# uzh-rpg/event_representation_study

Measured on AMD Instinct MI355X. Metric: events/sec/GPU (OptimizedRep, Gen1 640x480) + 12-rep GWD matrix wall-time, higher is better.
Workload: dtype f64

## Files before the change

### event_representation_study_amd/csrc/evrep_bin.hip

```cpp
#include "evrep_common.h"

namespace evrep {

#ifndef EVREP_BIN_THREADS
#define EVREP_BIN_THREADS 256
#endif
constexpr int kBinThreads = EVREP_BIN_THREADS;
constexpr int kBinWaves = kBinThreads / kWave;

template <typename Op>
__device__ inline int wave_reduce_dpp(int v, int identity, Op op) {
    v = op(v, __builtin_amdgcn_update_dpp(identity, v, 0x111, 0xf, 0xf, false));
    v = op(v, __builtin_amdgcn_update_dpp(identity, v, 0x112, 0xf, 0xf, false));
    v = op(v, __builtin_amdgcn_update_dpp(identity, v, 0x114, 0xf, 0xf, false));
    v = op(v, __builtin_amdgcn_update_dpp(identity, v, 0x118, 0xf, 0xf, false));
    v = op(v, __builtin_amdgcn_update_dpp(identity, v, 0x142, 0xa, 0xf, false));
    v = op(v, __builtin_amdgcn_update_dpp(identity, v, 0x143, 0xc, 0xf, false));
    return __builtin_amdgcn_readlane(v, 63);
}
__device__ inline int wave_min(int v) { return wave_reduce_dpp(v, INT32_MAX, [](int a, int b) { return min(a, b); }); }
__device__ inline int wave_max(int v) { return wave_reduce_dpp(v, INT32_MIN, [](int a, int b) { return max(a, b); }); }
__device__ inline uint32_t wave_or(uint32_t v) { return (uint32_t)wave_reduce_dpp((int)v, 0, [](int a, int b) { return a | b; }); }
__device__ inline int wave_sum(int v) { return wave_reduce_dpp(v, 0, [](int a, int b) { return a + b; }); }

__device__ inline void wave_phase_lds() {
    __builtin_amdgcn_fence(__ATOMIC_RELEASE, "wavefront");
    __builtin_amdgcn_wave_barrier();
    __builtin_amdgcn_fence(__ATOMIC_ACQUIRE, "wavefront");
}

struct BlockStats {
    int32_t tmin, tmax, xmin, xmax, ymin, ymax;
    uint32_t neg_flags, oob_flags, status;
    int32_t n_valid;
    int32_t pad[2];
};
static_assert(sizeof(BlockStats) == 48, "BlockStats");

__device__ inline void stats_identity(BlockStats &s) {
    s.tmin = INT32_MAX; s.tmax = INT32_MIN; s.xmin = INT32_MAX; s.xmax = INT32_MIN; s.ymin = INT32_MAX; s.ymax = INT32_MIN;
    s.neg_flags = 0; s.oob_flags = 0; s.status = 0; s.n_valid = 0; s.pad[0] = 0; s.pad[1] = 0;
}
__device__ inline void stats_merge(BlockStats &a, const BlockStats &b) {
    a.tmin = min(a.tmin, b.tmin); a.tmax = max(a.tmax, b.tmax);
    a.xmin = min(a.xmin, b.xmin); a.xmax = max(a.xmax, b.xmax);
    a.ymin = min(a.ymin, b.ymin); a.ymax = max(a.ymax, b.ymax);
    a.neg_flags |= b.neg_flags; a.oob_flags |= b.oob_flags; a.status |= b.status; a.n_valid += b.n_valid;
}
__device__ inline void stats_wave_reduce(BlockStats &s) {
    s.tmin = wave_min(s.tmin); s.tmax = wave_max(s.tmax);
    s.xmin = wave_min(s.xmin); s.xmax = wave_max(s.xmax);
    s.ymin = wave_min(s.ymin); s.ymax = wave_max(s.ymax);
    s.neg_flags = wave_or(s.neg_flags); s.oob_flags = wave_or(s.oob_flags); s.status = wave_or(s.status);
    s.n_valid = wave_sum(s.n_valid);
}

constexpr int kRegBatch = 8;

__device__ inline bool decode_window_block(int B, int nblk, int &b, int &blk) {
    const int id = blockIdx.x;
    const int per_group = 8 * nblk;
    const int grp = id / per_group, r = id - grp * per_group;
    const int nw = min(8, B - 8 * grp);
    if (nw == 8) {
        b = grp * 8 + (r & 7);
        blk = r >> 3;
        return true;
    }
    if (r >= nw * nblk) return false;
    b = grp * 8 + r / nblk;
    blk = r - (r / nblk) * nblk;
    return true;
}

#ifdef EVREP_TU_CORE
static __global__ __launch_bounds__(kBinThreads) void k_row_hist(const int4 *__restrict__ ev, const int64_t *__restrict__ off,
                                                      int B, int H, int W, int chunk, int nblk,
                                                      uint32_t *__restrict__ table, BlockStats *__restrict__ stats) {
    extern __shared__ uint32_t hist[];
    __shared__ BlockStats wstats[kBinWaves];
    int b, blk;
    if (!decode_window_block(B, nblk, b, blk)) return;
    const int64_t beg = off[b];
    const int64_t n = off[b + 1] - beg;
    const int64_t lo = (int64_t)blk * chunk;
    if (lo >= n) return;
    for (int i = threadIdx.x; i < H; i += kBinThreads) hist[i] = 0;
    __syncthreads();
    const int64_t hi = (lo + chunk < n) ? lo + chunk : n;
    const MdesWindows mw = mdes_windows(n);
    const int64_t HW = (int64_t)H * W;
    BlockStats st;
    stats_identity(st);
    for (int64_t r0 = lo; r0 < hi; r0 += (int64_t)kRegBatch * kBinThreads) {
        int4 e[kRegBatch];
        int tprev[kRegBatch];
#pragma unroll
        for (int i = 0; i < kRegBatch; ++i) {
            const int64_t r = r0 + (int64_t)i * kBinThreads + threadIdx.x;
            e[i] = make_int4(0, 0, INT32_MAX, 0);
            tprev[i] = INT32_MIN;
            if (r < hi) {
                e[i] = ev[beg + r];
                if ((threadIdx.x & 63) == 0 && r > 0) tprev[i] = ev[beg + r - 1].z;
            }
        }
#pragma unroll
        for (int i = 0; i < kRegBatch; ++i) {
            const int up = __shfl_up(e[i].z, 1, 64);
            if ((threadIdx.x & 63) != 0) tprev[i] = up;
        }
#pragma unroll
        for (int i = 0; i < kRegBatch; ++i) {
            const int64_t r = r0 + (int64_t)i * kBinThreads + threadIdx.x;
            if (r < hi) {
                const int64_t key = (int64_t)e[i].x + (int64_t)e[i].y * W;
                const uint32_t memb = mdes_membership(mw, (int32_t)r);
                if (e[i].w == -1) st.neg_flags |= memb;
                if (key >= 0 && key < HW) {
                    atomicAdd(&hist[(uint32_t)key / (uint32_t)W], 1u);
                    ++st.n_valid;
                } else {
                    st.status |= EVREP_ST_OOB;
                    const int cls = e[i].w == 1 ? 1 : (e[i].w == -1 ? 2 : (e[i].w == 0 ? 3 : 0));
                    st.oob_flags |= memb | (cls ? (memb << (7 * cls)) : 0u);
                }
                if (tprev[i] > e[i].z) st.status |= EVREP_ST_UNSORTED;
                st.tmin = min(st.tmin, e[i].z); st.tmax = max(st.tmax, e[i].z);
                st.xmin = min(st.xmin, e[i].x); st.xmax = max(st.xmax, e[i].x);
                st.ymin = min(st.ymin, e[i].y); st.ymax = max(st.ymax, e[i].y);
            }
        }
    }
    stats_wave_reduce(st);
    if ((threadIdx.x & 63) == 0) wstats[threadIdx.x >> 6] = st;
    __syncthreads();
    if (threadIdx.x == 0) {
        BlockStats t = wstats[0];
        for (int w = 1; w < kBinWaves; ++w) stats_merge(t, wstats[w]);
        stats[(size_t)b * nblk + blk] = t;
    }
    uint32_t *dst = table + ((size_t)b * nblk + blk) * H;
    for (int i = threadIdx.x; i < H; i += kBinThreads) dst[i] = hist[i];
}
#endif

#ifdef EVREP_TU_CORE
static __global__ __launch_bounds__(kBinThreads) void k_row_scan(const int64_t *__restrict__ off, int H, int chunk, int nblk,
                                                      uint32_t *__restrict__ table, uint32_t *__restrict__ row_off,
                                                      const BlockStats *__restrict__ stats, WindowMeta *__restrict__ meta) {
    extern __shared__ uint32_t rowtot[];
    __shared__ BlockStats wstats[kBinWaves];
    __shared__ uint32_t tmp[kBinWaves];
    const int b = blockIdx.x;
    const int64_t beg = off[b];
    const int64_t n = off[b + 1] - beg;
    const int nb = (int)((n + chunk - 1) / chunk);
    BlockStats st;
    stats_identity(st);
    for (int blk = threadIdx.x; blk < nb; blk += kBinThreads) stats_merge(st, stats[(size_t)b * nblk + blk]);
    stats_wave_reduce(st);
    if ((threadIdx.x & 63) == 0) wstats[threadIdx.x >> 6] = st;
    for (int r = threadIdx.x; r < H; r += kBinThreads) {
        uint32_t run = 0;
        for (int b0 = 0; b0 < nb; b0 += kRegBatch) {
            uint32_t v[kRegBatch];
#pragma unroll
            for (int i = 0; i < kRegBatch; ++i)
                v[i] = (b0 + i < nb) ? table[((size_t)b * nblk + b0 + i) * H + r] : 0u;
#pragma unroll
            for (int i = 0; i < kRegBatch; ++i)
                if (b0 + i < nb) { table[((size_t)b * nblk + b0 + i) * H + r] = run; run += v[i]; }
        }
        rowtot[r] = run;
    }
    __syncthreads();
    const int per = (H + kBinThreads - 1) / kBinThreads;
    const int r0 = threadIdx.x * per;
    uint32_t local = 0;
    for (int k = 0; k < per; ++k) if (r0 + k < H) local += rowtot[r0 + k];
    uint32_t total;
    uint32_t run = block_exclusive_scan<kBinWaves>(local, tmp, &total);
    for (int k = 0; k < per; ++k)
        if (r0 + k < H) { const uint32_t t = rowtot[r0 + k]; rowtot[r0 + k] = run; run += t; }
    __syncthreads();
    uint32_t *ro = row_off + (size_t)b * (H + 1);
    for (int r = threadIdx.x; r < H; r += kBinThreads) ro[r] = (uint32_t)beg + rowtot[r];
    if (threadIdx.x == 0) {
        ro[H] = (uint32_t)beg + total;
        BlockStats t = wstats[0];
        for (int w = 1; w < kBinWaves; ++w) stats_merge(t, wstats[w]);
        WindowMeta m;
        m.tmin = t.tmin; m.tmax = t.tmax; m.xmin = t.xmin; m.xmax = t.xmax; m.ymin = t.ymin; m.ymax = t.ymax;
        m.neg_flags = t.neg_flags; m.oob_flags = t.oob_flags; m.status = t.status; m.n_valid = t.n_valid;
        if (n <= 0) m.status |= EVREP_ST_EMPTY;
        else if (t.tmin == t.tmax) m.status |= EVREP_ST_FLAT_TIME;
        for (int i = 0; i < 6; ++i) m.pad[i] = 0;
        meta[b] = m;
    }
}
#endif

#ifdef EVREP_TU_CORE
static __global__ __launch_bounds__(kBinThreads) void k_row_scatter(const int4 *__restrict__ ev, const int64_t *__restrict__ off,
                                                         int B, int H, int W, int chunk, int nblk,
                                                         const uint32_t *__restrict__ table,
                                                         const uint32_t *__restrict__ row_off, Rec *__restrict__ sorted1) {
    extern __shared__ uint32_t cnt[];
    int b, blk;
    if (!decode_window_block(B, nblk, b, blk)) return;
    const int64_t beg = off[b];
    const int64_t n = off[b + 1] - beg;
    const int64_t lo = (int64_t)blk * chunk;
    if (lo >= n) return;
    const int64_t hi = (lo + chunk < n) ? lo + chunk : n;
    const int64_t nloc = hi - lo;
    const int lane = threadIdx.x & 63, wave = threadIdx.x >> 6;
    const int64_t wlo = lo + nloc * wave / kBinWaves, whi = lo + nloc * (wave + 1) / kBinWaves;
    const int64_t HW = (int64_t)H * W;
    constexpr int kSuper = kRegBatch * kWave;
    const int nsuper = (int)((whi - wlo + kSuper - 1) / kSuper);
    for (int i = threadIdx.x; i < kBinWaves * H; i += kBinThreads) cnt[i] = 0;
    __syncthreads();
    uint32_t *mycnt = cnt + wave * H;
    int4 e[kRegBatch];
    for (int sb = 0; sb < nsuper; ++sb) {
#pragma unroll
        for (int i = 0; i < kRegBatch; ++i) {
            const int64_t r = wlo + (int64_t)sb * kSuper + i * kWave + lane;
            e[i] = make_int4(-1, -1, 0, 0);
            if (r < whi) e[i] = ev[beg + r];
        }
#pragma unroll
        for (int i = 0; i < kRegBatch; ++i) {
            const int64_t r = wlo + (int64_t)sb * kSuper + i * kWave + lane;
            const int64_t key = (int64_t)e[i].x + (int64_t)e[i].y * W;
            if (r < whi && key >= 0 && key < HW) atomicAdd(&mycnt[(uint32_t)key / (uint32_t)W], 1u);
        }
    }
    __syncthreads();
    for (int row = threadIdx.x; row < H; row += kBinThreads) {
        uint32_t base = row_off[(size_t)b * (H + 1) + row] + table[((size_t)b * nblk + blk) * H + row];
#pragma unroll
        for (int w = 0; w < kBinWaves; ++w) { const uint32_t t = cnt[w * H + row]; cnt[w * H + row] = base; base += t; }
    }
    __syncthreads();
    const int nbits = bits_for(H);
    volatile uint32_t *vcnt = mycnt;
    for (int sb = 0; sb < nsuper; ++sb) {
        if (nsuper > 1) {
#pragma unroll
            for (int i = 0; i < kRegBatch; ++i) {
                const int64_t r = wlo + (int64_t)sb * kSuper + i * kWave + lane;
                e[i] = make_int4(-1, -1, 0, 0);
                if (r < whi) e[i] = ev[beg + r];
            }
        }
#pragma unroll
        for (int i = 0; i < kRegBatch; ++i) {
            const int64_t r0 = wlo + (int64_t)sb * kSuper + i * kWave;
            if (r0 >= whi) break;
            const int64_t r = r0 + lane;
            const int64_t key = (int64_t)e[i].x + (int64_t)e[i].y * W;
            const bool valid = r < whi && key >= 0 && key < HW;
            const uint32_t row = valid ? (uint32_t)key / (uint32_t)W : 0u;
            uint32_t rk; bool last;
            wave_match(row, nbits, valid, lane, rk, last);
            uint32_t pos = 0;
            if (valid) {
                pos = vcnt[row] + rk;
                sorted1[pos] = make_int4((int)key, (int)r, e[i].z, e[i].w);
            }
            __builtin_amdgcn_wave_barrier();
            if (valid && last) vcnt[row] = pos + 1;
            __builtin_amdgcn_wave_barrier();
        }
    }
}
#endif

constexpr int kStageRecs = 2048;
__host__ __device__ inline size_t fused_scatter_lds_bytes(int H) {
    return (size_t)(kBinWaves + 3) * H * sizeof(uint32_t) + (size_t)kStageRecs * sizeof(Rec);
}

#ifdef EVREP_TU_CORE
static __global__ __launch_bounds__(kBinThreads) void k_row_scatter_fused(const int4 *__restrict__ ev, const int64_t *__restrict__ off,
                                                               int B, int H, int W, int chunk, int nblk,
                                                               const uint32_t *__restrict__ table,
                                                               const BlockStats *__restrict__ stats,
                                                               uint32_t *__restrict__ row_off, WindowMeta *__restrict__ meta,
                                                               Rec *__restrict__ sorted1) {
    extern __shared__ __align__(16) unsigned char smem_raw[];
    Rec *stage = reinterpret_cast<Rec *>(smem_raw);
    uint32_t *cnt = reinterpret_cast<uint32_t *>(stage + kStageRecs);
    uint32_t *rowtot = cnt + kBinWaves * H;
    uint32_t *lbase = rowtot + H;
    uint32_t *delta = lbase + H;
    __shared__ BlockStats wstats[kBinWaves];
    __shared__ uint32_t tmp[kBinWaves];
    int b, blk;
    if (!decode_window_block(B, nblk, b, blk)) return;
    const int64_t beg = off[b];
    const int64_t n = off[b + 1] - beg;
    const int64_t lo = (int64_t)blk * chunk;
    if (lo >= n && !(blk == 0)) return;
    const int nb = (int)((n + chunk - 1) / chunk);
    if (n <= 0) {
        uint32_t *ro = row_off + (size_t)b * (H + 1);
        for (int r = threadIdx.x; r <= H; r += kBinThreads) ro[r] = (uint32_t)beg;
        if (threadIdx.x == 0) {
            WindowMeta m;
            m.tmin = INT32_MAX; m.tmax = INT32_MIN; m.xmin = INT32_MAX; m.xmax = INT32_MIN; m.ymin = INT32_MAX; m.ymax = INT32_MIN;
            m.neg_flags = 0; m.oob_flags = 0; m.status = EVREP_ST_EMPTY; m.n_valid = 0;
            for (int i = 0; i < 6; ++i) m.pad[i] = 0;
            meta[b] = m;
        }
        return;
    }
    const int64_t hi = (lo + chunk < n) ? lo + chunk : n;
    const int64_t nloc = hi - lo;
    const int lane = threadIdx.x & 63, wave = threadIdx.x >> 6;
    const int64_t wlo = lo + nloc * wave / kBinWaves, whi = lo + nloc * (wave + 1) / kBinWaves;
    const int64_t HW = (int64_t)H * W;
    for (int i = threadIdx.x; i < kBinWaves * H; i += kBinThreads) cnt[i] = 0;
    __syncthreads();
    uint32_t *mycnt = cnt + wave * H;
    int4 e[kRegBatch];
#pragma unroll
    for (int i = 0; i < kRegBatch; ++i) {
        const int64_t r = wlo + i * kWave + lane;
        e[i] = make_int4(-1, -1, 0, 0);
        if (r < whi) e[i] = ev[beg + r];
    }
#pragma unroll
    for (int i = 0; i < kRegBatch; ++i) {
        const int64_t r = wlo + i * kWave + lane;
        const int64_t key = (int64_t)e[i].x + (int64_t)e[i].y * W;
        if (r < whi && key >= 0 && key < HW) atomicAdd(&mycnt[(uint32_t)key / (uint32_t)W], 1u);
    }
    if (blk == 0) {
        BlockStats st;
        stats_identity(st);
        for (int k = threadIdx.x; k < nb; k += kBinThreads) stats_merge(st, stats[(size_t)b * nblk + k]);
        stats_wave_reduce(st);
        if (lane == 0) wstats[wave] = st;
    }
    __syncthreads();
    for (int r = threadIdx.x; r < H; r += kBinThreads) {
        uint32_t tot = 0, before = 0;
        for (int b0 = 0; b0 < nb; b0 += kRegBatch) {
            uint32_t v[kRegBatch];
#pragma unroll
            for (int i = 0; i < kRegBatch; ++i) v[i] = (b0 + i < nb) ? table[((size_t)b * nblk + b0 + i) * H + r] : 0u;
#pragma unroll
            for (int i = 0; i < kRegBatch; ++i) { tot += v[i]; if (b0 + i < blk) before += v[i]; }
        }
        rowtot[r] = tot;
        delta[r] = before;
        uint32_t own = 0;
#pragma unroll
        for (int w = 0; w < kBinWaves; ++w) own += cnt[w * H + r];
        lbase[r] = own;
    }
    __syncthreads();
    const int per = (H + kBinThreads - 1) / kBinThreads;
    const int r0 = threadIdx.x * per;
    uint32_t loc_t = 0, loc_o = 0;
    for (int k = 0; k < per; ++k) if (r0 + k < H) { loc_t += rowtot[r0 + k]; loc_o += lbase[r0 + k]; }
    uint32_t total_t, total_o;
    uint32_t run_t = block_exclusive_scan<kBinWaves>(loc_t, tmp, &total_t);
    uint32_t run_o = block_exclusive_scan<kBinWaves>(loc_o, tmp, &total_o);
    for (int k = 0; k < per; ++k)
        if (r0 + k < H) {
            const uint32_t t = rowtot[r0 + k]; rowtot[r0 + k] = run_t; run_t += t;
            const uint32_t o = lbase[r0 + k];  lbase[r0 + k] = run_o;  run_o += o;
        }
    __syncthreads();
    for (int r = threadIdx.x; r < H; r += kBinThreads) {
        const uint32_t gstart = (uint32_t)beg + rowtot[r] + delta[r];
        uint32_t base = lbase[r];
        delta[r] = gstart - base;
#pragma unroll
        for (int w = 0; w < kBinWaves; ++w) { const uint32_t t = cnt[w * H + r]; cnt[w * H + r] = base; base += t; }
        if (blk == 0) row_off[(size_t)b * (H + 1) + r] = (uint32_t)beg + rowtot[r];
    }
    if (blk == 0 && threadIdx.x == 0) {
        row_off[(size_t)b * (H + 1) + H] = (uint32_t)beg + total_t;
        BlockStats t = wstats[0];
        for (int w = 1; w < kBinWaves; ++w) stats_merge(t, wstats[w]);
        WindowMeta m;
        m.tmin = t.tmin; m.tmax = t.tmax; m.xmin = t.xmin; m.xmax = t.xmax; m.ymin = t.ymin; m.ymax = t.ymax;
        m.neg_flags = t.neg_flags; m.oob_flags = t.oob_flags; m.status = t.status; m.n_valid = t.n_valid;
        if (t.tmin == t.tmax) m.status |= EVREP_ST_FLAT_TIME;
        for (int i = 0; i < 6; ++i) m.pad[i] = 0;
        meta[b] = m;
    }
    __syncthreads();
    const int nbits = bits_for(H);
    volatile uint32_t *vcnt = mycnt;
#pragma unroll
    for (int i = 0; i < kRegBatch; ++i) {
        const int64_t rr0 = wlo + i * kWave;
        if (rr0 >= whi) break;
        const int64_t r = rr0 + lane;
        const int64_t key = (int64_t)e[i].x + (int64_t)e[i].y * W;
        const bool valid = r < whi && key >= 0 && key < HW;
        const uint32_t row = valid ? (uint32_t)key / (uint32_t)W : 0u;
        uint32_t rk; bool last;
        wave_match(row, nbits, valid, lane, rk, last);
        uint32_t pos = 0;
        if (valid) {
            pos = vcnt[row] + rk;
            stage[pos] = make_int4((int)key, (int)r, e[i].z, e[i].w);
        }
        __builtin_amdgcn_wave_barrier();
        if (valid && last) vcnt[row] = pos + 1;
        __builtin_amdgcn_wave_barrier();
    }
    __syncthreads();
    for (uint32_t t = threadIdx.x; t < total_o; t += kBinThreads) {
        const Rec rec = stage[t];
        const uint32_t row = (uint32_t)rec.x / (uint32_t)W;
        sorted1[delta[row] + t] = rec;
    }
}
#endif

#ifdef EVREP_TU_CORE
static __global__ __launch_bounds__(kWave) void k_col_sort(const Rec *__restrict__ sorted1, const uint32_t *__restrict__ row_off,
                                                   int H, int W, int nchunk, Rec *__restrict__ sorted2,
                                                   uint32_t *__restrict__ chunk_off) {
    extern __shared__ uint32_t cnt[];
    const int b = blockIdx.y, row = blockIdx.x;
    const int lane = threadIdx.x;
    const uint32_t rs = row_off[(size_t)b * (H + 1) + row], re = row_off[(size_t)b * (H + 1) + row + 1];
    const uint32_t n = re - rs;
    uint32_t *co = chunk_off + ((size_t)b * H + row) * (nchunk + 1);
    if (n == 0) {
        for (int c = lane; c <= nchunk; c += kWave) co[c] = rs;
        return;
    }
    constexpr uint32_t kSuper = 4 * kWave;
    const int rowbase = row * W;
    const uint32_t nsuper = (n + kSuper - 1) / kSuper;
    Rec e[4];
    for (int i = lane; i < W; i += kWave) cnt[i] = 0;
    __syncthreads();
    for (uint32_t sb = 0; sb < nsuper; ++sb) {
#pragma unroll
        for (int i = 0; i < 4; ++i) {
            const uint32_t j = sb * kSuper + i * kWave + lane;
            e[i] = make_int4(0, 0, 0, 0);
            if (j < n) e[i] = sorted1[rs + j];
        }
#pragma unroll
        for (int i = 0; i < 4; ++i)
            if (sb * kSuper + i * kWave + lane < n) atomicAdd(&cnt[e[i].x - rowbase], 1u);
    }
    __syncthreads();
    const int per = (W + kWave - 1) / kWave;
    const int c0 = lane * per;
    uint32_t local = 0;
    for (int k = 0; k < per; ++k) if (c0 + k < W) local += cnt[c0 + k];
    uint32_t incl = local;
#pragma unroll
    for (int d = 1; d < 64; d <<= 1) { const uint32_t o = __shfl_up(incl, d, 64); if (lane >= d) incl += o; }
    uint32_t run = incl - local;
    for (int k = 0; k < per; ++k)
        if (c0 + k < W) { const uint32_t t = cnt[c0 + k]; cnt[c0 + k] = run; run += t; }
    __syncthreads();
    for (int c = lane; c <= nchunk; c += kWave) co[c] = (c * kChunkPx < W) ? rs + cnt[c * kChunkPx] : re;
    __syncthreads();
    const int nbits = bits_for(W);
    volatile uint32_t *vcnt = cnt;
    for (uint32_t sb = 0; sb < nsuper; ++sb) {
        if (nsuper > 1) {
#pragma unroll
// ... 169 lines not shown
    volatile uint16_t *vpos = cnt16 + (size_t)wave * Hp;
#pragma unroll
    for (int i = 0; i < kBsPerLane; ++i) {
        if (wlo + i * kWave >= whi) break;
        const bool valid = rows[i] != 0xffffffffu;
        const uint32_t row = valid ? rows[i] : 0u;
        uint32_t rk = 0; bool last = false;
        if (!(BS_DEBUG & 2)) wave_match(row, nbits, valid, lane, rk, last);
        uint32_t pos = 0;
        if (valid) {
            pos = (BS_DEBUG & 2) ? (uint32_t)(wave * 512 + i * 64 + lane) : (uint32_t)vpos[row] + rk;
            const int64_t r = wlo + i * kWave + lane;
            const Rec rec = make_int4((int)((int64_t)e[i].x + (int64_t)e[i].y * W), (int)r, e[i].z, e[i].w);
            if (BS_DEBUG & 16) sorted1[beg + lo + pos] = rec; else stage[pos] = rec;
        }
        __builtin_amdgcn_wave_barrier();
        if (valid && last) vpos[row] = (uint16_t)(pos + 1);
        __builtin_amdgcn_wave_barrier();
    }
    __syncthreads();
    Rec *dst = sorted1 + beg + lo;
    if (!(BS_DEBUG & (4 | 16)))
        for (uint32_t t = threadIdx.x; t < total; t += kBsThreads) dst[t] = stage[t];
}
#endif

#ifndef EVREP_CS_WAVES
#define EVREP_CS_WAVES 8
#endif
constexpr int kCsWaves = EVREP_CS_WAVES;
constexpr int kCsRowWaves = 4;
constexpr int kCsMaxRuns = 128;
__host__ __device__ inline int col_sort_per4(int W) { return ((W + kWave - 1) / kWave + 3) / 4; }
__host__ __device__ inline int col_sort_words(int W) { return kWave * 4 * col_sort_per4(W); }
__host__ __device__ inline int col_sort_wave_words(int W) { return col_sort_words(W) + 2 * kCsMaxRuns; }

#ifndef CS_WAVES
#define CS_WAVES 8
#endif
#ifdef EVREP_TU_CORE
static __global__ __launch_bounds__(kCsWaves * kWave) __attribute__((amdgpu_waves_per_eu(CS_WAVES))) void k_col_sort_runs(const int4 *__restrict__ ev, const Rec *__restrict__ sorted1, const int64_t *__restrict__ off,
                                                                     const uint32_t *__restrict__ table,
                                                                     const BlockStats *__restrict__ stats, int H, int W, int nblk,
                                                                     int nchunk, int kpr, int chunk_shift, int by_key,
                                                                     Rec *__restrict__ sorted2,
                                                                     uint32_t *__restrict__ chunk_off, WindowMeta *__restrict__ meta) {
    extern __shared__ __align__(16) uint32_t cnt_all[];
    const int lane = threadIdx.x & 63, wave = threadIdx.x >> 6;
    const int b = blockIdx.y, unit = blockIdx.x * (int)(blockDim.x >> 6) + wave;
    if (unit >= (by_key ? H * kpr : H)) return;
    const int row = by_key ? unit / kpr : unit;
    const int ck = by_key ? unit - row * kpr : 0;
    const int Wu = by_key ? min(kChunkPx, W - ck * kChunkPx) : W;
    uint32_t *cnt = cnt_all + (size_t)wave * col_sort_wave_words(by_key ? kChunkPx : W);
    const int64_t beg = off[b];
    const int64_t n_win = off[b + 1] - beg;
    const int nb = min((int)(((uint32_t)n_win + (1u << chunk_shift) - 1u) >> chunk_shift), nblk);
    uint32_t ta[2] = {0u, 0u}, tb[2] = {0u, 0u};
#pragma unroll
    for (int h = 0; h < 2; ++h) {
        const int k = lane + h * kWave;
        if (k < nb) {
            const uint32_t *tk = table + ((size_t)b * nblk + k) * ((size_t)H * kpr + 1);
            ta[h] = tk[by_key ? (size_t)unit : (size_t)row * kpr];
            tb[h] = tk[by_key ? (size_t)unit + 1 : (size_t)(row + 1) * kpr];
        }
    }
    if (unit == 0) {
        BlockStats st;
        stats_identity(st);
#pragma unroll
        for (int h = 0; h < 2; ++h) {
            const int k = lane + h * kWave;
            if (k < nb) {
                const int4 *sp = reinterpret_cast<const int4 *>(stats + (size_t)b * nblk + k);
                const int4 q0 = sp[0], q1 = sp[1], q2 = sp[2];
                st.tmin = min(st.tmin, q0.x); st.tmax = max(st.tmax, q0.y); st.xmin = min(st.xmin, q0.z); st.xmax = max(st.xmax, q0.w);
                st.ymin = min(st.ymin, q1.x); st.ymax = max(st.ymax, q1.y);
                st.neg_flags |= (uint32_t)q1.z; st.oob_flags |= (uint32_t)q1.w;
                st.status |= (uint32_t)q2.x; st.n_valid += q2.y;
            }
        }
        stats_wave_reduce(st);
        if (lane == 0) {
            WindowMeta m;
            m.tmin = st.tmin; m.tmax = st.tmax; m.xmin = st.xmin; m.xmax = st.xmax; m.ymin = st.ymin; m.ymax = st.ymax;
            m.neg_flags = st.neg_flags; m.oob_flags = st.oob_flags; m.status = st.status & 0xffffu; m.n_valid = st.n_valid;
            if (n_win <= 0) m.status |= EVREP_ST_EMPTY;
            else if (st.tmin == st.tmax) m.status |= EVREP_ST_FLAT_TIME;
            for (int i = 0; i < 6; ++i) m.pad[i] = 0;
            meta[b] = m;
        }
    }
    constexpr uint32_t kSuper = 4 * kWave;
    const uint32_t rbeg = (uint32_t)beg + (uint32_t)wave_sum((int)(ta[0] + ta[1]));
    const uint32_t len0 = tb[0] - ta[0], len1 = tb[1] - ta[1];
    uint32_t incl0 = len0, incl1 = len1;
#pragma unroll
    for (int d = 1; d < 64; d <<= 1) {
        const uint32_t o0 = __shfl_up(incl0, d, 64), o1 = __shfl_up(incl1, d, 64);
        if (lane >= d) { incl0 += o0; incl1 += o1; }
    }
    const uint32_t tot0 = (uint32_t)__builtin_amdgcn_readlane((int)incl0, 63);
    incl1 += tot0;
    const uint32_t n = (uint32_t)__builtin_amdgcn_readlane((int)incl1, 63);
    const uint32_t pre0 = incl0 - len0, pre1 = incl1 - len1;
    const uint32_t src0 = (uint32_t)beg + ((uint32_t)lane << chunk_shift) + ta[0] - pre0;
    const uint32_t src1 = (uint32_t)beg + ((uint32_t)(lane + kWave) << chunk_shift) + ta[1] - pre1;
    const uint32_t rend = rbeg + n;
    uint32_t *runs = cnt + col_sort_words(by_key ? kChunkPx : W);
    if (nb > kBsChainBlocks) {
        runs[lane] = pre0;
        runs[kWave + lane] = pre1;
        runs[kCsMaxRuns + lane] = src0;
        runs[kCsMaxRuns + kWave + lane] = src1;
        wave_phase_lds();
    }
    const Rec8 *sorted8 = reinterpret_cast<const Rec8 *>(sorted1);
    const int4 *evw = ev + beg;
    auto load = [&](uint32_t at) -> Rec {
        return by_key ? rec8_unpack(sorted8[at], row * W, ck * kChunkPx, evw) : sorted1[at];
    };
    auto fetch = [&](uint32_t j) -> Rec {
        if (nb <= kBsChainBlocks) {
            uint32_t s = (uint32_t)__builtin_amdgcn_readlane((int)src0, 0);
            uint32_t prev = s;
            for (int k = 1; k < nb; ++k) {
                const uint32_t pk = (uint32_t)__builtin_amdgcn_readlane((int)pre0, k);
                const uint32_t sk = (uint32_t)__builtin_amdgcn_readlane((int)src0, k);
                s += (j >= pk) ? sk - prev : 0u;
                prev = sk;
            }
            return load(s + j);
        }
        uint32_t lo = 0, hi = (uint32_t)nb;
#pragma unroll
        for (int step = 0; step < 7; ++step) {
            const uint32_t mid = (lo + hi) >> 1;
            const bool go = hi - lo > 1 && runs[mid] <= j;
            if (hi - lo > 1) { if (go) lo = mid; else hi = mid; }
        }
        return load(runs[kCsMaxRuns + lo] + j);
    };
    Rec e[4];
#pragma unroll
    for (int i = 0; i < 4; ++i) {
        const uint32_t j = i * kWave + lane;
        e[i] = make_int4(0, 0, 0, 0);
        if (j < n) e[i] = fetch(j);
    }
    const int nbits = bits_for(Wu);
    const int per4 = col_sort_per4(Wu);
    uint4 *cnt4 = reinterpret_cast<uint4 *>(cnt) + (size_t)lane * per4;
    volatile uint32_t *vcnt = cnt;
    uint32_t *co = chunk_off + ((size_t)b * H + row) * (nchunk + 1);
    if (by_key && lane == 0) {
        co[ck] = rbeg;
        if (ck == kpr - 1) co[kpr] = rend;
    }
    if (n == 0) {
        if (!by_key) for (int c = lane; c <= nchunk; c += kWave) co[c] = rbeg;
        return;
    }
    const int rowbase = row * W + ck * kChunkPx;
    const uint32_t nsuper = (n + kSuper - 1) / kSuper;
    for (int k = 0; k < per4; ++k) cnt4[k] = make_uint4(0u, 0u, 0u, 0u);
    wave_phase_lds();
#pragma unroll
    for (int i = 0; i < 4; ++i)
        if ((uint32_t)(i * kWave + lane) < n) atomicAdd(&cnt[e[i].x - rowbase], 1u);
    for (uint32_t sb = 1; sb < nsuper; ++sb)
        for (int i = 0; i < 4; ++i) {
            const uint32_t j = sb * kSuper + i * kWave + lane;
            if (j < n) atomicAdd(&cnt[fetch(j).x - rowbase], 1u);
        }
    wave_phase_lds();
    uint32_t local = 0;
    for (int k = 0; k < per4; ++k) { const uint4 v = cnt4[k]; local += v.x + v.y + v.z + v.w; }
    uint32_t inc2 = local;
#pragma unroll
    for (int d = 1; d < 64; d <<= 1) { const uint32_t o = __shfl_up(inc2, d, 64); if (lane >= d) inc2 += o; }
    uint32_t run = inc2 - local;
    for (int k = 0; k < per4; ++k) {
        const uint4 v = cnt4[k];
        uint4 o;
        o.x = run; o.y = o.x + v.x; o.z = o.y + v.y; o.w = o.z + v.z;
        run = o.w + v.w;
        cnt4[k] = o;
    }
    wave_phase_lds();
    if (!by_key) for (int c = lane; c <= nchunk; c += kWave) co[c] = (c * kChunkPx < W) ? rbeg + cnt[c * kChunkPx] : rend;
    wave_phase_lds();
    for (uint32_t sb = 0; sb < nsuper; ++sb) {
#pragma unroll
        for (int i = 0; i < 4; ++i) {
            const uint32_t j0 = sb * kSuper + i * kWave;
            if (j0 >= n) break;
            const bool valid = j0 + lane < n;
            Rec rec = e[i];
            if (sb > 0) { rec = make_int4(0, 0, 0, 0); if (valid) rec = fetch(j0 + lane); }
            const uint32_t col = valid ? (uint32_t)(rec.x - rowbase) : 0u;
            uint32_t rk; bool last;
            wave_match(col, nbits, valid, lane, rk, last);
            uint32_t pos = 0;
            if (valid) {
                pos = vcnt[col] + rk;
                sorted2[rbeg + pos] = rec;
            }
            __builtin_amdgcn_wave_barrier();
            if (valid && last) vcnt[col] = pos + 1;
            __builtin_amdgcn_wave_barrier();
        }
    }
}
#endif

#ifndef KS_DIRECT_WRITE
#define KS_DIRECT_WRITE 0
#endif
#ifndef KS_DEBUG
#define KS_DEBUG 0
#endif
constexpr int kKsHotGroup = 16;
__host__ __device__ inline size_t block_keysort_lds_bytes(int NK, int cap, int chunk) {
    return (size_t)cap * sizeof(Rec8) + (size_t)chunk * sizeof(uint16_t) + (size_t)(NK + 4) * sizeof(uint32_t);
}

#ifndef KS_WAVES_512
#define KS_WAVES_512 6
#endif
#ifndef KS_WAVES_1024
#define KS_WAVES_1024 8
#endif
template <int TPB, int PL = 8>
__global__ __launch_bounds__(TPB) __attribute__((amdgpu_waves_per_eu(TPB == 1024 ? KS_WAVES_1024 : KS_WAVES_512))) void k_block_keysort(const int4 *__restrict__ ev, const int64_t *__restrict__ off,
                                                             int B, int H, int W, int kpr, int nblk, int cap,
                                                             uint32_t *__restrict__ table, BlockStats *__restrict__ stats,
                                                             Rec *__restrict__ sorted1, int64_t *__restrict__ nwin,
                                                             uint32_t *__restrict__ hot) {
    extern __shared__ __align__(16) unsigned char smem_raw[];
    constexpr int kChunk = TPB * PL, kNW = TPB / kWave, kPerWave = PL * kWave;
    if (blockIdx.x == 0 && threadIdx.x < 128) hot[threadIdx.x * 16] = 0u;
    const int NK = H * kpr;
    Rec8 *stage = reinterpret_cast<Rec8 *>(smem_raw);
    uint16_t *rankbuf = reinterpret_cast<uint16_t *>(stage + cap);
    uint32_t *base = reinterpret_cast<uint32_t *>(rankbuf + kChunk);
    __shared__ int bstats[12];
    __shared__ uint32_t tmp[kNW];
    __shared__ uint32_t nhot_s;
    int b, blk;
    if (!decode_window_block(B, nblk, b, blk)) return;
    const int64_t beg = off[b];
    const int64_t n = off[b + 1] - beg;
    const int64_t lo = (int64_t)blk * kChunk;
    if (blk == 0 && threadIdx.x == 0) nwin[b] = n;
    if (lo >= n) return;
    const int nblock = (int)((lo + kChunk < n) ? kChunk : n - lo);
    const int lane = threadIdx.x & 63, wave = threadIdx.x >> 6;
    const int w0 = wave * kPerWave;
    const int lo32 = (int)lo;
    const int4 *evb = ev + beg + lo;
    int4 e[PL];
    int tprev[PL];
#pragma unroll
    for (int i = 0; i < PL; ++i) {
        const int li = w0 + i * kWave + lane;
        e[i] = make_int4(-1, -1, INT32_MAX, 0);
        tprev[i] = INT32_MIN;
        if (li < nblock) {
            e[i] = evb[li];
            if (lane == 0 && (li > 0 || lo > 0)) tprev[i] = evb[li - 1].z;
        }
    }
    for (int i = threadIdx.x; i <= NK; i += TPB) base[i] = 0;
    if (threadIdx.x == 0) nhot_s = 0u;
    if (threadIdx.x < 12) {
        const int f = threadIdx.x;
        bstats[f] = (f == 0 || f == 2 || f == 4) ? INT32_MAX : ((f == 1 || f == 3 || f == 5) ? INT32_MIN : 0);
    }
    __syncthreads();
    const MdesWindows mw = mdes_windows(n);
    uint32_t full = 0, part = 0;
#pragma unroll
    for (int i = 0; i < 7; ++i) {
        if (mw.lo[i] <= lo32 && lo32 + nblock <= mw.hi[i]) full |= 1u << i;
        else if (!(lo32 + nblock <= mw.lo[i] || lo32 >= mw.hi[i])) part |= 1u << i;
    }
    BlockStats st;
    stats_identity(st);
    uint32_t ko[PL];
    uint32_t sneg = 0;
    bool cut = false;
    const int a0 = lo32 + w0, a1 = min(lo32 + w0 + kPerWave, lo32 + nblock);
    if (part) {
#pragma unroll
        for (int q = 0; q < 7; ++q) cut |= (mw.lo[q] > a0 && mw.lo[q] < a1) || (mw.hi[q] > a0 && mw.hi[q] < a1);
    }
    const uint32_t memb_u = cut ? 0u : (full | (part ? (mdes_membership(mw, a0) & part) : 0u));
    const int HW = H * W;
#pragma unroll
    for (int i = 0; i < PL; ++i) {
        const int li = w0 + i * kWave + lane;
        const bool in = li < nblock;
        const int up = __builtin_amdgcn_update_dpp(0, e[i].z, 0x138 , 0xf, 0xf, false);
        if (lane != 0) tprev[i] = up;
        uint32_t row = (uint32_t)e[i].y, col = (uint32_t)e[i].x;
        bool valid = in && (uint32_t)e[i].x < (uint32_t)W && (uint32_t)e[i].y < (uint32_t)H;
        if (__any(in && (uint32_t)e[i].x >= (uint32_t)W)) {
            const int64_t key = (int64_t)e[i].x + (int64_t)e[i].y * W;
            valid = in && key >= 0 && key < (int64_t)HW;
            if (valid) { row = (uint32_t)key / (uint32_t)W; col = (uint32_t)key - row * (uint32_t)W; }
        }
        ko[i] = 0xffffffffu;
        if (valid) {
            const uint32_t key = row * (uint32_t)kpr + (col >> 7);
            ko[i] = key | (atomicAdd(&base[key], 1u) << 16);
        }
        if (KS_DEBUG & 4) continue;
        if (!cut) {
            if (__any(in && e[i].w == -1)) sneg |= memb_u;
        } else if (in && e[i].w == -1) {
            st.neg_flags |= full | (mdes_membership(mw, lo32 + li) & part);
        }
        if (__any(in && !valid)) {
            if (in && !valid) {
                const uint32_t memb = cut ? (full | (mdes_membership(mw, lo32 + li) & part)) : memb_u;
                st.status |= EVREP_ST_OOB;
                const int cls = e[i].w == 1 ? 1 : (e[i].w == -1 ? 2 : (e[i].w == 0 ? 3 : 0));
                st.oob_flags |= memb | (cls ? (memb << (7 * cls)) : 0u);
            }
        }
        if (in) {
            if (valid) ++st.n_valid;
            if (tprev[i] > e[i].z) st.status |= EVREP_ST_UNSORTED;
            if ((uint32_t)(e[i].w + 1) > 2u) st.status |= kStEscaped;
            st.tmin = min(st.tmin, e[i].z); st.tmax = max(st.tmax, e[i].z);
            st.xmin = min(st.xmin, e[i].x); st.xmax = max(st.xmax, e[i].x);
            st.ymin = min(st.ymin, e[i].y); st.ymax = max(st.ymax, e[i].y);
        }
    }
    st.neg_flags |= sneg;
    stats_wave_reduce(st);
    if (lane == 0) {
        atomicMin(&bstats[0], st.tmin); atomicMax(&bstats[1], st.tmax);
        atomicMin(&bstats[2], st.xmin); atomicMax(&bstats[3], st.xmax);
        atomicMin(&bstats[4], st.ymin); atomicMax(&bstats[5], st.ymax);
        atomicOr(reinterpret_cast<uint32_t *>(&bstats[6]), st.neg_flags);
        atomicOr(reinterpret_cast<uint32_t *>(&bstats[7]), st.oob_flags);
        atomicOr(reinterpret_cast<uint32_t *>(&bstats[8]), st.status);
        atomicAdd(&bstats[9], st.n_valid);
    }
    __syncthreads();
    const int per = (NK + TPB - 1) / TPB;
    const int k0 = (int)threadIdx.x * per;
    uint32_t local = 0;
    for (int k = 0; k < per; ++k) if (k0 + k < NK) local += base[k0 + k];
    uint32_t total;
    uint32_t run = block_exclusive_scan<kNW>(local, tmp, &total);
    for (int k = 0; k < per; ++k)
        if (k0 + k < NK) {
            const uint32_t c = base[k0 + k];
            uint32_t tag = 0u;
            if (c > (uint32_t)kKsHotGroup) tag = (atomicAdd(&nhot_s, 1u) + 1u) << 16;
            base[k0 + k] = run | tag;
            run += c;
        }
    if (threadIdx.x == 0) base[NK] = total;
    if (threadIdx.x < 12) reinterpret_cast<int *>(stats + (size_t)b * nblk + blk)[threadIdx.x] = bstats[threadIdx.x];
    __syncthreads();
    uint32_t *tb = table + ((size_t)b * nblk + blk) * ((size_t)NK + 1);
    if (!(KS_DEBUG & 8))
        for (int k = threadIdx.x; k <= NK; k += TPB) tb[k] = base[k] & 0xffffu;
    const uint32_t nhot = nhot_s;
    const uint32_t mine0 = (uint32_t)(w0 + lane);
#pragma unroll
    for (int i = 0; i < PL; ++i) {
        if (ko[i] != 0xffffffffu) {
            const uint32_t bw = base[ko[i] & 0xffffu];
            if (!(bw >> 16)) rankbuf[(bw & 0xffffu) + (ko[i] >> 16)] = (uint16_t)(mine0 + i * kWave);
        }
    }
    if (nhot) {
        constexpr int kHs = kChunk / 16;
        uint32_t *hcnt = reinterpret_cast<uint32_t *>(stage);
        for (uint32_t t = lane; t < nhot; t += kWave) hcnt[wave * kHs + t] = 0u;
        wave_phase_lds();
#pragma unroll
        for (int i = 0; i < PL; ++i)
            if (ko[i] != 0xffffffffu) {
                const uint32_t hsl = base[ko[i] & 0xffffu] >> 16;
                if (hsl) atomicAdd(&hcnt[wave * kHs + hsl - 1u], 1u);
            }
        __syncthreads();
        if (threadIdx.x < nhot) {
            uint32_t acc = 0;
            for (int w = 0; w < kNW; ++w) { const uint32_t c = hcnt[w * kHs + threadIdx.x]; hcnt[w * kHs + threadIdx.x] = acc; acc += c; }
        }
        __syncthreads();
        const int hbits = bits_for((int)nhot);
        volatile uint32_t *vh = hcnt + wave * kHs;
#pragma unroll
        for (int i = 0; i < PL; ++i) {
            const uint32_t bw = ko[i] != 0xffffffffu ? base[ko[i] & 0xffffu] : 0u;
            const bool hot = (bw >> 16) != 0u;
            if (!__any(hot)) continue;
            const uint32_t slot = hot ? (bw >> 16) - 1u : 0u;
            uint32_t rk; bool last;
            wave_match(slot, hbits, hot, lane, rk, last);
            uint32_t pos = 0;
            if (hot) {
                pos = vh[slot] + rk;
                ko[i] = ((bw & 0xffffu) + pos) | 0x80000000u;
            }
            __builtin_amdgcn_wave_barrier();
            if (hot && last) vh[slot] = pos + 1;
            __builtin_amdgcn_wave_barrier();
        }
    }
    __syncthreads();
    {
        uint32_t gb[PL], g[PL], sm[PL];
        uint32_t gmax = 0;
#pragma unroll
        for (int i = 0; i < PL; ++i) {
            gb[i] = 0; g[i] = 0; sm[i] = 0;
            if (ko[i] != 0xffffffffu && !(ko[i] >> 31)) {
                const uint32_t key = ko[i] & 0xffffu;
                const uint32_t bw = base[key];
                gb[i] = bw & 0xffffu;
                g[i] = (bw >> 16) ? 0u : (base[key + 1] & 0xffffu) - gb[i];
                if (KS_DEBUG & 1) { sm[i] = ko[i] >> 16; g[i] = 0; }
                if (g[i] == 1) g[i] = 0;
                gmax = max(gmax, g[i]);
            }
        }
        gmax = (uint32_t)wave_max((int)gmax);
        for (uint32_t j = 0; j < gmax; ++j) {
#pragma unroll
            for (int i = 0; i < PL; ++i)
                if (j < g[i]) sm[i] += (uint32_t)rankbuf[gb[i] + j] < mine0 + (uint32_t)(i * kWave) ? 1u : 0u;
        }
#pragma unroll
        for (int i = 0; i < PL; ++i)
            if (ko[i] != 0xffffffffu) ko[i] = (ko[i] >> 31) ? (ko[i] & 0x7fffffffu) : gb[i] + sm[i];
    }
    if (nhot) __syncthreads();
    Rec8 *dst = reinterpret_cast<Rec8 *>(sorted1) + beg + lo;
#if KS_DIRECT_WRITE
#pragma unroll
    for (int i = 0; i < PL; ++i) {
        if (ko[i] != 0xffffffffu && !(KS_DEBUG & 2)) {
            int col = e[i].x;
            if ((uint32_t)col >= (uint32_t)W) { const uint32_t key = (uint32_t)(e[i].x + e[i].y * W); col = (int)(key % (uint32_t)W); }
            dst[ko[i]] = rec8_pack(col, lo32 + w0 + i * kWave + lane, e[i].z, e[i].w);
        }
    }
    return;
#endif
    for (uint32_t pb = 0; pb < total && !(KS_DEBUG & 2); pb += (uint32_t)cap) {
        if (pb) __syncthreads();
#pragma unroll
        for (int i = 0; i < PL; ++i) {
            const uint32_t pos = ko[i] - pb;
            if (pos < (uint32_t)cap) {
                int col = e[i].x;
                if ((uint32_t)col >= (uint32_t)W) { const uint32_t key = (uint32_t)(e[i].x + e[i].y * W); col = (int)(key % (uint32_t)W); }
                stage[pos] = rec8_pack(col, lo32 + w0 + i * kWave + lane, e[i].z, e[i].w);
            }
        }
        __syncthreads();
        const uint32_t cnt = min((uint32_t)cap, total - pb);
        for (uint32_t t = threadIdx.x; t < cnt; t += TPB) dst[pb + t] = stage[t];
    }
}

#ifdef EVREP_TU_CORE
static __global__ __launch_bounds__(kWave) void k_window_meta(const int64_t *__restrict__ nwin, const BlockStats *__restrict__ stats,
                                                      int nblk, int chunk_shift, WindowMeta *__restrict__ meta) {
    const int b = blockIdx.x, lane = threadIdx.x;
    const int64_t n_win = nwin[b];
    const int nb = min((int)(((uint32_t)n_win + (1u << chunk_shift) - 1u) >> chunk_shift), nblk);
    BlockStats st;
    stats_identity(st);
    for (int k = lane; k < nb; k += kWave) stats_merge(st, stats[(size_t)b * nblk + k]);
    stats_wave_reduce(st);
    if (lane == 0) {
        WindowMeta m;
        m.tmin = st.tmin; m.tmax = st.tmax; m.xmin = st.xmin; m.xmax = st.xmax; m.ymin = st.ymin; m.ymax = st.ymax;
        m.neg_flags = st.neg_flags; m.oob_flags = st.oob_flags; m.status = st.status & 0xffffu; m.n_valid = st.n_valid;
        if (n_win <= 0) m.status |= EVREP_ST_EMPTY;
        else if (st.tmin == st.tmax) m.status |= EVREP_ST_FLAT_TIME;
        for (int i = 0; i < 6; ++i) m.pad[i] = 0;
        meta[b] = m;
    }
}
#endif

}
```

### event_representation_study_amd/csrc/evrep_builders.hip

```cpp
#include "evrep_common.h"
#include "evrep_est_table.h"

namespace evrep {

__host__ __device__ inline size_t align16(size_t v) { return (v + 15) & ~(size_t)15; }

#ifndef EVREP_ES_WAVES
#define EVREP_ES_WAVES 6
#endif
#ifndef EVREP_TORE_WAVES
#define EVREP_TORE_WAVES 1
#endif
#ifndef EVREP_VOXEL_WAVES
#define EVREP_VOXEL_WAVES 6
#endif
#ifndef EVREP_PARTS
#define EVREP_PARTS 2
#endif
#ifndef EVREP_DEFER_MULT
#define EVREP_DEFER_MULT 1
#endif
#ifndef EVREP_XCD_MAP
#define EVREP_XCD_MAP 1
#endif
// ... 118 lines not shown
}

template <typename OutT>
__device__ inline void tile_store(const OutT *tile, int count, OutT *__restrict__ dst) {
    constexpr int V = 16 / (int)sizeof(OutT);
    if ((reinterpret_cast<uintptr_t>(dst) & 15u) == 0) {
        const int nvec = count / V;
        int v = threadIdx.x;
#if EVREP_NT_STORES
        typedef float nt4 __attribute__((ext_vector_type(4)));
        const nt4 *n4 = reinterpret_cast<const nt4 *>(tile);
        nt4 *o4 = reinterpret_cast<nt4 *>(dst);
        for (; v + 3 * kWave < nvec; v += 4 * kWave) {
            const nt4 a = n4[v], b = n4[v + kWave], c = n4[v + 2 * kWave], d = n4[v + 3 * kWave];
            __builtin_nontemporal_store(a, o4 + v); __builtin_nontemporal_store(b, o4 + v + kWave);
            __builtin_nontemporal_store(c, o4 + v + 2 * kWave); __builtin_nontemporal_store(d, o4 + v + 3 * kWave);
        }
        for (; v < nvec; v += kWave) __builtin_nontemporal_store(n4[v], o4 + v);
#else
        const float4 *s4 = reinterpret_cast<const float4 *>(tile);
        float4 *d4 = reinterpret_cast<float4 *>(dst);
        for (; v + 3 * kWave < nvec; v += 4 * kWave) {
            const float4 a = s4[v], b = s4[v + kWave], c = s4[v + 2 * kWave], d = s4[v + 3 * kWave];
            d4[v] = a; d4[v + kWave] = b; d4[v + 2 * kWave] = c; d4[v + 3 * kWave] = d;
        }
        for (; v < nvec; v += kWave) d4[v] = s4[v];
#endif
        for (int e = nvec * V + threadIdx.x; e < count; e += kWave) dst[e] = tile[e];
    } else {
        for (int e = threadIdx.x; e < count; e += kWave) dst[e] = tile[e];
    }
}

#ifndef EVREP_STREAM_BYRUN
#define EVREP_STREAM_BYRUN 12
#endif
#ifndef EVREP_STREAM_G
#define EVREP_STREAM_G 4
#endif
#ifndef EVREP_ORDERED_BYRUN
#define EVREP_ORDERED_BYRUN 48
#endif
#ifndef EVREP_VOXEL_BYRUN
#define EVREP_VOXEL_BYRUN 48
#endif
#ifndef EVREP_MDES_STREAM_BYRUN
#define EVREP_MDES_STREAM_BYRUN 48
#endif
__device__ inline int chunk_unit(int total) {
    const int lin = (int)(blockIdx.x + gridDim.x * (blockIdx.y + gridDim.y * blockIdx.z));
#if EVREP_XCD_MAP
    if ((total & 7) == 0) {
        const int per = total >> 3, xcd = lin & 7;
#ifdef EVREP_XCD_ROT
        int idx = (lin >> 3) + xcd * (EVREP_XCD_ROT);
        idx %= per;
#else
        const int idx = lin >> 3;
#endif
        return xcd * per + idx;
    }
#endif
    return lin;
}

struct ChunkGeom {
    int b, row, c0, npix;
    uint32_t cs, ce;
};

struct BinView {
    const int4 *ev;
    const Rec *sorted;
    const uint32_t *chunk_off;
    const uint32_t *table;
    const BlockStats *stats;
    const WindowMeta *meta;
    Rec *spill;
    int nblk, fused, chunk_shift;
    uint32_t *hot;
    uint32_t hot_cap;
    double *placed_pool;
    BlockStats *stats_rw;
#ifdef EVREP_TIMING
    unsigned long long *dbg;
    unsigned long long *dbg_wave;
#endif
};

struct UnitRecs {
    const Rec *sorted;
    uint32_t cs, ce;
    int nstaged;
    Rec r0;
    int nseg, pos;
    bool deferred;
    int part;
    uint32_t pst, pen;
    bool hot_lds;
    int dpx, npixu;
    int sub;
};

__device__ inline uint32_t wave_incl_scan(uint32_t v) {
    int x = (int)v;
    x += __builtin_amdgcn_update_dpp(0, x, 0x111, 0xf, 0xf, false);
    x += __builtin_amdgcn_update_dpp(0, x, 0x112, 0xf, 0xf, false);
    x += __builtin_amdgcn_update_dpp(0, x, 0x114, 0xf, 0xf, false);
    x += __builtin_amdgcn_update_dpp(0, x, 0x118, 0xf, 0xf, false);
    x += __builtin_amdgcn_update_dpp(0, x, 0x142, 0xa, 0xf, false);
    x += __builtin_amdgcn_update_dpp(0, x, 0x143, 0xc, 0xf, false);
    return (uint32_t)x;
}

__device__ inline uint32_t wave_incl_max_scan(uint32_t v) {
    int x = (int)v;
    x = max(x, __builtin_amdgcn_update_dpp(0, x, 0x111, 0xf, 0xf, false));
    x = max(x, __builtin_amdgcn_update_dpp(0, x, 0x112, 0xf, 0xf, false));
    x = max(x, __builtin_amdgcn_update_dpp(0, x, 0x114, 0xf, 0xf, false));
    x = max(x, __builtin_amdgcn_update_dpp(0, x, 0x118, 0xf, 0xf, false));
    x = max(x, __builtin_amdgcn_update_dpp(0, x, 0x142, 0xa, 0xf, false));
    x = max(x, __builtin_amdgcn_update_dpp(0, x, 0x143, 0xc, 0xf, false));
    return (uint32_t)x;
}

__device__ inline int piece_px0(int code) { return code < kHotParts ? code * kWave : ((code - kHotParts) >> 2) * kWave + ((code - kHotParts) & 3) * (kWave / 4); }
__device__ inline int piece_npx(int code) { return code < kHotParts ? kWave : kWave / 4; }
template <bool HOT, typename Body>
__device__ inline void run_units(const BinView &bv, Body body) {
    if constexpr (!HOT) {
        body(chunk_unit((int)(gridDim.x * gridDim.y * gridDim.z)), -1);
    } else {
        const uint32_t l = blockIdx.x % kHotLists, capl = hot_sublist_cap(bv.hot_cap);
        const uint32_t nraw = (uint32_t)__builtin_amdgcn_readfirstlane((int)bv.hot[l * 16]);
        if (nraw == 0u) return;
        const uint32_t n = min(nraw, capl);
        const uint32_t *items = bv.hot + kHotHdrWords + (size_t)l * capl;
        for (uint32_t it = blockIdx.x / kHotLists; it < n; it += gridDim.x / kHotLists) {
            const int item = __builtin_amdgcn_readfirstlane((int)items[it]);
            if (item >= 0) body(item / kHotCodes, item % kHotCodes);
            wave_phase();
        }
        if (threadIdx.x == 0) {
            const uint32_t ticket = atomicAdd(&bv.hot[(kHotLists + l) * 16], 1u);
            if (ticket + 1u == gridDim.x / kHotLists) {
                bv.hot[(kHotLists + l) * 16] = 0u;
                bv.hot[l * 16] = 0u;
            }
        }
    }
}
__device__ inline bool defer_unit(const BinView &bv, int uid, int nparts, uint32_t splitmask) {
    const uint32_t capl = hot_sublist_cap(bv.hot_cap);
    const int lane = threadIdx.x, p = lane >> 2, sq = lane & 3;
    const bool split = (splitmask >> p) & 1u;
    const bool active = p < nparts && (split || sq == 0);
    const uint64_t am = __ballot(active);
    const uint32_t nitems = (uint32_t)__popcll(am), pos = (uint32_t)__popcll(am & ((1ull << lane) - 1ull));
    const uint32_t code = split ? (uint32_t)(kHotParts + 4 * p + sq) : (uint32_t)p;
    uint32_t l = ((uint32_t)uid * 0x9E3779B1u) >> 26;
    for (int tries = 0; tries < kHotLists; ++tries, l = (l + 1) % kHotLists) {
        uint32_t at = 0;
        if (threadIdx.x == 0) at = atomicAdd(&bv.hot[l * 16], nitems);
        at = (uint32_t)__builtin_amdgcn_readfirstlane((int)at);
        uint32_t *items = bv.hot + kHotHdrWords + (size_t)l * capl;
        if (at + nitems <= capl) {
            if (active) items[at + pos] = (uint32_t)uid * (uint32_t)kHotCodes + code;
            return true;
        }
        if (active && at + pos < capl) items[at + pos] = 0xffffffffu;
    }
// ... 211 lines not shown
        const uint32_t px1 = v1 ? (uint32_t)(r1.x - keybase) : 0u;
        if (v0) atomicAdd(&cnt[px], 1u);
        if (v1) atomicAdd(&cnt[px1], 1u);
        wave_phase();
        {
            uint32_t local = 0;
            for (int k = 0; k < per4; ++k) {
                const int v = lane * per4 + k;
                if (v * 4 < npixu) { const uint4 c = cnt4[v]; local += c.x + c.y + c.z + c.w; }
            }
            uint32_t run = wave_incl_scan(local) - local;
            for (int k = 0; k < per4; ++k) {
                const int v = lane * per4 + k;
                if (v * 4 < npixu) {
                    const uint4 c = cnt4[v];
                    uint4 o;
                    o.x = run; o.y = o.x + c.x; o.z = o.y + c.y; o.w = o.z + c.z;
                    run = o.w + c.w;
                    cnt4[v] = o;
                }
            }
        }
        wave_phase();
        uint32_t rk; bool last;
        wave_match(px, nbits, v0, lane, rk, last);
        uint32_t pos = 0;
        if (v0) { pos = cnt[px] + rk; w.evbuf[pos] = r; }
        wave_phase();
        if (v0 && last) cnt[px] = pos + 1;
        wave_phase();
        wave_match(px1, nbits, v1, lane, rk, last);
        if (v1) w.evbuf[cnt[px1] + rk] = r1;
        wave_phase();
        if (v0) r = w.evbuf[lane];
        u.r0 = r;
        return u;
    }
    const int dpx = segbase - keybase;
    const int plo = HOT ? piece_px0(part) + dpx : 0, phi = HOT ? min(piece_px0(part) + piece_npx(part), npix_out) + dpx : npixu;
    u.part = HOT ? part : -2;
#ifndef EVREP_MAIN_SPILL_BATCH
#define EVREP_MAIN_SPILL_BATCH 4
#endif
#ifndef EVREP_HOT_SPILL_BATCH
#define EVREP_HOT_SPILL_BATCH 16
#endif
    constexpr int kSpillBatch = HOT ? EVREP_HOT_SPILL_BATCH : EVREP_MAIN_SPILL_BATCH;
    const uint32_t cs = (uint32_t)beg + (uint32_t)__builtin_amdgcn_readlane((int)wave_incl_scan(a), 63);
    const bool hot_sub = HOT && Split::enabled && Split::in_hot && part >= kHotSub0 && part < kHotSub0 + kHotSubMax;
    if (HOT && !(Split::enabled && Split::in_hot && (part == kHotWhole || hot_sub))) {
      if constexpr (HOT) {
        const Rec *slot = bv.spill + cs;
        const int px = plo + lane;
        const bool own = px >= 0 && px < phi && px < npixu;
        uint32_t lo0 = 0, hi0 = nrec, lo1 = 0, hi1 = nrec;
        const int key = keybase + px;
        while (__any(own && (lo0 < hi0 || lo1 < hi1))) {
            if (own && lo0 < hi0) { const uint32_t mid = (lo0 + hi0) >> 1; if (slot[mid].x < key) lo0 = mid + 1; else hi0 = mid; }
            if (own && lo1 < hi1) { const uint32_t mid = (lo1 + hi1) >> 1; if (slot[mid].x <= key) lo1 = mid + 1; else hi1 = mid; }
        }
        w.mark(3);
        u.pst = own ? lo0 : 0u; u.pen = own ? lo1 : 0u;
        u.hot_lds = false;
        u.cs = cs; u.ce = cs + nrec;
        u.nstaged = 0;
        u.dpx = dpx; u.npixu = npixu;
        return u;
      }
    }
    if constexpr (Split::enabled && Split::in_hot && !HOT) {
        const uint32_t stw = wave_or(lane < nb ? split.st_lane : 0u);
        if (!(stw & kStEscaped) && (nrec >= split.min_rec || (split.coop_min != 0u && nrec >= split.coop_min)) && nrec <= 65535u && dpx == 0) {
            bool ok;
            if (split.coop_min != 0u && nrec >= split.coop_min) {
                ok = defer_items(bv, uid, (uint32_t)kHotCoop, 1u);
            } else if (Split::sliceable && nrec >= kHotSubMin) {
                uint4 *z = reinterpret_cast<uint4 *>(bv.spill + cs);
                const uint32_t nz = (kHotSubHdrBytes + 4u * split_gwpp(split.words_per_px) * (uint32_t)npixu + 15u) / 16u;
                for (uint32_t i = (uint32_t)lane; i < nz; i += kWave) z[i] = make_uint4(0u, 0u, 0u, 0u);
                ok = defer_items(bv, uid, (uint32_t)kHotSub0, hot_sub_count(nrec));
            } else {
                ok = defer_items(bv, uid, (uint32_t)kHotWhole, 1u);
            }
            if (!ok && lane == 0) atomicOr(&bv.stats_rw[(size_t)b * bv.nblk].status, EVREP_ST_HOT_OVERFLOW);
            u.deferred = true;
            u.ce = nrec;
            return u;
        }
    }
    for (int v = lane; v * 4 < npixu; v += kWave) cnt4[v] = make_uint4(0u, 0u, 0u, 0u);
    wave_phase();
    uint32_t jlo = 0, jhi = nrec;
    if (hot_sub) {
        const uint32_t S = hot_sub_count(nrec), qs = hot_sub_quota(nrec, S);
        jlo = min(nrec, (uint32_t)(part - kHotSub0) * qs);
        jhi = min(nrec, jlo + qs);
    }
    const bool by_run = !hot_sub && nrec >= (uint32_t)EVREP_ORDERED_BYRUN * (uint32_t)nb;
    const uint32_t run0 = (uint32_t)beg + ((uint32_t)lane << bv.chunk_shift) + a;
    uint32_t *runs2 = cnt + npixu;
    if (!by_run && nb > kBsChainBlocks) { runs2[lane] = pre; runs2[64 + lane] = src; }
    wave_phase();
    auto src_of = [&](uint32_t j) -> uint32_t {
        if (nb <= kBsChainBlocks) {
            uint32_t sx = (uint32_t)__builtin_amdgcn_readlane((int)src, 0);
            uint32_t prev = sx;
            for (int k = 1; k < nb; ++k) {
                const uint32_t pk = (uint32_t)__builtin_amdgcn_readlane((int)pre, k);
                const uint32_t sk = (uint32_t)__builtin_amdgcn_readlane((int)src, k);
                sx += (j >= pk) ? sk - prev : 0u;
                prev = sk;
            }
            return sx + j;
        }
        uint32_t lo = 0, hi = (uint32_t)nb;
#pragma unroll
        for (int step = 0; step < 6; ++step) {
            const uint32_t mid = (lo + hi) >> 1;
            const bool go = hi - lo > 1 && runs2[mid] <= j;
            if (hi - lo > 1) { if (go) lo = mid; else hi = mid; }
        }
        return runs2[64 + lo] + j;
    };
    int rk_ = 0;
    uint32_t ro_ = 0;
    uint32_t addr[kSpillBatch], bcnt[kSpillBatch];
    Rec8 q[kSpillBatch];
    auto sweep_begin = [&]() { rk_ = 0; ro_ = by_run ? 0u : jlo; };
    auto skip_empty = [&]() {
        uint32_t lk = rk_ < nb ? (uint32_t)__builtin_amdgcn_readlane((int)len, rk_) : 0u;
        while (rk_ < nb && ro_ >= lk) { ++rk_; ro_ = 0; lk = rk_ < nb ? (uint32_t)__builtin_amdgcn_readlane((int)len, rk_) : 0u; }
        return lk;
    };
    auto sweep_done = [&]() -> bool { if (by_run) { skip_empty(); return rk_ >= nb; } return ro_ >= jhi; };
    auto load_batch = [&]() -> bool {
        bool any = false;
        if (by_run) {
#pragma unroll
            for (int sl = 0; sl < kSpillBatch; ++sl) {
                const uint32_t lk = skip_empty();
                bcnt[sl] = 0u; addr[sl] = 0u;
                if (rk_ < nb) {
                    addr[sl] = (uint32_t)__builtin_amdgcn_readlane((int)run0, rk_) + ro_;
                    bcnt[sl] = min(lk - ro_, (uint32_t)kWave);
                    ro_ += kWave;
                    any = true;
                }
            }
#pragma unroll
            for (int sl = 0; sl < kSpillBatch; ++sl) {
                q[sl] = make_uint2(0u, 0u);
                if ((uint32_t)lane < bcnt[sl]) q[sl] = s8[addr[sl] + (uint32_t)lane];
            }
        } else {
#pragma unroll
            for (int sl = 0; sl < kSpillBatch; ++sl) {
                const uint32_t j0 = ro_ + (uint32_t)(sl * kWave);
                bcnt[sl] = j0 < jhi ? min(jhi - j0, (uint32_t)kWave) : 0u;
                q[sl] = make_uint2(0u, 0u);
                if ((uint32_t)lane < bcnt[sl]) q[sl] = s8[src_of(j0 + (uint32_t)lane)];
            }
            any = ro_ < jhi;
            ro_ += (uint32_t)(kSpillBatch * kWave);
        }
        return any;
    };
    auto px_of = [&](const Rec8 &r) -> uint32_t { return ((r.y & 511u) - (uint32_t)c0) & 511u; };
// ... 24 lines not shown
        const uint32_t wbytes = ((uint32_t)npixu * (uint32_t)split.words_per_px * 4u + 15u) & ~15u;
        if (wbytes + 64u * 8u <= room && nrec <= 65535u && dpx == 0 && split.begin()) {
            const uint32_t lcap = split_list_cap(room, wbytes);
            uint4 *t4 = reinterpret_cast<uint4 *>(w.tile);
            for (uint32_t v = (uint32_t)lane; v * 16u < wbytes; v += kWave) t4[v] = make_uint4(0u, 0u, 0u, 0u);
            wave_phase();
            uint2 *list = reinterpret_cast<uint2 *>(reinterpret_cast<unsigned char *>(w.tile) + wbytes);
            uint2 *glist = reinterpret_cast<uint2 *>(bv.spill + cs);
            unsigned char *slot = reinterpret_cast<unsigned char *>(bv.spill + cs);
            const uint32_t gwpp = split_gwpp(split.words_per_px);
            uint2 *sublists = reinterpret_cast<uint2 *>(slot + ((kHotSubHdrBytes + 4u * gwpp * (uint32_t)npixu + 15u) & ~15u));
            if (hot_sub) glist = sublists + jlo;
            const uint32_t lcap_eff = hot_sub ? 0u : lcap;
            uint32_t nk = 0;
            sweep_begin();
            while (load_batch()) {
                uint2 aux[kSpillBatch];
#pragma unroll
                for (int sl = 0; sl < kSpillBatch; ++sl) {
                    aux[sl] = make_uint2(0u, 0u);
                    if ((uint32_t)lane < bcnt[sl]) aux[sl] = split.pre(q[sl]);
                }
#pragma unroll
                for (int sl = 0; sl < kSpillBatch; ++sl) {
                    if (bcnt[sl] == 0u) break;
                    bool keep = false;
                    uint2 e = make_uint2(0u, 0u);
                    if ((uint32_t)lane < bcnt[sl]) keep = split.f(px_of(q[sl]), q[sl], e, aux[sl]);
                    const uint64_t km = __ballot(keep);
                    if (km) {
                        const uint32_t at = nk + (uint32_t)__popcll(km & ((1ull << lane) - 1ull));
                        if (keep) {
                            if (at < lcap_eff) list[at] = e; else glist[at] = e;
                            atomicAdd(&cnt[e.y], 1u);
                        }
                        nk += (uint32_t)__popcll(km);
                    }
                }
                if (sweep_done()) break;
            }
            wave_phase();
            if (hot_sub) {
                uint32_t *gw = reinterpret_cast<uint32_t *>(slot + kHotSubHdrBytes);
                uint32_t *hdr = reinterpret_cast<uint32_t *>(slot);
                const uint32_t *lw = reinterpret_cast<const uint32_t *>(w.tile);
                for (uint32_t px = (uint32_t)lane; px < (uint32_t)npixu; px += kWave) split.merge(lw + px * (uint32_t)split.words_per_px, gw + px * gwpp);
                for (uint32_t px = (uint32_t)lane; px < (uint32_t)npixu; px += kWave) { const uint32_t kc = cnt[px]; if (kc) atomicAdd(gw + px * gwpp + (gwpp - 1u), kc); }
                const uint32_t S = hot_sub_count(nrec);
                uint32_t ticket = 0;
                __threadfence();
                if (lane == 0) {
                    hdr[1 + (part - kHotSub0)] = nk;
                    __threadfence();
                    ticket = atomicAdd(hdr, 1u);
                }
                ticket = (uint32_t)__builtin_amdgcn_readfirstlane((int)ticket);
                if (ticket + 1u != S) { u.deferred = true; return u; }
                __threadfence();
                uint32_t *lwm = reinterpret_cast<uint32_t *>(w.tile);
                for (uint32_t px = (uint32_t)lane; px < (uint32_t)npixu; px += kWave) {
                    for (uint32_t k = 0; k < (uint32_t)split.words_per_px; ++k)
                        lwm[px * (uint32_t)split.words_per_px + k] = __hip_atomic_load(gw + px * gwpp + k, __ATOMIC_RELAXED, __HIP_MEMORY_SCOPE_AGENT);
                    cnt[px] = __hip_atomic_load(gw + px * gwpp + (gwpp - 1u), __ATOMIC_RELAXED, __HIP_MEMORY_SCOPE_AGENT);
                }
                uint32_t tot = 0;
                if (lane < (int)S) tot = __hip_atomic_load(hdr + 1 + lane, __ATOMIC_RELAXED, __HIP_MEMORY_SCOPE_AGENT);
                const uint32_t incl = wave_incl_scan(tot);
                nk = (uint32_t)__builtin_amdgcn_readlane((int)incl, 63);
                wave_phase();
                u.sub = (int)S;
            }
            if (split.done()) {
                u.part = -5;
                u.cs = cs; u.ce = cs + nrec;
                u.nstaged = 0;
                u.dpx = dpx; u.npixu = npixu;
                u.pst = nk; u.pen = wbytes;
                return u;
            }
            for (int v = lane; v * 4 < npixu; v += kWave) cnt4[v] = make_uint4(0u, 0u, 0u, 0u);
            wave_phase();
        }
        if constexpr (HOT) {
            if (lane == 0) atomicOr(&bv.stats_rw[(size_t)b * bv.nblk].status, EVREP_ST_HOT_OVERFLOW);
            u.deferred = true;
            return u;
        }
    }
    if constexpr (LAST && !HOT) {
        if (npixu <= w.bigcap) {
            sweep_begin();
            while (load_batch()) {
#pragma unroll
                for (int sl = 0; sl < kSpillBatch; ++sl)
                    if ((uint32_t)lane < bcnt[sl]) atomicMax(&cnt[px_of(q[sl])], (((q[sl].y >> 11) + 1u) << 2) | ((q[sl].y >> 9) & 3u));
                if (sweep_done()) break;
            }
            wave_phase();
            uint32_t nlast = 0;
            for (int p0 = 0; p0 < npixu; p0 += kWave) {
                const int px = p0 + lane;
                const uint32_t v = cnt[px];
                const uint64_t m = __ballot(v != 0u);
                const uint32_t pos = nlast + (uint32_t)__popcll(m & ((1ull << lane) - 1ull));
                if (v != 0u) {
                    const int rank = (int)(v >> 2) - 1;
                    const uint32_t p2 = v & 3u;
                    *w.big_at(pos) = make_int4(keybase + px, rank, 0, p2 == 3u ? evw[rank].w : (int)p2 - 1);
                }
                cnt[px] = pos + (v != 0u ? 1u : 0u);
                nlast += (uint32_t)__popcll(m);
            }
            wave_phase();
            u.part = -3;
            u.cs = cs; u.ce = cs + nlast;
            u.nstaged = 0;
            u.dpx = dpx; u.npixu = npixu;
            u.pst = 0; u.pen = 0;
            return u;
        }
    }
    sweep_begin();
    bool resident = false;
    for (int round = 0; load_batch(); ++round) {
#pragma unroll
        for (int sl = 0; sl < kSpillBatch; ++sl)
            if ((uint32_t)lane < bcnt[sl]) atomicAdd(&cnt[px_of(q[sl])], 1u);
        if (sweep_done()) { resident = round == 0; break; }
    }
    wave_phase();
    {
        uint32_t local = 0;
        for (int k = 0; k < per4; ++k) {
            const int v = lane * per4 + k;
            if (v * 4 < npixu) { const uint4 c = cnt4[v]; local += c.x + c.y + c.z + c.w; }
        }
        uint32_t run = wave_incl_scan(local) - local;
        for (int k = 0; k < per4; ++k) {
            const int v = lane * per4 + k;
            if (v * 4 < npixu) {
                const uint4 c = cnt4[v];
                uint4 o;
                o.x = run; o.y = o.x + c.x; o.z = o.y + c.y; o.w = o.z + c.z;
                run = o.w + c.w;
                cnt4[v] = o;
            }
        }
    }
    wave_phase();
    const bool in_lds = !HOT && nrec <= (uint32_t)w.bigcap;
    bool defer = false;
    uint32_t defer_mask = 0u;
    if (!HOT && !in_lds) {
        bool fits = true;
        uint32_t splitmask = 0u;
        for (int o0 = 0; o0 < npix_out; o0 += kWave) {
            const int lo = o0 + dpx, hi = min(o0 + kWave, npix_out) + dpx;
            const uint32_t b0 = lo <= 0 ? 0u : (lo < npixu ? cnt[lo] : nrec), b1 = hi <= 0 ? 0u : (hi < npixu ? cnt[hi] : nrec);
            fits = fits && b1 - b0 <= (uint32_t)(EVREP_DEFER_MULT * w.bigcap);
            if (b1 - b0 > (uint32_t)(w.bigcap - w.nstage + kHotStage)) splitmask |= 1u << (o0 / kWave);
        }
#ifdef EVREP_NO_QUARTERS
        splitmask = 0u;
#endif
#ifdef EVREP_NO_DEFER
        fits = true;
#endif
        if constexpr (Split::enabled && !Split::in_hot) fits = true;
        defer = !fits;
        defer_mask = splitmask;
    }
    wave_phase();
    volatile uint32_t *vcnt = cnt;
    if (!resident) sweep_begin();
    for (bool more = resident ? true : load_batch(); more; more = resident ? false : load_batch()) {
#pragma unroll
        for (int sl = 0; sl < kSpillBatch; ++sl) {
            if (bcnt[sl] == 0u) break;
            uint32_t px = px_of(q[sl]);
            const bool valid = (uint32_t)lane < bcnt[sl] && (int)px >= plo && (int)px < phi;
            if (!__any(valid)) continue;
            if (!valid) px = 0u;
            uint32_t rk; bool last;
            wave_match(px, nbits, valid, lane, rk, last);
            uint32_t pos = 0;
            if (valid) {
                pos = vcnt[px] + rk;
                const Rec rec = rec8_unpack(q[sl], row_base, c0, evw);
                if (in_lds) *w.big_at(pos) = rec; else bv.spill[cs + pos] = rec;
            }
            __builtin_amdgcn_wave_barrier();
            if (valid && last) vcnt[px] = pos + 1;
            __builtin_amdgcn_wave_barrier();
        }
    }
    wave_phase();
    if (defer) {
        if (!defer_unit(bv, uid, (npix_out + kWave - 1) / kWave, defer_mask) && lane == 0)
            atomicOr(&bv.stats_rw[(size_t)b * bv.nblk].status, EVREP_ST_HOT_OVERFLOW);
        u.deferred = true;
        u.ce = nrec;
        return u;
    }
    u.pst = 0; u.pen = 0;
    if (in_lds) u.part = -3;
    u.hot_lds = false;
    __builtin_amdgcn_fence(__ATOMIC_RELEASE, "workgroup");
    __builtin_amdgcn_wave_barrier();
    __builtin_amdgcn_fence(__ATOMIC_ACQUIRE, "workgroup");
    u.cs = cs;
    u.ce = cs + nrec;
    u.nstaged = 0;
    u.dpx = dpx; u.npixu = npixu;
    return u;
}

template <typename OutT, bool HOT>
__device__ inline void stage_classic(UnitRecs &u, WaveLds<OutT, HOT> &w) {
    const int nrec = (int)(u.ce - u.cs), lane = threadIdx.x;
    const int n = min(nrec, w.nstage);
    if (n <= kWave || (w.nstage <= 2 * kEvStage && nrec > w.nstage)) return;
    const Rec *src = u.sorted + u.cs + lane;
    const bool h1 = kWave + lane < n, h2 = 2 * kWave + lane < n, h3 = 3 * kWave + lane < n;
    Rec t1 = make_int4(0, 0, 0, 0), t2 = t1, t3 = t1;
    if (h1) t1 = src[kWave];
    if (h2) t2 = src[2 * kWave];
    if (h3) t3 = src[3 * kWave];
    if (h1) w.evbuf[kWave + lane] = t1;
    if (h2) w.evbuf[2 * kWave + lane] = t2;
    if (h3) w.evbuf[3 * kWave + lane] = t3;
    u.nstaged = n;
}

template <typename OutT, bool HOT, bool LAST = false, typename Visit = NoVisit, typename Split = NoSplit>
__device__ inline UnitRecs unit_front(const BinView &bv, const int64_t *__restrict__ off, int H, int W, int nchunk, const UnitCfg &uc,
                                      WaveLds<OutT, HOT> &w, ChunkGeom &g, int uid, int part, Visit visit = Visit(), Split split = Split()) {
    int chunk, nch;
    g = unit_geom(H, W, nchunk, uc, chunk, nch, uid);
    if (bv.fused) {
        const int klo = g.row * nchunk + chunk, khi = klo + nch;
        const UnitRecs u = unit_records<OutT, HOT, LAST, Visit, Split>(bv, off, g.b, H * nchunk, klo, khi, g.row * W + g.c0, w.segcap, w, g.row * W + g.c0, g.c0, uid, g.npix, part, visit, split);
        g.cs = u.cs; g.ce = u.ce;
        return u;
    }
    const uint32_t *co = bv.chunk_off + ((size_t)g.b * H + g.row) * (nchunk + 1);
    g.cs = co[chunk];
    g.ce = co[chunk + nch];
    UnitRecs u;
    u.sorted = bv.sorted; u.cs = g.cs; u.ce = g.ce; u.nstaged = kEvStage;
    u.r0 = make_int4(INT32_MIN, 0, 0, 0);
    u.nseg = -1; u.pos = (int)threadIdx.x; u.deferred = false; u.part = -1; u.hot_lds = false; u.sub = 0;
    if ((int)threadIdx.x < (int)(g.ce - g.cs)) u.r0 = bv.sorted[g.cs + threadIdx.x];
    stage_classic(u, w);
    return u;
}

struct MetaRaw {
    int4 q0, q1, q2;
};
__device__ inline MetaRaw meta_prefetch(const BinView &bv, int b) {
    MetaRaw r;
    r.q0 = make_int4(0, 0, 0, 0); r.q1 = r.q0; r.q2 = r.q0;
    if (bv.fused) {
        if ((int)threadIdx.x < bv.nblk) {
            const int4 *sp = reinterpret_cast<const int4 *>(bv.stats + (size_t)b * bv.nblk + threadIdx.x);
            r.q0 = sp[0]; r.q1 = sp[1]; r.q2 = sp[2];
        }
    } else if (threadIdx.x == 0) {
        const int4 *mp = reinterpret_cast<const int4 *>(bv.meta + b);
        r.q0 = mp[0]; r.q1 = mp[1]; r.q2 = mp[2];
    }
    return r;
}
__device__ inline WindowMeta meta_finish(const BinView &bv, const int64_t *__restrict__ off, int b, const MetaRaw &r) {
    WindowMeta m;
    if (!bv.fused) {
        m.tmin = __builtin_amdgcn_readfirstlane(r.q0.x); m.tmax = __builtin_amdgcn_readfirstlane(r.q0.y);
        m.xmin = __builtin_amdgcn_readfirstlane(r.q0.z); m.xmax = __builtin_amdgcn_readfirstlane(r.q0.w);
        m.ymin = __builtin_amdgcn_readfirstlane(r.q1.x); m.ymax = __builtin_amdgcn_readfirstlane(r.q1.y);
        m.neg_flags = (uint32_t)__builtin_amdgcn_readfirstlane(r.q1.z);
        m.oob_flags = (uint32_t)__builtin_amdgcn_readfirstlane(r.q1.w);
        m.status = (uint32_t)__builtin_amdgcn_readfirstlane(r.q2.x); m.n_valid = __builtin_amdgcn_readfirstlane(r.q2.y);
        return m;
    }
    const int lane = threadIdx.x;
    const int64_t n_win = off[b + 1] - off[b];
    const int nb = min((int)(((uint32_t)n_win + (1u << bv.chunk_shift) - 1u) >> bv.chunk_shift), bv.nblk);
    BlockStats st;
    stats_identity(st);
    if (lane < nb) {
        st.tmin = r.q0.x; st.tmax = r.q0.y; st.xmin = r.q0.z; st.xmax = r.q0.w;
        st.ymin = r.q1.x; st.ymax = r.q1.y; st.neg_flags = (uint32_t)r.q1.z; st.oob_flags = (uint32_t)r.q1.w;
        st.status = (uint32_t)r.q2.x; st.n_valid = r.q2.y;
    }
    m.tmin = nb > 0 ? __builtin_amdgcn_readlane(st.tmin, 0) : INT32_MAX;
    m.tmax = nb > 0 ? __builtin_amdgcn_readlane(st.tmax, min(nb, kWave) - 1) : INT32_MIN;
    if (nb > kWave) {
        BlockStats s2;
        stats_identity(s2);
        if (kWave + lane < nb) {
            const int4 *sp = reinterpret_cast<const int4 *>(bv.stats + (size_t)b * bv.nblk + kWave + lane);
            const int4 a0 = sp[0], a1 = sp[1], a2 = sp[2];
            s2.tmin = a0.x; s2.tmax = a0.y; s2.xmin = a0.z; s2.xmax = a0.w;
            s2.ymin = a1.x; s2.ymax = a1.y; s2.neg_flags = (uint32_t)a1.z; s2.oob_flags = (uint32_t)a1.w;
            s2.status = (uint32_t)a2.x; s2.n_valid = a2.y;
        }
        m.tmax = __builtin_amdgcn_readlane(s2.tmax, nb - kWave - 1);
        stats_merge(st, s2);
    }
    m.xmin = wave_min(st.xmin); m.xmax = wave_max(st.xmax);
    m.ymin = wave_min(st.ymin); m.ymax = wave_max(st.ymax);
    m.neg_flags = wave_or(st.neg_flags); m.oob_flags = wave_or(st.oob_flags);
    m.status = wave_or(st.status); m.n_valid = wave_sum(st.n_valid);
    if (m.status & EVREP_ST_UNSORTED) {
        m.tmin = wave_min(st.tmin);
        m.tmax = wave_max(st.tmax);
    }
    return m;
}
__device__ inline WindowMeta window_meta(const BinView &bv, const int64_t *__restrict__ off, int b) {
    return meta_finish(bv, off, b, meta_prefetch(bv, b));
}

template <typename OutT>
__device__ inline void sparse_store(const OutT *vlist, const unsigned char *map, int npix, int C, OutT *__restrict__ dst) {
    constexpr int V = 16 / (int)sizeof(OutT);
    typedef float nt4 __attribute__((ext_vector_type(4)));
    const int lane = threadIdx.x;
    const int vpp = C / V;
    const uint32_t inv = (65536u + (uint32_t)vpp - 1u) / (uint32_t)vpp;
    const int nvec = npix * vpp;
    const int dq = (int)((64u * inv) >> 16), dr = 64 - dq * vpp;
    const nt4 *vl4 = reinterpret_cast<const nt4 *>(vlist);
    nt4 *o4 = reinterpret_cast<nt4 *>(dst) + lane;
    int pixel = (int)(((uint32_t)lane * inv) >> 16);
    int sub = lane - pixel * vpp;
    auto gather = [&]() -> nt4 {
        const nt4 r = vl4[(int)map[pixel] * vpp + sub];
        sub += dr; pixel += dq;
        if (sub >= vpp) { sub -= vpp; ++pixel; }
        return r;
    };
    int v0 = 0;
    for (; v0 + 4 * kWave <= nvec; v0 += 4 * kWave) {
        const nt4 a = gather(), b = gather(), c = gather(), d = gather();
#if EVREP_NT_STORES
        __builtin_nontemporal_store(a, o4 + v0); __builtin_nontemporal_store(b, o4 + v0 + kWave);
        __builtin_nontemporal_store(c, o4 + v0 + 2 * kWave); __builtin_nontemporal_store(d, o4 + v0 + 3 * kWave);
#else
        o4[v0] = a; o4[v0 + kWave] = b; o4[v0 + 2 * kWave] = c; o4[v0 + 3 * kWave] = d;
#endif
    }
    for (; v0 < nvec; v0 += kWave) {
        if (v0 + lane < nvec) {
            const nt4 a = gather();
#if EVREP_NT_STORES
            __builtin_nontemporal_store(a, o4 + v0);
#else
            o4[v0] = a;
#endif
        }
    }
}

template <typename OutT, int CMAX, bool HOT, typename KeyAt, typename RecAt, typename RecStaged, typename PostHeads, typename Reduce>
__device__ inline void emit_core(uint32_t nrec, int nseg_pre, bool all_staged, KeyAt key_at, RecAt get, RecStaged get_staged,
                                 PostHeads post_heads, int key0, int npix, int C, OutT *__restrict__ dst, WaveLds<OutT, HOT> &w,
                                 const OutT *bg, Reduce reduce) {
    const int lane = threadIdx.x;
    const int PP = w.partpx;
    constexpr int V = 16 / (int)sizeof(OutT);
    const bool sparse_ok = EVREP_SPARSE_EMIT && (C % V) == 0 && (reinterpret_cast<uintptr_t>(dst) & 15u) == 0 &&
                           (bg == nullptr || bg == w.bg);
    const int sparse_cap = min(kWave, PP);
    const bool sparse_late = sparse_ok && nrec > (uint32_t)sparse_cap && nrec <= 2u * kWave && all_staged;
    bool sparse = sparse_ok && nrec <= (uint32_t)sparse_cap;
    if (!sparse && !sparse_late && (!bg || nrec == 0)) tile_fill(w.tile, min(PP, npix), C, bg);
    const uint32_t empty4 = (uint32_t)PP * 0x01010101u;
    if ((sparse || sparse_late) && !bg && lane * V < EVREP_MAX_CHANNELS)
        reinterpret_cast<float4 *>(w.bg)[lane] = make_float4(0.f, 0.f, 0.f, 0.f);
    if (nrec == 0) {
        if (sparse) {
            unsigned char *map = reinterpret_cast<unsigned char *>(w.segs);
            for (int i = lane; i * 4 < npix; i += kWave) reinterpret_cast<uint32_t *>(map)[i] = empty4;
            wave_phase();
            w.pace();
            sparse_store(w.tile, map, npix, C, dst);
            return;
        }
        wave_phase();
        w.pace();
        for (int part = 0; part * PP < npix; ++part)
            tile_store(w.tile, min(PP, npix - part * PP) * C, dst + (size_t)part * PP * C);
        return;
    }
    int nseg = 0;
    if (nseg_pre >= 0) {
        nseg = nseg_pre;
    } else {
        int carry = INT32_MIN;
// ... 696 lines not shown
#pragma unroll
        for (int c = 0; c < D::kMaxC; ++c) vals[c] = (OutT)rr[c];
    };

    constexpr bool kSplitHot = MdesIsErgo12<D>::value && sizeof(OutT) < 8;
    constexpr bool kSplit = MdesIsErgo12<D>::value && (kSplitHot ? HOT : !HOT);
    constexpr bool kSplitDefer = kSplitHot && !HOT;
    ChunkGeom g;
    UnitRecs u;
    bool esc = false;
    if constexpr (kSplit) {
        uint32_t *words = reinterpret_cast<uint32_t *>(w.tile);
        MdesWindows smw;
        int32_t stmin = 0;
        uint64_t pmask = 0ull;
        auto sbegin = [&]() -> bool {
            const WindowMeta m = meta_finish(bv, off, b0, mraw);
            stmin = __builtin_amdgcn_readfirstlane(m.tmin);
            smw = mdes_windows(n_win);
            const uint32_t neg_flags = (uint32_t)__builtin_amdgcn_readfirstlane((int)m.neg_flags);
            const uint32_t oob_flags = (uint32_t)__builtin_amdgcn_readfirstlane((int)m.oob_flags);
            uint32_t a0 = 0, a1 = 0, a2 = 0;
#pragma unroll
            for (int c = 0; c < D::kMaxC; ++c) {
                const int wi = D::win(P, c), f = D::func(P, c);
                uint32_t cls = 7u;
                int field = 0;
                if (f == EVREP_F_TIMESTAMP_POS || f == EVREP_F_COUNT_POS) { cls = 4u; field = 1; }
                if (f == EVREP_F_TIMESTAMP_NEG || f == EVREP_F_COUNT_NEG) {
                    const bool has_neg = (neg_flags >> wi) & 1u;
                    cls = has_neg ? 1u : 2u;
                    field = has_neg ? 2 : 3;
                }
                if (n_win <= 0 || ((oob_flags >> (7 * field + wi)) & 1u)) cls = 0u;
                a0 |= (cls & 1u) << c; a1 |= ((cls >> 1) & 1u) << c; a2 |= ((cls >> 2) & 1u) << c;
            }
            pmask = (uint64_t)a0 | ((uint64_t)a1 << 16) | ((uint64_t)a2 << 32);
            return true;
        };
        auto sf = [&](uint32_t px, const Rec8 &q, uint2 &e, const uint2 &) -> bool {
            const int rank = (int)(q.y >> 11);
            const uint32_t p2 = (q.y >> 9) & 3u;
            if (p2 == 3u) { esc = true; return false; }
            const int p = (int)p2 - 1;
            const uint32_t tt = (uint32_t)((int64_t)(int32_t)q.x - (int64_t)stmin);
            uint32_t *wd = words + px * (uint32_t)kErgoSplitWords;
            uint32_t chans = ergo_chans_of(0);
            chans |= rank < smw.hi[1] ? ergo_chans_of(1) : (rank < smw.hi[2] ? ergo_chans_of(2) : (rank < smw.hi[3] ? ergo_chans_of(3) : 0u));
            chans |= rank >= smw.lo[4] ? ergo_chans_of(4) : 0u;
            chans |= rank >= smw.lo[5] ? ergo_chans_of(5) : 0u;
            chans |= rank >= smw.lo[6] ? ergo_chans_of(6) : 0u;
            const uint32_t hits = chans & (uint32_t)(pmask >> (16u * p2));
            auto hit = [&](int c) -> bool { return (hits >> c) & 1u; };
            const uint32_t pinc = p > 0 ? 1u : 0x10000u;
            if (hit(0)) { if (p != 0) atomicAdd(wd + 0, pinc); else atomicAdd(wd + 1, 1u); }
            if (hit(3) && p != 0) atomicAdd(wd + 2, pinc);
            if (hit(5)) atomicAdd(wd + 1, 0x10000u);
            const bool h8 = hit(8), h9 = hit(9), h10 = hit(10), h6 = hit(6), h1 = hit(1);
            const uint32_t bits = hits & ((1u << 2) | (1u << 4) | (1u << 7) | (1u << 11) | (1u << 8) | (1u << 9) | (1u << 10));
            if (bits) atomicOr(wd + 3, bits);
            if (h6) atomicAdd(wd + 3, 0x10000u);
            if (h8) atomicMax(wd + 4, tt);
            if (h9) atomicMax(wd + 5, tt);
            if (h10) atomicMax(wd + 6, tt);
            e = make_uint2(tt, px);
            return h6 || h1;
        };
        auto sdone = [&]() -> bool { return !__any(esc); };
        auto smerge = [](const uint32_t *m, uint32_t *gw) {
            if (m[0]) atomicAdd(gw + 0, m[0]);
            if (m[1]) atomicAdd(gw + 1, m[1]);
            if (m[2]) atomicAdd(gw + 2, m[2]);
            if (m[3] & 0xffffu) atomicOr(gw + 3, m[3] & 0xffffu);
            if (m[3] >> 16) atomicAdd(gw + 3, m[3] & 0xffff0000u);
            if (m[4]) atomicMax(gw + 4, m[4]);
            if (m[5]) atomicMax(gw + 5, m[5]);
            if (m[6]) atomicMax(gw + 6, m[6]);
        };
        u = unit_front<OutT, HOT, false, NoVisit>(bv, off, H, W, nchunk, uc, w, g, uid, part, NoVisit(), unit_split_merge<kSplitHot>(sbegin, sf, sdone, kErgoSplitWords, smerge));
    } else if constexpr (kSplitDefer) {
        auto never = []() -> bool { return false; };
        auto nof = [](uint32_t, const Rec8 &, uint2 &, const uint2 &) -> bool { return false; };
        auto sp = unit_split<true>(never, nof, never, kErgoSplitWords,
                                   (uint32_t)mraw.q2.x | ((uc.xflags & (kXfHandOverWhole | kXfHandOverMonsters | kXfCoopErgo12)) ? 0u : kStEscaped),
                                   (uc.xflags & kXfHandOverWhole) ? 0u : kHotSubMin);
        sp.coop_min = (uc.xflags & kXfCoopErgo12) ? kErgoCoopMin : 0u;
        u = unit_front<OutT, HOT, false, NoVisit>(bv, off, H, W, nchunk, uc, w, g, uid, part, NoVisit(), sp);
    } else {
        u = unit_front(bv, off, H, W, nchunk, uc, w, g, uid, part);
    }
    if (u.deferred) return;
    w.mark(0);
    OutT *dst = out + (((size_t)g.b * H + g.row) * (size_t)W + g.c0) * C;
    setup();
    w.mark(1);

    if constexpr (kSplit) {
        if (u.part == -5) {
            const int lane = threadIdx.x;
            const uint32_t nk = u.pst;
            const uint32_t *words = reinterpret_cast<const uint32_t *>(w.tile);
            volatile uint32_t *cnt = reinterpret_cast<volatile uint32_t *>(w.segs);
            scan_pixel_counters(reinterpret_cast<uint32_t *>(w.segs), u.npixu);
            const uint32_t room = (uint32_t)(reinterpret_cast<const unsigned char *>(w.segs) - reinterpret_cast<const unsigned char *>(w.tile));
            const uint32_t lcap = split_list_cap(room, u.pen);
            const uint32_t nrec = u.ce - u.cs;
            const bool sliced = u.sub > 0;
            const bool big = nk > lcap || sliced;
            const uint2 *list = reinterpret_cast<const uint2 *>(reinterpret_cast<const unsigned char *>(w.tile) + u.pen);
            double *placed = reinterpret_cast<double *>(reinterpret_cast<unsigned char *>(w.tile) + u.pen);
            const uint2 *glist = reinterpret_cast<const uint2 *>(bv.spill + u.cs);
            double *gplaced = sliced ? bv.placed_pool + u.cs : reinterpret_cast<double *>(bv.spill + u.cs) + nrec;
            uint32_t spre = 0xffffffffu, soff = 0u;
            const unsigned long long *sublists = reinterpret_cast<const unsigned long long *>(
                reinterpret_cast<const unsigned char *>(bv.spill + u.cs) + ((kHotSubHdrBytes + 4u * split_gwpp(kErgoSplitWords) * (uint32_t)u.npixu + 15u) & ~15u));
            if (sliced) {
                const uint32_t *hdr = reinterpret_cast<const uint32_t *>(bv.spill + u.cs);
                uint32_t tot = 0;
                if (lane < u.sub) tot = __hip_atomic_load(hdr + 1 + lane, __ATOMIC_RELAXED, __HIP_MEMORY_SCOPE_AGENT);
                const uint32_t incl = wave_incl_scan(tot);
                if (lane < u.sub) { spre = incl - tot; soff = (uint32_t)lane * hot_sub_quota(nrec, (uint32_t)u.sub); }
            }
            auto sub_at = [&](uint32_t j) -> uint2 {
                uint32_t at = (uint32_t)__builtin_amdgcn_readlane((int)soff, 0) + j;
                for (int k = 1; k < u.sub; ++k) {
                    const uint32_t pk = (uint32_t)__builtin_amdgcn_readlane((int)spre, k);
                    const uint32_t ok = (uint32_t)__builtin_amdgcn_readlane((int)soff, k);
                    if (j >= pk) at = ok + (j - pk);
                }
                const unsigned long long v = __hip_atomic_load(sublists + at, __ATOMIC_RELAXED, __HIP_MEMORY_SCOPE_AGENT);
                return make_uint2((uint32_t)v, (uint32_t)(v >> 32));
            };
            const int nbits = 32 - __builtin_clz((unsigned)u.npixu - 1u);
            auto place = [&](const uint2 &e, bool valid, double *dstp) {
                const uint32_t px = valid ? e.y : 0u;
                uint32_t rk; bool last;
                wave_match(px, nbits, valid, lane, rk, last);
                uint32_t pos = 0;
                if (valid) { pos = cnt[px] + rk; dstp[pos] = (double)e.x / interval; }
                __builtin_amdgcn_wave_barrier();
                if (valid && last) cnt[px] = pos + 1;
                __builtin_amdgcn_wave_barrier();
            };
            if (!big) {
                uint2 ek[kSplitBatches];
#pragma unroll
                for (int i = 0; i < kSplitBatches; ++i) {
                    const uint32_t j = (uint32_t)(i * kWave + lane);
                    ek[i] = make_uint2(0u, 0u);
                    if (j < nk) ek[i] = list[j];
                }
                wave_phase();
#pragma unroll
                for (int i = 0; i < kSplitBatches; ++i)
                    if ((uint32_t)(i * kWave) < nk) place(ek[i], (uint32_t)(i * kWave + lane) < nk, placed);
            } else {
                __builtin_amdgcn_fence(__ATOMIC_RELEASE, "workgroup");
                __builtin_amdgcn_wave_barrier();
                __builtin_amdgcn_fence(__ATOMIC_ACQUIRE, "workgroup");
                for (uint32_t j0 = 0; j0 < nk; j0 += 4 * kWave) {
                    uint2 ek[4];
#pragma unroll
                    for (int i = 0; i < 4; ++i) {
                        const uint32_t j = j0 + (uint32_t)(i * kWave + lane);
                        ek[i] = make_uint2(0u, 0u);
                        if (j < nk) {
                            if (sliced) ek[i] = sub_at(j);
// ... 688 lines not shown
#endif

template <int CM, bool HOT = false>
__global__ __launch_bounds__(kWave, HOT ? 4 : EVREP_ES_WAVES) void k_event_stack(BinView bv,
                                                      const int64_t *__restrict__ off, int H, int W, int nchunk, UnitCfg uc,
                                                      int S, int premap, float scale, float *__restrict__ out) {
    extern __shared__ __align__(16) unsigned char smem[];
    run_units<HOT>(bv, [&](int uid, int part) {
        WaveLds<float, HOT> w(smem, S, (uc.span + uc.merge) * kChunkPx, uc.stage, uc.partpx);
        w.arm(uc.hold);
        ChunkGeom g;
        const UnitRecs u = unit_front<float, HOT, true>(bv, off, H, W, nchunk, uc, w, g, uid, part);
        if (u.deferred) return;
        float *dst = out + (((size_t)g.b * H + g.row) * (size_t)W + g.c0) * S;
        const int64_t n_win = off[g.b + 1] - off[g.b];
        int offk[CM];
        {
            int cur = (int)n_win, o = 0;
#pragma unroll
            for (int k = 0; k < CM; ++k) { offk[k] = o; cur /= 2; o += cur; }
        }
        auto reduce = [&](uint32_t jb, uint32_t je, auto get, float(&vals)[CM]) {
            const Rec e = get(je - 1);
            int p = e.w;
            if (premap == 1) p = (p + 1) >> 1;
            const float v = (float)(int8_t)(premap == 2 ? p : 2 * p - 1) * scale;
#pragma unroll
            for (int l = 0; l < CM; ++l) vals[l] = (e.y >= offk[l]) ? v : 0.0f;
        };
        emit_chunk<float, CM, HOT, false>(u, g.row * W + g.c0, g.npix, S, dst, w, (const float *)nullptr, reduce);
    });
}

constexpr int kMaxSlices = 8;

__device__ inline double exp_neg_range(double x) {
    if (x < -746.0) return 0.0;
    const double n = rint(x * 1.4426950408889634);
    double r = fma(n, -6.93147180369123816490e-01, x);
    r = fma(n, -1.90821492927058770002e-10, r);
    double p = 2.08767569878680989792e-09;
    p = fma(p, r, 2.50521083854417187751e-08);
    p = fma(p, r, 2.75573192239858906526e-07);
    p = fma(p, r, 2.75573192239858906526e-06);
    p = fma(p, r, 2.48015873015873015873e-05);
    p = fma(p, r, 1.98412698412698412698e-04);
    p = fma(p, r, 1.38888888888888888889e-03);
    p = fma(p, r, 8.33333333333333333333e-03);
    p = fma(p, r, 4.16666666666666666667e-02);
    p = fma(p, r, 1.66666666666666666667e-01);
    p = fma(p, r, 5.00000000000000000000e-01);
    p = fma(p, r, 1.0);
    p = fma(p, r, 1.0);
    return ldexp(p, (int)n);
}

__device__ inline double div_tau(double d, double tau, double inv_tau) {
    const double q = d * inv_tau;
    return fma(fma(-q, tau, d), inv_tau, q);
}

struct TsCuts {
    int32_t idx[kMaxSlices];
    int32_t tcut[kMaxSlices];
    int32_t live[kMaxSlices];
    int32_t tref;
    int32_t direct;
    int32_t pad[6];
    double bg[2 * kMaxSlices];
    double fac[kMaxSlices];
    double tcutf[kMaxSlices];
};
static_assert(sizeof(TsCuts) == kTsCutsBytes, "TsCuts");

#ifdef EVREP_TU_BUILDERS
static __global__ void k_ts_cuts(BinView bv, const int4 *__restrict__ ev, const int64_t *__restrict__ off, int S,
                          const int32_t *__restrict__ indices, double tau, double scale, TsCuts *__restrict__ cuts,
                          const double *__restrict__ tf) {
    const int b = blockIdx.x, s = threadIdx.x;
    __shared__ int sidx[kMaxSlices];
    const int64_t beg = off[b];
    const int64_t n = off[b + 1] - beg;
    int32_t wtmin = INT32_MAX, wtmax = INT32_MIN;
    if (bv.fused) {
        const int nb = min((int)(((uint32_t)n + (1u << bv.chunk_shift) - 1u) >> bv.chunk_shift), bv.nblk);
        for (int k = s; k < nb; k += kWave) {
            const int2 q = *reinterpret_cast<const int2 *>(bv.stats + (size_t)b * bv.nblk + k);
            wtmin = min(wtmin, q.x);
            wtmax = max(wtmax, q.y);
        }
        wtmin = wave_min(wtmin);
        wtmax = wave_max(wtmax);
    } else if (n > 0) {
        wtmin = bv.meta[b].tmin;
        wtmax = bv.meta[b].tmax;
    }
    if (s < S) {
        int idx = 0, tc = 0;
        if (n > 0) {
            if (indices) {
                idx = indices[b * S + s];
            } else {
                const int32_t t0 = ev[beg].z, tl = ev[beg + n - 1].z;
                const double den = (double)(int32_t)(tl - t0);
                const double target = (double)(s + 1);
                int64_t lo = 0, hi = n;
                while (lo < hi) {
                    const int64_t mid = lo + (hi - lo) / 2;
                    const double q = (double)(int32_t)(ev[beg + mid].z - t0) / den;
                    const double tn = q * (double)S;
                    if (tn < target) lo = mid + 1; else hi = mid;
                }
                idx = (int)lo;
            }
            tc = (idx >= 0 && idx < n) ? ev[beg + idx].z : 0;
        }
        sidx[s] = idx;
        cuts[b].idx[s] = idx;
        cuts[b].tcut[s] = tc;
        cuts[b].tcutf[s] = (tf && n > 0 && idx >= 0 && idx < n) ? tf[beg + idx] : (double)tc;
    }
    __syncthreads();
    if (s == 0) {
        bool alive = n > 0;
        for (int k = 0; k < kMaxSlices; ++k) {
            if (k < S) {
                if (k > 0 && sidx[k] <= sidx[k - 1]) alive = false;
                if (sidx[k] < 0 || sidx[k] >= n) alive = false;
                cuts[b].live[k] = alive ? 1 : 0;
            } else {
                cuts[b].live[k] = 0;
                cuts[b].idx[k] = 0;
                cuts[b].tcut[k] = 0;
            }
            double v = 0.0;
            if (k < S && alive) v = exp_neg_range((-(tau * 3.0 + 1.0) - cuts[b].tcutf[k]) / tau) * scale;
            cuts[b].bg[2 * k] = v;
            cuts[b].bg[2 * k + 1] = v;
        }
        int tref = 0;
        for (int k = 0; k < kMaxSlices; ++k) if (k < S && cuts[b].live[k]) tref = cuts[b].tcut[k];
        int direct = 0, nlive = 0;
        for (int k = 0; k < kMaxSlices; ++k) {
            double f = 0.0;
            if (k < S && cuts[b].live[k]) {
                const double x = ((double)tref - (double)cuts[b].tcut[k]) / tau;
                if (x > 600.0 || x < -600.0) direct = 1;
                f = exp(x) * scale;
                ++nlive;
            }
            cuts[b].fac[k] = f;
        }
        if (nlive > 0 && (((double)wtmin - (double)tref) / tau < -700.0 || ((double)wtmax - (double)tref) / tau > 700.0)) direct = 1;
        cuts[b].tref = tref;
        cuts[b].direct = tf ? 1 : direct;
    }
}
#endif

#ifndef EVREP_TS_WAVES
#define EVREP_TS_WAVES 4
#endif
template <typename OutT, int CM, bool FACT, bool HOT = false>
__global__ __launch_bounds__(kWave, HOT ? 4 : EVREP_TS_WAVES) void k_time_surface(BinView bv, const int64_t *__restrict__ off,
                                                       const TsCuts *__restrict__ cuts, int H, int W, int nchunk, UnitCfg uc,
                                                       int S, double tau, int premap, double scale, const double *__restrict__ tf,
                                                       OutT *__restrict__ out) {
    extern __shared__ __align__(16) unsigned char smem[];
    run_units<HOT>(bv, [&](int uid, int part) {
        const int C = 2 * S;
        WaveLds<OutT, HOT> w(smem, C, (uc.span + uc.merge) * kChunkPx, uc.stage);
        w.arm(uc.hold);
        int chunk0;
        const TsCuts *cp = cuts + unit_geom(H, W, nchunk, uc, chunk0, uid).b;
        struct { int idx[(CM / 2)], tcut[(CM / 2)], live[(CM / 2)]; } cu;
#pragma unroll
// ... 681 lines not shown
                double acc = 0.0;
                for (uint32_t j = jb; j < je; ++j) {
                    const Rec ec = get(j);
                    double p = (double)ec.w;
                    if (mode == 1 && ec.w == 0) p = -1.0;
                    const double bpos = __hiloint2double(ec.z, ec.y);
                    if (!(bpos > (mode == 1 ? -0.0 : -1.0) && bpos < 1.0e9) && !(bpos == 0.0)) continue;
                    const int bi = (int)bpos;
                    const int blim = bi + pass;
                    if (blim < bins) {
                        double wgt;
                        if (mode == 2) wgt = 1.0;
                        else if (mode == 0) wgt = 1.0 - fabs((double)blim - bpos);
                        else { const double dts = bpos - (double)bi; wgt = pass ? dts : 1.0 - dts; }
                        const double wp = wgt * p;
                        if (blim != cur) {
                            if (cur >= 0) scr[cur] = acc;
                            acc = scr[blim];
                            cur = blim;
                        }
                        acc = acc + wp;
                    }
                }
                if (cur >= 0) scr[cur] = acc;
            }
#pragma unroll
            for (int c = 0; c < CM; ++c) vals[c] = c < bins ? scr[c] : 0.0;
            if (scale != 1.0) {
#pragma unroll
                for (int c = 0; c < CM; ++c) vals[c] = vals[c] * scale;
            }
        };
        emit_chunk<double, CM, HOT>(u, digest, g.row * W + g.c0, g.npix, bins, dst, w, (const double *)nullptr, reduce);
    });
}

__host__ __device__ inline size_t voxel_stream_lds_bytes(int bins, int npixa, int rb) {
    return align16((size_t)npixa * bins * 8) + (size_t)npixa * 4 + (size_t)(64 * rb + 128) * 4 + align16((size_t)npixa);
}
#ifndef EVREP_VS_WAVES
#define EVREP_VS_WAVES 6
#endif
template <int RB>
__global__ __launch_bounds__(kWave, EVREP_VS_WAVES) void k_voxel_stream(const int4 *__restrict__ ev, BinView bv, const int64_t *__restrict__ off,
                                                int H, int W, int nchunk, UnitCfg uc, int bins, int mode, double scale,
                                                const int64_t *__restrict__ t_range, const double *__restrict__ tnorm,
                                                double *__restrict__ out) {
    extern __shared__ __align__(16) unsigned char smem[];
    const int lane = threadIdx.x;
    const int uid = chunk_unit((int)(gridDim.x * gridDim.y * gridDim.z));
#ifdef EVREP_TIMING
    const long long vs_t0 = (long long)wall_clock64();
#endif
    int chunk, nch;
    const ChunkGeom g = unit_geom(H, W, nchunk, uc, chunk, nch, uid);
    const int b = g.b;
    const int64_t beg = off[b];
    const int64_t n_win = off[b + 1] - beg;
    int tz0 = 0, tz1 = 0;
    if (n_win > 0) { tz0 = ev[beg].z; tz1 = ev[beg + n_win - 1].z; }
    const int NK = H * nchunk, klo = g.row * nchunk + chunk;
    const StreamRuns R = stream_runs(bv, b, n_win, NK, klo, klo + nch);
    const int npixa = (uc.span + uc.merge) * kChunkPx;
    double *acc = reinterpret_cast<double *>(smem);
    uint32_t *tag = reinterpret_cast<uint32_t *>(smem + align16((size_t)npixa * bins * 8));
    uint32_t *head = tag + npixa;
    uint32_t *srcs = head + 64 * RB;
    unsigned char *touched = reinterpret_cast<unsigned char *>(srcs + 128);
    const int ncell = g.npix * bins;
    {
        uint4 *z = reinterpret_cast<uint4 *>(acc);
        for (int v = lane; v * 2 < ncell; v += kWave) z[v] = make_uint4(0u, 0u, 0u, 0u);
        uint4 *t4 = reinterpret_cast<uint4 *>(tag);
        for (int v = lane; v * 4 < npixa; v += kWave) t4[v] = make_uint4(~0u, ~0u, ~0u, ~0u);
        if (scale != 1.0) { uint4 *c4 = reinterpret_cast<uint4 *>(touched); for (int v = lane; v * 16 < npixa; v += kWave) c4[v] = make_uint4(0u, 0u, 0u, 0u); }
    }
    const int nb = R.nb;
    const uint32_t nrec = nb > 0 ? R.nrec : 0u;
    const bool wide = nb > kWave;
    {
        const uint32_t avg = (uint32_t)((uint64_t)n_win / (uint64_t)(H * nchunk));
        if (nrec > (uint32_t)uc.stage && nrec > 3u * avg) {
            if (!defer_items(bv, uid, (uint32_t)kHotWhole, 1u) && lane == 0)
                atomicOr(&bv.stats_rw[(size_t)b * bv.nblk].status, EVREP_ST_HOT_OVERFLOW);
            return;
        }
    }
    double *dst = out + (((size_t)b * H + g.row) * (size_t)W + g.c0) * bins;
    double t0 = 0.0, den = 1.0;
    if (n_win > 0) { t0 = (double)tz0; den = (double)tz1 - t0; }
    if (t_range) { t0 = (double)t_range[2 * b]; den = (double)(t_range[2 * b + 1] - t_range[2 * b]); }
    const double *tw = tnorm ? tnorm + beg : nullptr;
    const int4 *evw = ev + beg;
    const int c0 = g.c0;
    const Rec8 *__restrict__ s8 = reinterpret_cast<const Rec8 *>(bv.sorted);
    auto bin_of = [&](const Rec8 &q) -> double {
        if (tw) return (double)(bins - 1) * tw[q.y >> 11];
        const int t = (int)q.x;
        if (mode == 2) {
            const int64_t num = (int64_t)(bins - 1) * ((int64_t)t - (int64_t)t0);
            return (double)num / (den == 0.0 ? 1.0 : den);
        }
        if (mode == 0) {
            const double tn = ((double)t - t0) / den;
            return (double)(bins - 1) * tn;
        }
        const double num = (double)bins * ((double)t - t0);
        return num / den;
    };
    auto pol_of = [&](const Rec8 &q) -> int {
        const uint32_t p2 = (q.y >> 9) & 3u;
        int p = (int)p2 - 1;
        if (p2 == 3u) p = evw[q.y >> 11].w;
        return p;
    };
    auto px_of = [&](const Rec8 &q) -> uint32_t { return ((q.y & 511u) - (uint32_t)c0) & 511u; };
    const double lowlim = mode == 1 ? -0.0 : -1.0;
    auto apply = [&](int pass, bool have, uint32_t px, double bpos, int p) {
        double pd = (double)p;
        if (mode == 1 && p == 0) pd = -1.0;
        bool ok = have && ((bpos > lowlim && bpos < 1.0e9) || bpos == 0.0);
        const int bi = ok ? (int)bpos : 0;
        const int blim = bi + pass;
        ok = ok && blim < bins;
        double wgt;
        if (mode == 2) wgt = 1.0;
        else if (mode == 0) wgt = 1.0 - fabs((double)blim - bpos);
        else { const double dts = bpos - (double)bi; wgt = pass ? dts : 1.0 - dts; }
        const double wp = wgt * pd;
        double *cell = acc + (px * (uint32_t)bins + (uint32_t)blim);
        bool pend = ok;
        while (__any(pend)) {
            if (pend) atomicMin(&tag[px], (uint32_t)lane);
            wave_phase();
            const bool win = pend && tag[px] == (uint32_t)lane;
            wave_phase();
            if (win) {
                *cell = *cell + wp;
                tag[px] = ~0u;
                pend = false;
            }
            wave_phase();
        }
    };
    if (nrec != 0u) {
        const uint32_t src0 = (uint32_t)beg + ((uint32_t)lane << bv.chunk_shift) + R.a0 - R.pre0;
        const uint32_t src1 = (uint32_t)beg + ((uint32_t)(kWave + lane) << bv.chunk_shift) + R.a1 - R.pre1;
        const int npass = mode == 2 ? 1 : 2;
        if (nrec <= (uint32_t)(64 * RB)) {
#pragma unroll
            for (int i = 0; i < RB; ++i) head[lane + 64 * i] = 0u;
            srcs[lane] = src0;
            if (wide) srcs[kWave + lane] = src1;
            wave_phase();
            if (R.len0 > 0u && R.pre0 < (uint32_t)(64 * RB)) head[R.pre0] = (uint32_t)lane;
            if (wide && R.len1 > 0u && R.pre1 < (uint32_t)(64 * RB)) head[R.pre1] = (uint32_t)(kWave + lane);
            wave_phase();
            Rec8 q[RB];
            uint32_t carry = 0u;
#pragma unroll
            for (int i = 0; i < RB; ++i) {
                q[i] = make_uint2(0u, 0u);
                if ((uint32_t)(64 * i) < nrec) {
                    const uint32_t k = max(carry, wave_incl_max_scan(head[lane + 64 * i]));
                    carry = (uint32_t)__builtin_amdgcn_readlane((int)k, 63);
                    const uint32_t j = (uint32_t)(64 * i + lane);
                    if (j < nrec) q[i] = s8[srcs[k] + j];
// ... 826 lines not shown
```

### event_representation_study_amd/csrc/evrep_capi.hip

```cpp
#define EVREP_TU_CORE 1
#include "evrep_capi_shared.h"

#include "evrep_bin.hip"

using namespace evrep;

static thread_local char g_last_error[256] = "";

namespace evrep_host {
char *last_error_buf() { return g_last_error; }
int hip_check(hipError_t e, const char *what) {
    if (e == hipSuccess) return EVREP_OK;
    snprintf(g_last_error, sizeof(g_last_error), "%s: %s", what, hipGetErrorString(e));
    return EVREP_EHIP;
}
int column_sort_keys(const evrep_plan *plan, const int32_t *events, const int64_t *offsets, void *workspace, hipStream_t stream) {
    const int NK = plan->H * plan->nchunk;
    k_col_sort_runs<<<dim3((NK + kCsWaves - 1) / kCsWaves, plan->B), kCsWaves * kWave,
                                      (size_t)kCsWaves * col_sort_wave_words(kChunkPx) * 4, stream>>>(
        reinterpret_cast<const int4 *>(events), CWS(Rec, off_sorted1), offsets, CWS(uint32_t, off_table), CWS(BlockStats, off_stats), plan->H, plan->W, plan->nblk,
        plan->nchunk, plan->nchunk, plan->chunk == 4096 ? 12 : 13, 1, WS(Rec, off_sorted2), WS(uint32_t, off_chunkoff),
        WS(WindowMeta, off_meta));
    LAUNCH_CHECK("k_col_sort_runs");
    return EVREP_OK;
}
}
using evrep_host::hip_check;
using evrep_host::column_sort_keys;

extern "C" {

int evrep_abi_version(void) { return EVREP_ABI_VERSION; }
const char *evrep_last_hip_error(void) { return g_last_error; }

int evrep_plan_init(evrep_plan *plan, int32_t B, int32_t H, int32_t W, int64_t total_events,
                    int64_t max_events_per_window) {
    return evrep_plan_init_ex(plan, B, H, W, total_events, max_events_per_window, 0u);
}

int evrep_plan_set_pacing(evrep_plan *plan, int32_t ticks) {
    if (!plan || plan->abi_version != EVREP_ABI_VERSION || ticks < -1 || ticks > 100000) return EVREP_EINVAL;
    plan->pacing = ticks;
    return EVREP_OK;
}

int evrep_plan_init_ex(evrep_plan *plan, int32_t B, int32_t H, int32_t W, int64_t total_events,
                       int64_t max_events_per_window, uint32_t flags) {
    const bool f_classic = flags & EVREP_PLAN_NO_KEY_PASS, f_three = flags & EVREP_PLAN_THREE_KERNEL;
    const bool f_force_ks = flags & EVREP_PLAN_FORCE_KEY_SORTED, f_big = flags & EVREP_PLAN_BIG_BLOCKS;
    if (!plan || B <= 0 || H <= 0 || W <= 0 || H > EVREP_MAX_DIM || W > EVREP_MAX_DIM) return EVREP_EINVAL;
    if (total_events < 0 || max_events_per_window < 0 || max_events_per_window > total_events) return EVREP_EINVAL;
    if (total_events >= (int64_t)1 << 31 || (int64_t)H * W >= (int64_t)1 << 30) return EVREP_EINVAL;
    if (B > 65535 || (int64_t)B * H * ((W + kChunkPx - 1) / kChunkPx) >= (int64_t)1 << 31) return EVREP_EINVAL;
    memset(plan, 0, sizeof(*plan));
    plan->abi_version = EVREP_ABI_VERSION;
    plan->B = B; plan->H = H; plan->W = W;
    plan->total_events = total_events;
    plan->max_events_per_window = max_events_per_window;
    plan->flags = (int32_t)flags;
    plan->pacing = -1;
    int64_t chunk = 2048;
    int64_t nblk = (max_events_per_window + chunk - 1) / chunk;
    if (nblk > 128) {
        chunk = ((max_events_per_window + 127) / 128 + 255) / 256 * 256;
        nblk = (max_events_per_window + chunk - 1) / chunk;
    }
    const bool two_kernel = max_events_per_window <= (int64_t)kCsMaxRuns * kBsChunk &&
                            block_rowsort_lds_bytes(H) + 1024 <= 160 * 1024 && !f_three;
    if (two_kernel) {
        chunk = kBsChunk;
        nblk = (max_events_per_window + chunk - 1) / chunk;
    }
    if (nblk < 1) nblk = 1;
    plan->chunk = (int32_t)chunk;
    plan->nblk = (int32_t)nblk;
    plan->nchunk = (W + kChunkPx - 1) / kChunkPx;
    plan->reserved = two_kernel ? 1 : 0;
    const int64_t NK = (int64_t)H * plan->nchunk;
    const bool key_sorted = two_kernel && max_events_per_window <= (int64_t)kCsMaxRuns * kBsChunk && NK < 65535 &&
                            block_keysort_lds_bytes((int)NK, 4096, kBsChunk) + 1024 <= 160 * 1024 &&
                            ((double)max_events_per_window <= kKeySortedMaxPerUnit * (double)NK || f_force_ks) && !f_classic && !f_three;
    const bool key_dense = !key_sorted && two_kernel && NK < 65535 &&
                           block_keysort_lds_bytes((int)NK, 4096, kBsChunk) + 1024 <= 160 * 1024 &&
                           !f_classic && !f_three;
    size_t table_words = (size_t)B * nblk * (H + 1);
    if (key_dense) {
        plan->reserved = 3;
        table_words = (size_t)B * nblk * ((size_t)NK + 1);
    }
    if (key_sorted) {
        plan->reserved = 2;
        if (max_events_per_window <= (int64_t)kBsChainBlocks * 4096 && !f_big) {
            chunk = 4096;
            nblk = (max_events_per_window + chunk - 1) / chunk;
            if (nblk < 1) nblk = 1;
            plan->chunk = (int32_t)chunk;
            plan->nblk = (int32_t)nblk;
        }
        table_words = (size_t)B * nblk * ((size_t)NK + 1);
    }
    size_t o = 0;
    plan->off_meta = o;    o += up256((size_t)B * sizeof(WindowMeta));
    plan->off_table = o;   o += up256(table_words * sizeof(uint32_t));
    plan->off_stats = o;   o += up256((size_t)B * nblk * sizeof(BlockStats));
    plan->off_rowoff = o;  o += up256((size_t)B * (H + 1) * sizeof(uint32_t));
    plan->off_chunkoff = o; o += up256((size_t)B * H * (plan->nchunk + 1) * sizeof(uint32_t));
    plan->off_sorted1 = o; o += up256((size_t)(total_events + 1) * sizeof(Rec));
    plan->off_sorted2 = o; o += up256((size_t)(total_events + 1) * sizeof(Rec));
    plan->off_cuts = o;    o += up256((size_t)B * kTsCutsBytes);
    plan->off_scratch = o; o += up256(4 * ((size_t)kHotHdrWords + (size_t)kHotLists * hot_sublist_cap(hot_items_total(total_events))));
    plan->workspace_bytes = o;
    return EVREP_OK;
}

size_t evrep_workspace_bytes(const evrep_plan *plan) { return plan ? plan->workspace_bytes : 0; }

int evrep_bin_events(const evrep_plan *plan, const int32_t *events, const int64_t *offsets, void *workspace,
                     void *stream_) {
    int rc = check_common(plan, events, offsets, workspace);
    if (rc) return rc;
    hipStream_t stream = as_stream(stream_);
    const int B = plan->B, H = plan->H, W = plan->W, chunk = plan->chunk, nblk = plan->nblk;
    const int4 *ev = reinterpret_cast<const int4 *>(events);
    WindowMeta *meta = WS(WindowMeta, off_meta);
    uint32_t *table = WS(uint32_t, off_table);
    uint32_t *row_off = WS(uint32_t, off_rowoff);
    Rec *s1 = WS(Rec, off_sorted1);
    Rec *s2 = WS(Rec, off_sorted2);
    BlockStats *stats = WS(BlockStats, off_stats);
    const unsigned xgrid = 8u * (unsigned)((B + 7) / 8) * (unsigned)nblk;
    uint32_t *hot = WS(uint32_t, off_scratch);
    if (plan->reserved != 2 && plan->reserved != 3) {
        int rc2 = hip_check(hipMemsetAsync(hot, 0, (size_t)kHotHdrWords * 4, stream), "hipMemsetAsync(hot list)");
        if (rc2) return rc2;
    }
    if (plan->reserved == 2 || plan->reserved == 3) {
        if ((chunk != kBsChunk && chunk != 4096) || nblk > kCsMaxRuns) return EVREP_EINVAL;
        const int NK = H * plan->nchunk;
        auto opt_in = [&](const void *fn, size_t lds) -> int {
            if (lds <= 64 * 1024) return EVREP_OK;
            return hip_check(hipFuncSetAttribute(fn, hipFuncAttributeMaxDynamicSharedMemorySize, 160 * 1024 - 1024),
                             "hipFuncSetAttribute(k_block_keysort)");
        };
        if (chunk == 4096) {
            const int cap = block_keysort_lds_bytes(NK, 4096, 4096) <= 52 * 1024 ? 4096
                            : (block_keysort_lds_bytes(NK, 2048, 4096) <= 52 * 1024 ? 2048 : 4096);
            if (int rc2 = opt_in(reinterpret_cast<const void *>(&k_block_keysort<1024, 4>), block_keysort_lds_bytes(NK, cap, 4096))) return rc2;
            k_block_keysort<1024, 4><<<xgrid, 1024, block_keysort_lds_bytes(NK, cap, 4096), stream>>>(
                ev, offsets, B, H, W, plan->nchunk, nblk, cap, table, stats, s1, reinterpret_cast<int64_t *>(row_off), hot);
        } else {
            const int cap = block_keysort_lds_bytes(NK, 4096, kBsChunk) <= 79 * 1024 ? 4096
                            : (block_keysort_lds_bytes(NK, kBsChunk, kBsChunk) + 1024 <= 160 * 1024 ? kBsChunk : 4096);
            if (int rc2 = opt_in(reinterpret_cast<const void *>(&k_block_keysort<1024>), block_keysort_lds_bytes(NK, cap, kBsChunk))) return rc2;
            k_block_keysort<1024><<<xgrid, kBsThreads, block_keysort_lds_bytes(NK, cap, kBsChunk), stream>>>(
                ev, offsets, B, H, W, plan->nchunk, nblk, cap, table, stats, s1, reinterpret_cast<int64_t *>(row_off), hot);
        }
        LAUNCH_CHECK("k_block_keysort");
        if (plan->reserved == 3) return column_sort_keys(plan, events, offsets, workspace, stream);
        return EVREP_OK;
    }
    if (plan->reserved == 1) {
        if (chunk != kBsChunk || nblk > kCsMaxRuns) return EVREP_EINVAL;
        const size_t lds = block_rowsort_lds_bytes(H);
        if (lds > 64 * 1024) {
            int rc2 = hip_check(hipFuncSetAttribute(reinterpret_cast<const void *>(&k_block_rowsort),
                                                    hipFuncAttributeMaxDynamicSharedMemorySize, 160 * 1024 - 1024),
                                "hipFuncSetAttribute(k_block_rowsort)");
            if (rc2) return rc2;
        }
        k_block_rowsort<<<xgrid, kBsThreads, lds, stream>>>(ev, offsets, B, H, W, nblk, table, stats, s1);
        LAUNCH_CHECK("k_block_rowsort");
        if (BS_DEBUG & 15) return EVREP_OK;
        constexpr int rows_per_wg = kCsRowWaves;
        k_col_sort_runs<<<dim3((H + rows_per_wg - 1) / rows_per_wg, B), kCsRowWaves * kWave, (size_t)kCsRowWaves * col_sort_wave_words(W) * 4, stream>>>(
            ev, s1, offsets, table, stats, H, W, nblk, plan->nchunk, 1, 13, 0, s2, WS(uint32_t, off_chunkoff), meta);
        LAUNCH_CHECK("k_col_sort_runs");
        return EVREP_OK;
    }
    k_row_hist<<<xgrid, kBinThreads, (size_t)H * 4, stream>>>(ev, offsets, B, H, W, chunk, nblk, table, stats);
    LAUNCH_CHECK("k_row_hist");
    if (chunk <= kStageRecs && fused_scatter_lds_bytes(H) <= 65536 && !(plan->flags & EVREP_PLAN_NO_FUSED_SCATTER)) {
        k_row_scatter_fused<<<xgrid, kBinThreads, fused_scatter_lds_bytes(H), stream>>>(ev, offsets, B, H, W, chunk, nblk, table,
                                                                                     stats, row_off, meta, s1);
        LAUNCH_CHECK("k_row_scatter_fused");
    } else {
        k_row_scan<<<B, kBinThreads, (size_t)H * 4, stream>>>(offsets, H, chunk, nblk, table, row_off, stats, meta);
        LAUNCH_CHECK("k_row_scan");
        k_row_scatter<<<xgrid, kBinThreads, (size_t)kBinWaves * H * 4, stream>>>(ev, offsets, B, H, W, chunk, nblk, table, row_off, s1);
        LAUNCH_CHECK("k_row_scatter");
    }
    k_col_sort<<<dim3(H, B), kWave, (size_t)W * 4, stream>>>(s1, row_off, H, W, plan->nchunk, s2, WS(uint32_t, off_chunkoff));
    LAUNCH_CHECK("k_col_sort");
    return EVREP_OK;
}

static int read_meta_field(const evrep_plan *plan, const void *workspace, size_t field_off, size_t field_bytes,
                           void *dst, hipStream_t stream) {
    const char *meta = static_cast<const char *>(workspace) + plan->off_meta;
    if (plan->reserved == 2) {
        char *ws = const_cast<char *>(static_cast<const char *>(workspace));
        k_window_meta<<<plan->B, kWave, 0, stream>>>(reinterpret_cast<const int64_t *>(ws + plan->off_rowoff),
                                                     reinterpret_cast<const BlockStats *>(ws + plan->off_stats), plan->nblk, plan->chunk == 4096 ? 12 : 13,
                                                     reinterpret_cast<WindowMeta *>(ws + plan->off_meta));
        int rc0 = hip_check(hipGetLastError(), "k_window_meta");
        if (rc0) return rc0;
    }
    int rc = hip_check(hipMemcpy2DAsync(dst, field_bytes, meta + field_off, sizeof(WindowMeta), field_bytes,
                                        (size_t)plan->B, hipMemcpyDeviceToHost, stream), "hipMemcpy2DAsync(meta)");
    if (rc) return rc;
    return hip_check(hipStreamSynchronize(stream), "hipStreamSynchronize");
}

int evrep_copy_window_meta_async(const evrep_plan *plan, const void *workspace, void *meta_out, void *stream_) {
    if (!plan || plan->abi_version != EVREP_ABI_VERSION || !workspace || !meta_out) return EVREP_EINVAL;
    hipStream_t stream = as_stream(stream_);
    const char *meta = static_cast<const char *>(workspace) + plan->off_meta;
    if (plan->reserved == 2) {
        char *ws = const_cast<char *>(static_cast<const char *>(workspace));
        k_window_meta<<<plan->B, kWave, 0, stream>>>(reinterpret_cast<const int64_t *>(ws + plan->off_rowoff),
                                                     reinterpret_cast<const BlockStats *>(ws + plan->off_stats), plan->nblk, plan->chunk == 4096 ? 12 : 13,
                                                     reinterpret_cast<WindowMeta *>(ws + plan->off_meta));
        LAUNCH_CHECK("k_window_meta");
    }
    return hip_check(hipMemcpyAsync(meta_out, meta, (size_t)plan->B * sizeof(WindowMeta), hipMemcpyDeviceToHost, stream),
                     "hipMemcpyAsync(meta)");
}

int evrep_read_status(const evrep_plan *plan, const void *workspace, uint32_t *status, void *stream_) {
    if (!plan || !workspace || !status) return EVREP_EINVAL;
    return read_meta_field(plan, workspace, offsetof(WindowMeta, status), sizeof(uint32_t), status,
                           as_stream(stream_));
}

int evrep_read_bbox(const evrep_plan *plan, const void *workspace, int32_t *bbox, void *stream_) {
    if (!plan || !workspace || !bbox) return EVREP_EINVAL;
    static_assert(offsetof(WindowMeta, ymax) - offsetof(WindowMeta, xmin) == 12, "xmin, xmax, ymin, ymax are contiguous");
    int rc = read_meta_field(plan, workspace, offsetof(WindowMeta, xmin), 4 * sizeof(int32_t), bbox,
                             as_stream(stream_));
    if (rc) return rc;
    for (int b = 0; b < plan->B; ++b) {
        const int32_t t = bbox[4 * b + 1];
        bbox[4 * b + 1] = bbox[4 * b + 2];
        bbox[4 * b + 2] = t;
    }
    return EVREP_OK;
}

}
```

### event_representation_study_amd/csrc/evrep_capi_builders.h

```cpp
#pragma once
#include <type_traits>
#include "evrep_capi_shared.h"
#include "evrep_bin.hip"
#include "evrep_builders.hip"

using namespace evrep;

template <int N> using Cap = std::integral_constant<int, N>;
template <typename T> struct Type { using type = T; };

static inline bool ks_pass(const evrep_plan *plan) { return plan->reserved == 2 && plan->nblk <= kBsMaxBlocks; }

static inline BinView bin_view(const evrep_plan *plan, const int32_t *events, void *workspace, bool runs = false) {
    BinView bv;
    bv.ev = reinterpret_cast<const int4 *>(events);
    bv.fused = (runs ? plan->reserved == 2 : ks_pass(plan)) ? 1 : 0;
    bv.sorted = bv.fused ? CWS(Rec, off_sorted1) : CWS(Rec, off_sorted2);
    bv.chunk_off = CWS(uint32_t, off_chunkoff);
    bv.table = CWS(uint32_t, off_table);
    bv.stats = CWS(BlockStats, off_stats);
    bv.meta = CWS(WindowMeta, off_meta);
    bv.spill = WS(Rec, off_sorted2);
    bv.nblk = plan->nblk;
    bv.hot = WS(uint32_t, off_scratch);
    bv.hot_cap = hot_items_total(plan->total_events);
    bv.stats_rw = WS(BlockStats, off_stats);
    bv.placed_pool = reinterpret_cast<double *>(static_cast<char *>(workspace) + plan->off_sorted1 + align16((size_t)plan->total_events * 8));
    bv.chunk_shift = plan->chunk == 4096 ? 12 : 13;
#ifdef EVREP_TIMING
    bv.dbg = reinterpret_cast<unsigned long long *>(static_cast<char *>(workspace) + plan->off_sorted1 +
                                                    (bv.fused ? up256((size_t)plan->total_events * 8) : 0));
    bv.dbg_wave = nullptr;
#endif
    return bv;
}

static inline int ensure_column_sorted(const evrep_plan *plan, const int32_t *events, const int64_t *offsets, void *workspace, hipStream_t stream) {
    if (plan->reserved != 2) return EVREP_OK;
    return evrep_host::column_sort_keys(plan, events, offsets, workspace, stream);
}
static inline int ensure_pixel_stream(const evrep_plan *plan, const int32_t *events, const int64_t *offsets, void *workspace, hipStream_t stream) {
    if (plan->reserved != 2 || ks_pass(plan)) return EVREP_OK;
    return evrep_host::column_sort_keys(plan, events, offsets, workspace, stream);
}

static inline double records_per_unit(const evrep_plan *plan) { return (double)plan->max_events_per_window / ((double)plan->H * plan->nchunk); }
constexpr double kSparseMaxPerUnit = 30.0;
constexpr double kStage128MinPerUnit = 28.0;
constexpr double kHandOverMaxPerUnit = 90.0;
constexpr double kSweepMainMinPerUnit = 150.0;
constexpr double kTsStreamMinPerUnit = 28.0;
constexpr double kErgoStreamMinPerUnitF32 = 28.0, kErgoStreamMinPerUnitF64 = 100.0;

constexpr int kStreamMaxW = 512 * 8;
static inline bool stream_allowed(const evrep_plan *plan, uint32_t ordered_bit) {
    return plan->reserved == 2 && !(plan->flags & ordered_bit) && plan->W <= kStreamMaxW;
}

static inline void unit_cfg_geometry(UnitCfg &uc, const evrep_plan *plan) {
    uc.nunit = units_per_row(plan->nchunk, uc.span, uc.merge);
    fastdiv_make((uint32_t)uc.nunit, uc.nunit_m, uc.nunit_sh);
    fastdiv_make((uint32_t)plan->H, uc.h_m, uc.h_sh);
}
static inline UnitCfg unit_cfg(const evrep_plan *plan, size_t pixel_bytes, int extra_chunks = 0, bool wide_part = false, bool deep_stage = true) {
    UnitCfg uc;
    const double per_unit = records_per_unit(plan);
    uc.span = (pixel_bytes * kChunkPx > 8192 || plan->nchunk < 2) ? 1 : (per_unit <= kSparseMaxPerUnit ? 2 : 1);
    uc.stage = (deep_stage && !ks_pass(plan) && per_unit > kDeepStageMinPerUnit) ? 256
               : ((uc.span + extra_chunks > 1 || per_unit > kStage128MinPerUnit || (plan->flags & EVREP_PLAN_X_STAGE128)) ? 128 : 64);
    if ((plan->flags & EVREP_PLAN_X_STAGE64) && ks_pass(plan) && uc.span == 1) uc.stage = 64;
    uc.partpx = (wide_part && per_unit <= kSparseMaxPerUnit) ? 2 * kPartPx : kPartPx;
    uc.hold = plan->pacing > 0 ? plan->pacing : 0;
    const int tail = plan->W % kChunkPx;
    uc.merge = (extra_chunks == 0 && tail != 0 && tail <= kChunkPx / 2 && plan->nchunk >= 2 && (plan->flags & EVREP_PLAN_X_TAIL_MERGE)) ? 1 : 0;
    uc.xflags = ((uc.span == 1 && (per_unit <= kHandOverMaxPerUnit || (plan->flags & EVREP_PLAN_X_HANDOVER_DENSE))) ||
                 ((plan->flags & EVREP_PLAN_X_HANDOVER2) && uc.span > 1)) ? kXfHandOverWhole : 0;
    if (uc.span > 1 && !(uc.xflags & kXfHandOverWhole) && !(plan->flags & EVREP_PLAN_X_NO_MONSTER_HANDOVER)) uc.xflags |= kXfHandOverMonsters;
    unit_cfg_geometry(uc, plan);
    return uc;
}
static inline UnitCfg stream_cfg(const evrep_plan *plan, UnitCfg uc) {
    uc.span = 1; uc.merge = 0; uc.hold = 0;
    unit_cfg_geometry(uc, plan);
    return uc;
}
static inline dim3 unit_grid(const evrep_plan *plan, const UnitCfg &uc) { return dim3(uc.nunit, plan->H, plan->B); }
static inline int sweep_main_stage(int stage, int words, size_t tile_bytes) {
    const size_t need = (size_t)kChunkPx * words * 4 + 1024, have = align16(tile_bytes) + align16((size_t)EVREP_MAX_CHANNELS * 4);
    const int st = (int)((need > have ? need - have : 0) + 15) / 16;
    return stage < st ? (st + 63) & ~63 : stage;
}
static inline int hot_sweep_stage(size_t words_bytes, size_t list_bytes, size_t tile_bytes) {
    const size_t have = align16(tile_bytes) + align16((size_t)EVREP_MAX_CHANNELS * 8), need = words_bytes + list_bytes;
    const int st = need > have ? (int)((need - have + 15) / 16) : 0;
    const int r = (st + 63) & ~63;
    return r > kHotStage ? r : kHotStage;
}
static inline UnitCfg hot_cfg(UnitCfg uc) { uc.stage = kHotStage; uc.hold = 0; return uc; }

static inline int auto_hold(const evrep_plan *plan, const void *kernel, size_t lds_bytes, int span, size_t pixel_bytes, int merge) {
    if (records_per_unit(plan) > kSparseMaxPerUnit) return 0;
    int waves = 0;
    if (hipOccupancyMaxActiveBlocksPerMultiprocessor(&waves, kernel, kWave, lds_bytes) != hipSuccess || waves <= 0) {
        (void)hipGetLastError();
        return 0;
    }
    const int nunit = units_per_row(plan->nchunk, span, merge);
    const double unit_bytes = (double)plan->W * (double)pixel_bytes / (double)nunit;
    const double ticks = 690.0 * ((double)waves * unit_bytes) / (19.0 * 12288.0);
// ... 3 lines not shown
```

### event_representation_study_amd/csrc/evrep_capi_builders.hip

```cpp
#define EVREP_TU_BUILDERS 1
#include <cstdlib>
#include "evrep_capi_builders.h"
#include "evrep_render.hip"

static inline size_t stream_pad(const evrep_plan *plan, size_t bytes) { return records_per_unit(plan) <= kSparseMaxPerUnit ? bytes : 0; }

extern "C" {

int evrep_event_stack(const evrep_plan *plan, const int32_t *events, const int64_t *offsets, void *workspace,
                      int32_t stack_size, int32_t premap, float scale, float *out, void *stream_) {
    int rc = check_common(plan, events, offsets, workspace);
    if (rc) return rc;
    if (stack_size <= 0 || stack_size > EVREP_MAX_CHANNELS || !out) return EVREP_EINVAL;
    hipStream_t stream = as_stream(stream_);
    if (stream_allowed(plan, EVREP_PLAN_X_ESTACK_ORDERED)) {
        const UnitCfg us = stream_cfg(plan, unit_cfg(plan, (size_t)stack_size * 4, 0, true, false));
        constexpr int kRB = 4;
        auto launch = [&](auto cm) {
            k_event_stack_stream<decltype(cm)::value, kRB><<<unit_grid(plan, us), kWave, event_stack_stream_lds_bytes(stack_size, kChunkPx, kRB) + stream_pad(plan, 1024), stream>>>(
                bin_view(plan, events, workspace, true), offsets, plan->H, plan->W, plan->nchunk, us, stack_size, premap, scale, out);
        };
        if (stack_size <= 8) launch(Cap<8>()); else if (stack_size <= 12) launch(Cap<12>()); else launch(Cap<16>());
        LAUNCH_CHECK("k_event_stack_stream");
        return EVREP_OK;
// ... 251 lines not shown
    auto launch = [&](auto cm) {
        constexpr int CM = decltype(cm)::value;
        if (sweep_main) {
            k_polstats<CM, false, true><<<unit_grid(plan, uc), kWave, chunk_lds_bytes(C, 4, seg, uc.stage, uc.partpx), stream>>>(
                bin_view(plan, events, workspace), offsets, tnorm, P, plan->H, plan->W, plan->nchunk, uc, out);
            return;
        }
        k_polstats<CM><<<unit_grid(plan, uc), kWave, chunk_lds_bytes(C, 4, seg, uc.stage, uc.partpx), stream>>>(
            bin_view(plan, events, workspace), offsets, tnorm, P, plan->H, plan->W, plan->nchunk, uc, out);
        if (ks_pass(plan)) k_polstats<CM, true><<<kHotGrid, kWave, chunk_lds_bytes(C, 4, seg, hc.stage, uc.partpx), stream>>>(
            bin_view(plan, events, workspace), offsets, tnorm, P, plan->H, plan->W, plan->nchunk, hc, out);
    };
    if (C <= 8) launch(Cap<8>()); else launch(Cap<16>());
    LAUNCH_CHECK("k_polstats");
    return EVREP_OK;
}

int evrep_est_voxel(const evrep_plan *plan, const int32_t *events, const int64_t *offsets, void *workspace,
                    const float *tnorm, int32_t C, const double *segments, int32_t nseg, const uint32_t *buckets,
                    int32_t nbucket, double lo, double hi, float *out, void *stream_) {
    int rc = check_common(plan, events, offsets, workspace);
    if (rc) return rc;
    if (C < 2 || C > kEstMaxBins || !segments || nseg < 1 || !buckets || nbucket < 1 || !(hi > lo) || !out) return EVREP_EINVAL;
    if (plan->total_events > 0 && !tnorm) return EVREP_EINVAL;
    EstParams P;
    memset(&P, 0, sizeof(P));
    P.C = C; P.nseg = nseg; P.nbucket = nbucket;
    P.lo = lo; P.inv_width = (double)nbucket / (hi - lo);
    for (int i = 0; i < C; ++i) P.shift[i] = (float)((double)i / (double)(C - 1));
    hipStream_t stream = as_stream(stream_);
    if (int rc3 = ensure_pixel_stream(plan, events, offsets, workspace, stream)) return rc3;
    const UnitCfg uc = unit_cfg(plan, (size_t)2 * C * 4);
    const int seg = (uc.span + uc.merge) * kChunkPx;
    k_est<false><<<unit_grid(plan, uc), kWave, chunk_lds_bytes(2 * C, 4, seg, uc.stage), stream>>>(
        bin_view(plan, events, workspace), offsets, tnorm, segments, buckets, P, plan->H, plan->W,
        plan->nchunk, uc, out);
    if (ks_pass(plan)) k_est<true><<<kHotGrid, kWave, chunk_lds_bytes(2 * C, 4, seg, kHotStage), stream>>>(
        bin_view(plan, events, workspace), offsets, tnorm, segments, buckets, P, plan->H, plan->W,
        plan->nchunk, hot_cfg(uc), out);
    LAUNCH_CHECK("k_est");
    return EVREP_OK;
}

int evrep_resize_taps(const void *in, int32_t in_dtype, int32_t B, int32_t H, int32_t W, int32_t C, int32_t Ho, int32_t Wo,
                      int32_t T, const int32_t *ystart, const int32_t *ycount, const double *ywt, const int32_t *xstart,
                      const int32_t *xcount, const double *xwt, double scale, int32_t out_dtype, void *out, void *stream_) {
    if (!in || !out || !ystart || !ycount || !ywt || !xstart || !xcount || !xwt) return EVREP_EINVAL;
    if (B <= 0 || B > 65535 || H <= 0 || W <= 0 || C <= 0 || Ho <= 0 || Wo <= 0 || T <= 0) return EVREP_EINVAL;
    if (!is_float_dtype(in_dtype) || !is_float_dtype(out_dtype)) return EVREP_EINVAL;
    hipStream_t stream = as_stream(stream_);
    ResizeTaps tp;
    tp.ystart = ystart; tp.ycount = ycount; tp.xstart = xstart; tp.xcount = xcount; tp.ywt = ywt; tp.xwt = xwt; tp.T = T;
    const size_t per = (size_t)Ho * Wo * C;
    const dim3 grid((unsigned)((per + kThreads - 1) / kThreads), (unsigned)B);
#define RESIZE_LAUNCH(IN, OUT) \
    k_resize_taps<IN, OUT><<<grid, kThreads, 0, stream>>>(static_cast<const IN *>(in), H, W, C, tp, Ho, Wo, scale, static_cast<OUT *>(out))
    if (in_dtype == EVREP_F64) { if (out_dtype == EVREP_F64) RESIZE_LAUNCH(double, double); else RESIZE_LAUNCH(double, float); }
    else { if (out_dtype == EVREP_F64) RESIZE_LAUNCH(float, double); else RESIZE_LAUNCH(float, float); }
#undef RESIZE_LAUNCH
    LAUNCH_CHECK("k_resize_taps");
    return EVREP_OK;
}

int evrep_probe_store(void *out, size_t bytes, void *stream_) {
    if (bad_ptr(out, 16)) return EVREP_EINVAL;
    const size_t tiles = bytes / 12288;
    if (tiles == 0 || tiles > 0x7fffffffu) return EVREP_EINVAL;
    k_store_probe<<<(unsigned)tiles, kWave, 8320, as_stream(stream_)>>>(static_cast<float *>(out), (int)tiles);
    LAUNCH_CHECK("k_store_probe");
    return EVREP_OK;
}

int evrep_render_state(const evrep_plan *plan, const int32_t *events, const int64_t *offsets, void *workspace,
                       uint8_t *state, int32_t *net, float *surface, double tau, void *stream_) {
    int rc = check_common(plan, events, offsets, workspace);
    if (rc) return rc;
    if (bad_ptr(state, 4) || misaligned(net, 4) || misaligned(surface, 4)) return EVREP_EINVAL;
    if (surface && !(tau > 0.0)) return EVREP_EINVAL;
    if ((int64_t)plan->H * plan->W * 4 >= (int64_t)1 << 31) return EVREP_EINVAL;
    hipStream_t stream = as_stream(stream_);
    const UnitCfg us = stream_cfg(plan, unit_cfg(plan, 4, 0, true, false));
    constexpr int kRB = 4;
    k_render_state<kRB><<<unit_grid(plan, us), kWave, render_state_lds_bytes(kChunkPx, kRB), stream>>>(
        bin_view(plan, events, workspace, true), offsets, plan->H, plan->W, plan->nchunk, us, tau, WS(WindowMeta, off_meta), state, net, surface);
    LAUNCH_CHECK("k_render_state");
    return EVREP_OK;
}

int evrep_render_compose(const uint8_t *state, const int32_t *net, const float *surface, const double *lut,
                         const uint8_t *canvas, int32_t canvas_is_batched, int32_t B, int32_t H, int32_t W, int32_t type,
                         uint32_t flags, void *out, void *stream_) {
    if (B <= 0 || B > 65535 || H <= 0 || W <= 0 || (int64_t)H * W * 4 >= (int64_t)1 << 31) return EVREP_EINVAL;
    if (type < EVREP_RENDER_RED_BLUE_OVERLAP || type > EVREP_RENDER_EVENT_FRAME || (flags & ~EVREP_RENDER_JITTER)) return EVREP_EINVAL;
    const bool colour = type <= EVREP_RENDER_BLACK_WHITE_NO_OVERLAP, jitter = flags & EVREP_RENDER_JITTER;
    if (jitter && !colour) return EVREP_EINVAL;
    if (bad_ptr(state, 4) || bad_ptr(out, 16) || misaligned(net, 4) || misaligned(surface, 4) || misaligned(lut, 8)) return EVREP_EINVAL;
    if (type == EVREP_RENDER_EVENT_FRAME && !net) return EVREP_EINVAL;
    if (type == EVREP_RENDER_TIME_SURFACE && (!surface || !lut)) return EVREP_EINVAL;
    if (canvas_is_batched != 0 && canvas_is_batched != 1) return EVREP_EINVAL;
    const size_t npx = (size_t)H * W;
    if (canvas && colour) {
        const uintptr_t c0 = reinterpret_cast<uintptr_t>(canvas), c1 = c0 + (canvas_is_batched ? (size_t)B : 1) * npx * 3;
        const uintptr_t o0 = reinterpret_cast<uintptr_t>(out), o1 = o0 + (size_t)B * npx * 3;
        if (c0 < o1 && o0 < c1) return EVREP_EINVAL;
    }
    hipStream_t stream = as_stream(stream_);
    const dim3 grid((unsigned)(((npx + 3) / 4 + 1 + kRcThreads - 1) / kRcThreads), (unsigned)B);
#define RENDER_LAUNCH(TYPE, JIT, LDS) \
    k_render_compose<TYPE, JIT><<<grid, kRcThreads, LDS, stream>>>(state, net, surface, lut, canvas, canvas_is_batched, B, H, W, out)
    switch (type) {
    case EVREP_RENDER_RED_BLUE_OVERLAP: if (jitter) RENDER_LAUNCH(EVREP_RENDER_RED_BLUE_OVERLAP, true, 0); else RENDER_LAUNCH(EVREP_RENDER_RED_BLUE_OVERLAP, false, 0); break;
    case EVREP_RENDER_RED_BLUE_NO_OVERLAP: if (jitter) RENDER_LAUNCH(EVREP_RENDER_RED_BLUE_NO_OVERLAP, true, 0); else RENDER_LAUNCH(EVREP_RENDER_RED_BLUE_NO_OVERLAP, false, 0); break;
    case EVREP_RENDER_BLACK_WHITE_NO_OVERLAP: if (jitter) RENDER_LAUNCH(EVREP_RENDER_BLACK_WHITE_NO_OVERLAP, true, 0); else RENDER_LAUNCH(EVREP_RENDER_BLACK_WHITE_NO_OVERLAP, false, 0); break;
    case EVREP_RENDER_TIME_SURFACE: RENDER_LAUNCH(EVREP_RENDER_TIME_SURFACE, false, 1024 * sizeof(double)); break;
    default: RENDER_LAUNCH(EVREP_RENDER_EVENT_FRAME, false, 0); break;
    }
#undef RENDER_LAUNCH
    LAUNCH_CHECK("k_render_compose");
    return EVREP_OK;
}

}
```

### event_representation_study_amd/csrc/evrep_capi_shared.h

```cpp
#pragma once
#include <stddef.h>
#include <stdio.h>
#include <stdlib.h>
#include <string.h>

#include "evrep_common.h"

#define EVREP_HIDDEN __attribute__((visibility("hidden")))

namespace evrep_host {
EVREP_HIDDEN char *last_error_buf();
EVREP_HIDDEN int hip_check(hipError_t e, const char *what);
EVREP_HIDDEN int column_sort_keys(const evrep_plan *plan, const int32_t *events, const int64_t *offsets, void *workspace, hipStream_t stream);
}

#define LAUNCH_CHECK(what)                                              \
    do {                                                                \
        int rc_ = evrep_host::hip_check(hipGetLastError(), what);       \
        if (rc_ != EVREP_OK) return rc_;                                \
    } while (0)

static inline size_t up256(size_t v) { return (v + 255) & ~(size_t)255; }

static inline bool misaligned(const void *p, uintptr_t a) { return (reinterpret_cast<uintptr_t>(p) & (a - 1)) != 0; }
static inline bool bad_ptr(const void *p, uintptr_t a) { return !p || misaligned(p, a); }
static inline bool is_float_dtype(int32_t dtype) { return dtype == EVREP_F64 || dtype == EVREP_F32; }
static inline hipStream_t as_stream(void *stream) { return static_cast<hipStream_t>(stream); }

static inline int check_common(const evrep_plan *plan, const void *events, const void *offsets, const void *ws) {
    if (!plan || plan->abi_version != EVREP_ABI_VERSION || !offsets || !ws) return EVREP_EINVAL;
    if (plan->total_events > 0 && !events) return EVREP_EINVAL;
    if (misaligned(events, 16) || misaligned(ws, 256)) return EVREP_EINVAL;
    return EVREP_OK;
}

struct Carver {
    char *base;
    size_t off = 0;
    explicit Carver(void *scratch) : base(static_cast<char *>(scratch)) {}
    template <typename T>
    T *take(size_t bytes) {
        T *part = reinterpret_cast<T *>(base ? base + off : nullptr);
        off += up256(bytes);
        return part;
    }
};

#define WS(type, field) reinterpret_cast<type *>(static_cast<char *>(workspace) + plan->field)
#define CWS(type, field) reinterpret_cast<const type *>(static_cast<const char *>(workspace) + plan->field)

constexpr double kKeySortedMaxPerUnit = 220.0;
constexpr double kDeepStageMinPerUnit = 110.0;
```

### event_representation_study_amd/csrc/evrep_common.h

```cpp
#pragma once
#include <hip/hip_runtime.h>
#include <stdint.h>

#include "evrep.h"

namespace evrep {

constexpr int kThreads = 256;
constexpr int kWaves = 4;
constexpr int kWave = 64;
constexpr int kChunkPx = 128;

#ifndef EVREP_HOT_STAGE
#define EVREP_HOT_STAGE 256
#endif
#ifndef EVREP_HOT_GRID
#define EVREP_HOT_GRID 4096
#endif
constexpr size_t kTsCutsBytes = 384;
constexpr int kHotStage = EVREP_HOT_STAGE;
constexpr int kHotGrid = EVREP_HOT_GRID;
constexpr int kHotParts = 8;
constexpr int kHotCodes = 64;
constexpr int kHotLists = 64;
constexpr int kHotWhole = kHotCodes - 1;
constexpr int kHotCoop = kHotCodes - 2;
constexpr int kHotSub0 = 40, kHotSubMax = 16;
#ifdef EVREP_TIMING
constexpr uint32_t kHotSubMin = 0x7fffffffu, kHotSubRecs = 1024u;
#else
constexpr uint32_t kHotSubMin = 4096u, kHotSubRecs = 1024u;
#endif
__host__ __device__ inline uint32_t hot_sub_count(uint32_t nrec) { const uint32_t s = nrec / kHotSubRecs; return s > (uint32_t)kHotSubMax ? (uint32_t)kHotSubMax : s; }
__host__ __device__ inline uint32_t hot_sub_quota(uint32_t nrec, uint32_t S) { return (((nrec + S - 1u) / S) + 63u) & ~63u; }
constexpr uint32_t kHotSubHdrBytes = 128u;
constexpr int kHotSplitStage = 576;
constexpr uint32_t kStEscaped = 1u << 16;
constexpr int kHotHdrWords = 2 * kHotLists * 16;
static_assert(kHotGrid % kHotLists == 0, "every sublist is worked off by kHotGrid / kHotLists workgroups");
__host__ __device__ inline uint32_t hot_sublist_cap(uint32_t cap_total) { return 2u * (cap_total / (kHotLists / 4) + 64u); }
__host__ __device__ inline uint32_t hot_items_total(int64_t total_events) { return (uint32_t)(kHotParts * ((size_t)total_events / 65 + 1)); }

struct WindowMeta {
    int32_t tmin, tmax;
    int32_t xmin, xmax, ymin, ymax;
    uint32_t neg_flags;
    uint32_t oob_flags;
    uint32_t status;
    int32_t n_valid;
    int32_t pad[6];
};
static_assert(sizeof(WindowMeta) == 64, "WindowMeta is one 64-byte line");

using Rec = int4;

using Rec8 = uint2;
__device__ inline Rec8 rec8_pack(int col, int rank, int t, int p) {
    const uint32_t p2 = (uint32_t)(p + 1) <= 2u ? (uint32_t)(p + 1) : 3u;
    return make_uint2((uint32_t)t, ((uint32_t)col & 511u) | (p2 << 9) | ((uint32_t)rank << 11));
}
__device__ inline Rec rec8_unpack(const Rec8 q, int row_base, int base_col, const int4 *__restrict__ ev_win) {
    const uint32_t w = q.y;
    const int col = base_col + (int)(((w & 511u) - (uint32_t)base_col) & 511u);
    const int rank = (int)(w >> 11);
    const uint32_t p2 = (w >> 9) & 3u;
    int p = (int)p2 - 1;
    if (p2 == 3u) p = ev_win[rank].w;
    return make_int4(row_base + col, rank, (int)q.x, p);
}

struct MdesWindows {
    int32_t lo[8], hi[8];
};

__host__ __device__ inline MdesWindows mdes_windows(int64_t n64) {
    MdesWindows w;
    int32_t n = (int32_t)n64;
    int32_t third = n / 3;
    w.lo[0] = 0; w.hi[0] = n;
    for (int i = 0; i < 3; ++i) { w.lo[1 + i] = i * third; w.hi[1 + i] = (i + 1) * third; }
    int32_t cur = n, start = 0;
    for (int i = 0; i < 3; ++i) { cur /= 2; start += cur; w.lo[4 + i] = start; w.hi[4 + i] = n; }
    w.lo[7] = 0; w.hi[7] = 0;
    return w;
}

__device__ inline uint32_t mdes_membership(const MdesWindows &w, int32_t r) {
    uint32_t m = 0;
#pragma unroll
    for (int i = 0; i < 7; ++i) m |= (r >= w.lo[i] && r < w.hi[i]) ? (1u << i) : 0u;
    return m;
}

using u32x4_t = __attribute__((ext_vector_type(4))) uint32_t;
__device__ inline u32x4_t gload16_raw(const void *p) {
    return *reinterpret_cast<const u32x4_t __attribute__((address_space(1))) *>(reinterpret_cast<uintptr_t>(p));
}
__device__ inline uint4 gload16_at(const void *base, uint32_t byte_off) {
    const u32x4_t v = *reinterpret_cast<const u32x4_t __attribute__((address_space(1))) *>(
        reinterpret_cast<const char __attribute__((address_space(1))) *>(reinterpret_cast<uintptr_t>(base)) + byte_off);
    return make_uint4(v.x, v.y, v.z, v.w);
}
__device__ inline double gload_f64(const double *p) {
    return *reinterpret_cast<const double __attribute__((address_space(1))) *>(reinterpret_cast<uintptr_t>(p));
}
__device__ inline void gstore16(void *p, uint4 v) {
    u32x4_t w; w.x = v.x; w.y = v.y; w.z = v.z; w.w = v.w;
    *reinterpret_cast<u32x4_t __attribute__((address_space(1))) *>(reinterpret_cast<uintptr_t>(p)) = w;
}
__device__ inline void gstore_f32(float *p, float v) {
    *reinterpret_cast<float __attribute__((address_space(1))) *>(reinterpret_cast<uintptr_t>(p)) = v;
}
__device__ inline void gstore_f64(double *p, double v) {
    *reinterpret_cast<double __attribute__((address_space(1))) *>(reinterpret_cast<uintptr_t>(p)) = v;
}
__device__ inline uint4 gload16(const void *p) { const u32x4_t v = gload16_raw(p); return make_uint4(v.x, v.y, v.z, v.w); }
__device__ inline float4 gload16f(const void *p) {
    const u32x4_t v = gload16_raw(p);
    return make_float4(__uint_as_float(v.x), __uint_as_float(v.y), __uint_as_float(v.z), __uint_as_float(v.w));
}

__device__ inline int lane_id() { return (int)__builtin_amdgcn_mbcnt_hi(~0u, __builtin_amdgcn_mbcnt_lo(~0u, 0u)); }

__device__ inline void wave_match(uint32_t key, int nbits, bool valid, int lane, uint32_t &rank, bool &last) {
    uint64_t mask = __ballot(valid);
    for (int b = 0; b < nbits; ++b) {
        bool bit = (key >> b) & 1u;
        uint64_t bal = __ballot(bit);
        mask &= bit ? bal : ~bal;
    }
    uint64_t below = (1ull << lane) - 1ull;
    rank = (uint32_t)__popcll(mask & below);
    last = (mask & ~below & ~(1ull << lane)) == 0ull;
}

// ... 39 lines not shown
```

### event_representation_study_amd/csrc/evrep_render.hip

```cpp
namespace evrep {

constexpr uint32_t kRsPos = 1u, kRsNeg = 2u, kRsLastPos = 4u, kRsFew = 8u;

__host__ __device__ inline size_t render_state_lds_bytes(int npixa, int rb) {
    return (size_t)npixa * 8 + (size_t)4 * npixa * 4 + (size_t)(64 * rb + 128) * 4 + align16((size_t)npixa);
}
template <int RB>
__global__ __launch_bounds__(kWave, 6) void k_render_state(BinView bv, const int64_t *__restrict__ off, int H, int W, int nchunk, UnitCfg uc,
                                                       double tau, WindowMeta *__restrict__ meta_out, unsigned char *__restrict__ state,
                                                       int32_t *__restrict__ net, float *__restrict__ surface) {
    extern __shared__ __align__(16) unsigned char smem[];
    const int lane = threadIdx.x;
    const int uid = chunk_unit((int)(gridDim.x * gridDim.y * gridDim.z));
    int chunk, nch;
    const ChunkGeom g = unit_geom(H, W, nchunk, uc, chunk, nch, uid);
    const int b = g.b;
    const int64_t beg = off[b];
    const int64_t n_win = off[b + 1] - beg;
    const int npixa = (uc.span + uc.merge) * kChunkPx;
    unsigned long long *last = reinterpret_cast<unsigned long long *>(smem);
    uint32_t *flg = reinterpret_cast<uint32_t *>(last + npixa);
    int *netl = reinterpret_cast<int *>(flg + npixa);
    float *acc = reinterpret_cast<float *>(netl + npixa);
    uint32_t *tag = reinterpret_cast<uint32_t *>(acc + npixa);
    uint32_t *head = tag + npixa;
    uint32_t *srcs = head + 64 * RB;
    unsigned char *sb = reinterpret_cast<unsigned char *>(srcs + 128);
    {
        uint4 *z = reinterpret_cast<uint4 *>(smem);
        for (int v = lane; v * 16 < npixa * 20; v += kWave) z[v] = make_uint4(0u, 0u, 0u, 0u);
        uint4 *t4 = reinterpret_cast<uint4 *>(tag);
        for (int v = lane; v * 4 < npixa; v += kWave) t4[v] = make_uint4(~0u, ~0u, ~0u, ~0u);
    }
    const int4 *evw = bv.ev + beg;
    int t_last = 0;
    if (surface && n_win > 0) t_last = evw[n_win - 1].z;
    const int c0 = g.c0;
    wave_phase();
    auto batch = [&](bool have, uint32_t px, uint32_t rank, int t, int p) {
        have = have && px < (uint32_t)g.npix;
        if (have) {
            const bool pos = p > 0;
            atomicMax(&last[px], ((unsigned long long)(rank + 1u) << 1) | (pos ? 1ull : 0ull));
            atomicOr(&flg[px], pos ? kRsPos : kRsNeg);
            if (net) atomicAdd(&netl[px], pos ? 1 : -1);
        }
        if (surface) {
            double v = 0.0;
            if (have) v = exp_neg_range((double)((int64_t)t - (int64_t)t_last) / tau);
            bool pend = have;
            while (__any(pend)) {
                if (pend) atomicMin(&tag[px], (uint32_t)lane);
                wave_phase();
                const bool win = pend && tag[px] == (uint32_t)lane;
                wave_phase();
                if (win) {
                    acc[px] = (float)((double)acc[px] + v);
                    tag[px] = ~0u;
                    pend = false;
                }
                wave_phase();
            }
        }
    };
    if (bv.fused) {
        stream_unit_records<RB>(bv, b, beg, n_win, H * nchunk, g.row * nchunk + chunk, g.row * nchunk + chunk + nch, head, srcs, StreamNoPre(),
            [&](bool have, const Rec8 &q, const uint2 &) {
                const uint32_t rank = q.y >> 11, p2 = (q.y >> 9) & 3u;
                int p = (int)p2 - 1;
                if (have && p2 == 3u) p = evw[rank].w;
                batch(have, ((q.y & 511u) - (uint32_t)c0) & 511u, rank, (int)q.x, p);
            });
    } else if (n_win > 0) {
        const uint32_t *co = bv.chunk_off + ((size_t)b * H + g.row) * (nchunk + 1);
        uint32_t cs = co[chunk], ce = co[chunk + nch];
        if ((int64_t)cs < beg || (int64_t)ce > beg + n_win) ce = cs;
        const int key0 = g.row * W + c0;
        for (uint32_t j = cs; j < ce; j += kWave) {
            const bool have = j + (uint32_t)lane < ce;
            Rec r = make_int4(key0, 0, 0, 0);
            if (have) r = bv.sorted[j + lane];
            batch(have, (uint32_t)(r.x - key0), (uint32_t)r.y, r.z, r.w);
        }
    }
    wave_phase();
    const uint32_t few = n_win <= 2 ? kRsFew : 0u;
    for (int px = lane; px < g.npix; px += kWave)
        sb[px] = (unsigned char)(flg[px] | (((uint32_t)last[px] & 1u) << 2) | few);
    wave_phase();
    const size_t o = ((size_t)b * H + g.row) * (size_t)W + (size_t)c0;
    {
        const int lead = min(g.npix, (int)((4u - (uint32_t)(o & 3u)) & 3u));
        const int nd = (g.npix - lead) >> 2, tail0 = lead + 4 * nd;
        unsigned char *dst = state + o;
        if (lane < lead) dst[lane] = sb[lane];
        if (lane < nd) {
            const unsigned char *s4 = sb + lead + 4 * lane;
            *reinterpret_cast<uint32_t *>(dst + lead + 4 * lane) = (uint32_t)s4[0] | ((uint32_t)s4[1] << 8) | ((uint32_t)s4[2] << 16) | ((uint32_t)s4[3] << 24);
        }
        if (tail0 + lane < g.npix) dst[tail0 + lane] = sb[tail0 + lane];
    }
    if (net) for (int px = lane; px < g.npix; px += kWave) net[o + px] = netl[px];
    if (surface) for (int px = lane; px < g.npix; px += kWave) surface[o + px] = acc[px];
    if (bv.fused && g.row == 0 && chunk == 0) {
        WindowMeta m = window_meta(bv, off, b);
        if (lane == 0) {
            m.status &= 0xffffu;
            if (n_win <= 0) m.status |= EVREP_ST_EMPTY;
            else if (m.tmin == m.tmax) m.status |= EVREP_ST_FLAT_TIME;
            for (int i = 0; i < 6; ++i) m.pad[i] = 0;
            meta_out[b] = m;
        }
    }
}

constexpr int kRcThreads = 256;
template <int TYPE, bool JIT>
__global__ __launch_bounds__(kRcThreads) void k_render_compose(const unsigned char *__restrict__ state, const int32_t *__restrict__ net,
                                                          const float *__restrict__ surface, const double *__restrict__ lut,
                                                          const unsigned char *__restrict__ canvas, int canvas_batched, int B, int H, int W,
                                                          void *__restrict__ out) {
    extern __shared__ __align__(16) unsigned char smem[];
    double *slut = reinterpret_cast<double *>(smem);
    if (TYPE == EVREP_RENDER_TIME_SURFACE) {
        for (int i = threadIdx.x; i < 1024; i += kRcThreads) slut[i] = lut[i];
        __syncthreads();
    }
    const int b = blockIdx.y;
    const uint32_t npx = (uint32_t)H * (uint32_t)W;
    const uint64_t wb = (uint64_t)b * npx, total = (uint64_t)B * npx;
    const uint64_t q = ((wb + 3u) >> 2) + (uint64_t)blockIdx.x * kRcThreads + threadIdx.x;
    const uint64_t g0 = q << 2;
    if (g0 >= wb + npx) return;
    const int nv = (int)min((uint64_t)4, total - g0);
    uint32_t sw = 0u;
    if (nv == 4) sw = *reinterpret_cast<const uint32_t *>(state + g0);
    else for (int k = 0; k < nv; ++k) sw |= (uint32_t)state[g0 + k] << (8 * k);
    uint32_t l = (uint32_t)(g0 - wb);
    int bb = b;
    uint32_t w3[3] = {0u, 0u, 0u};
#pragma unroll
    for (int k = 0; k < 4; ++k) {
        if (k < nv) {
            const uint64_t gp = g0 + (uint64_t)k;
            uint32_t s = (sw >> (8 * k)) & 255u;
            if (TYPE == EVREP_RENDER_TIME_SURFACE) {
                double4 c = make_double4(0.0, 0.0, 0.0, 0.0);
                const float f = surface[gp] * 256.0f;
                if (!(s & kRsFew) && f == f) {
                    const int idx = f >= 255.0f ? 255 : (f < 0.0f ? 0 : (int)f);
                    c = make_double4(slut[4 * idx], slut[4 * idx + 1], slut[4 * idx + 2], slut[4 * idx + 3]);
                }
                double2 *o2 = reinterpret_cast<double2 *>(out) + gp * 2u;
                o2[0] = make_double2(c.x, c.y);
                o2[1] = make_double2(c.z, c.w);
            } else {
                uint32_t r, gch, bl;
                if (TYPE == EVREP_RENDER_EVENT_FRAME) {
                    const int n = min(max(net[gp], -7), 7);
                    r = gch = bl = (uint32_t)min(max(20 * n + 128, 0), 255);
                } else {
                    if (JIT) {
                        const uint32_t y = l / (uint32_t)W, x = l - y * (uint32_t)W;
                        const unsigned char *sp = state + gp;
                        const uint32_t a = (y > 0u && x > 0u) ? sp[-(W + 1)] : 0u, c = x > 0u ? sp[-1] : 0u, d = y > 0u ? sp[-W] : 0u;
                        if (TYPE == EVREP_RENDER_RED_BLUE_OVERLAP) s |= a | c | d;
                        else s = (a & 3u) ? a : ((c & 3u) ? c : ((d & 3u) ? d : s));
                    }
                    if (!(s & 3u)) {
                        r = gch = bl = 255u;
                        if (canvas) {
                            const unsigned char *cp = canvas + ((canvas_batched ? (uint64_t)bb * npx : 0u) + l) * 3u;
                            r = cp[0]; gch = cp[1]; bl = cp[2];
                        }
                    } else if (TYPE == EVREP_RENDER_RED_BLUE_OVERLAP) {
                        r = (s & kRsNeg) ? 255u : 0u; gch = 0u; bl = (s & kRsPos) ? 255u : 0u;
                    } else if (TYPE == EVREP_RENDER_RED_BLUE_NO_OVERLAP) {
                        r = (s & kRsLastPos) ? 0u : 255u; gch = 0u; bl = (s & kRsLastPos) ? 255u : 0u;
                    } else {
                        r = gch = bl = (s & kRsLastPos) ? 255u : 0u;
                    }
                }
                const uint32_t vals[3] = {r, gch, bl};
#pragma unroll
                for (int ch = 0; ch < 3; ++ch) {
                    const int byte = 3 * k + ch;
                    w3[byte >> 2] |= vals[ch] << (8 * (byte & 3));
                }
            }
            if (++l == npx) { l = 0u; ++bb; }
        }
    }
    if (TYPE != EVREP_RENDER_TIME_SURFACE) {
        unsigned char *o1 = reinterpret_cast<unsigned char *>(out) + g0 * 3u;
        if (nv == 4) {
            uint32_t *o4 = reinterpret_cast<uint32_t *>(o1);
// ... 9 lines not shown
```

Baseline: 9.178 billion.

## Finalize window meta in keysort via last-block ticket instead of per-consumer reduction

The block keysort kernel now counts arriving blocks per window with a tagged atomic ticket. The last block merges all per-block stats and writes the final WindowMeta, which removes the separate k_window_meta launch. Downstream builders then read one precomputed meta record with a single load instead of reducing every block's stats themselves, and the render-state kernel no longer rewrites meta. In exchange, each block pays an atomic and a memory wait at the end, and correctness now rests on relaxed agent-scope atomics and on the ticket reset protocol working across calls.

```diff
diff --git a/event_representation_study_amd/csrc/evrep_bin.hip b/event_representation_study_amd/csrc/evrep_bin.hip
--- a/event_representation_study_amd/csrc/evrep_bin.hip
+++ b/event_representation_study_amd/csrc/evrep_bin.hip
@@ -53,6 +53,36 @@
     s.ymin = wave_min(s.ymin); s.ymax = wave_max(s.ymax);
     s.neg_flags = wave_or(s.neg_flags); s.oob_flags = wave_or(s.oob_flags); s.status = wave_or(s.status);
     s.n_valid = wave_sum(s.n_valid);
+}
+
+__device__ inline WindowMeta window_meta_of(const BlockStats &st, int64_t n_win) {
+    WindowMeta m;
+    m.tmin = st.tmin; m.tmax = st.tmax; m.xmin = st.xmin; m.xmax = st.xmax; m.ymin = st.ymin; m.ymax = st.ymax;
+    m.neg_flags = st.neg_flags; m.oob_flags = st.oob_flags; m.status = st.status & 0xffffu; m.n_valid = st.n_valid;
+    if (n_win <= 0) m.status |= EVREP_ST_EMPTY;
+    else if (st.tmin == st.tmax) m.status |= EVREP_ST_FLAT_TIME;
+    m.lib_status = st.status & 0xffff0000u;
+    for (int i = 0; i < 5; ++i) m.pad[i] = 0;
+    return m;
+}
+
+__device__ inline uint32_t ticket_arrive(unsigned long long *tw, unsigned long long seen, uint32_t nb) {
+    constexpr unsigned long long kRest = (unsigned long long)kTicketTag << 32;
+    if ((uint32_t)(seen >> 32) != kTicketTag || (uint32_t)seen >= nb) {
+        if (__hip_atomic_compare_exchange_strong(tw, &seen, kRest | 1ull, __ATOMIC_RELAXED, __ATOMIC_RELAXED, __HIP_MEMORY_SCOPE_AGENT))
+            return 1u;
+    }
+    return (uint32_t)__hip_atomic_fetch_add(tw, 1ull, __ATOMIC_RELAXED, __HIP_MEMORY_SCOPE_AGENT) + 1u;
+}
+__device__ inline void stats_load_agent(const BlockStats *rec, int (&q)[10]) {
+    const int *p = reinterpret_cast<const int *>(rec);
+#pragma unroll
+    for (int f = 0; f < 10; ++f) q[f] = __hip_atomic_load(p + f, __ATOMIC_RELAXED, __HIP_MEMORY_SCOPE_AGENT);
+}
+__device__ inline void stats_merge_words(BlockStats &a, const int (&q)[10]) {
+    a.tmin = min(a.tmin, q[0]); a.tmax = max(a.tmax, q[1]); a.xmin = min(a.xmin, q[2]); a.xmax = max(a.xmax, q[3]);
+    a.ymin = min(a.ymin, q[4]); a.ymax = max(a.ymax, q[5]);
+    a.neg_flags |= (uint32_t)q[6]; a.oob_flags |= (uint32_t)q[7]; a.status |= (uint32_t)q[8]; a.n_valid += q[9];
 }
 
 constexpr int kRegBatch = 8;
@@ -195,7 +225,8 @@
         m.neg_flags = t.neg_flags; m.oob_flags = t.oob_flags; m.status = t.status; m.n_valid = t.n_valid;
         if (n <= 0) m.status |= EVREP_ST_EMPTY;
         else if (t.tmin == t.tmax) m.status |= EVREP_ST_FLAT_TIME;
-        for (int i = 0; i < 6; ++i) m.pad[i] = 0;
+        m.lib_status = 0u;
+        for (int i = 0; i < 5; ++i) m.pad[i] = 0;
         meta[b] = m;
     }
 }
@@ -313,7 +344,8 @@
             WindowMeta m;
             m.tmin = INT32_MAX; m.tmax = INT32_MIN; m.xmin = INT32_MAX; m.xmax = INT32_MIN; m.ymin = INT32_MAX; m.ymax = INT32_MIN;
             m.neg_flags = 0; m.oob_flags = 0; m.status = EVREP_ST_EMPTY; m.n_valid = 0;
-            for (int i = 0; i < 6; ++i) m.pad[i] = 0;
+            m.lib_status = 0u;
+        for (int i = 0; i < 5; ++i) m.pad[i] = 0;
             meta[b] = m;
         }
         return;
@@ -393,7 +425,8 @@
         m.tmin = t.tmin; m.tmax = t.tmax; m.xmin = t.xmin; m.xmax = t.xmax; m.ymin = t.ymin; m.ymax = t.ymax;
         m.neg_flags = t.neg_flags; m.oob_flags = t.oob_flags; m.status = t.status; m.n_valid = t.n_valid;
         if (t.tmin == t.tmax) m.status |= EVREP_ST_FLAT_TIME;
-        for (int i = 0; i < 6; ++i) m.pad[i] = 0;
+        m.lib_status = 0u;
+        for (int i = 0; i < 5; ++i) m.pad[i] = 0;
         meta[b] = m;
     }
     __syncthreads();
@@ -729,15 +762,7 @@
             }
         }
         stats_wave_reduce(st);
-        if (lane == 0) {
-            WindowMeta m;
-            m.tmin = st.tmin; m.tmax = st.tmax; m.xmin = st.xmin; m.xmax = st.xmax; m.ymin = st.ymin; m.ymax = st.ymax;
-            m.neg_flags = st.neg_flags; m.oob_flags = st.oob_flags; m.status = st.status & 0xffffu; m.n_valid = st.n_valid;
-            if (n_win <= 0) m.status |= EVREP_ST_EMPTY;
-            else if (st.tmin == st.tmax) m.status |= EVREP_ST_FLAT_TIME;
-            for (int i = 0; i < 6; ++i) m.pad[i] = 0;
-            meta[b] = m;
-        }
+        if (lane == 0) meta[b] = window_meta_of(st, n_win);
     }
     constexpr uint32_t kSuper = 4 * kWave;
     const uint32_t rbeg = (uint32_t)beg + (uint32_t)wave_sum((int)(ta[0] + ta[1]));
@@ -883,8 +908,8 @@
 __global__ __launch_bounds__(TPB) __attribute__((amdgpu_waves_per_eu(TPB == 1024 ? KS_WAVES_1024 : KS_WAVES_512))) void k_block_keysort(const int4 *__restrict__ ev, const int64_t *__restrict__ off,
                                                              int B, int H, int W, int kpr, int nblk, int cap,
                                                              uint32_t *__restrict__ table, BlockStats *__restrict__ stats,
-                                                             Rec *__restrict__ sorted1, int64_t *__restrict__ nwin,
-                                                             uint32_t *__restrict__ hot) {
+                                                             Rec *__restrict__ sorted1, WindowMeta *__restrict__ meta,
+                                                             unsigned long long *__restrict__ ticket, uint32_t *__restrict__ hot) {
     extern __shared__ __align__(16) unsigned char smem_raw[];
     constexpr int kChunk = TPB * PL, kNW = TPB / kWave, kPerWave = PL * kWave;
     if (blockIdx.x == 0 && threadIdx.x < 128) hot[threadIdx.x * 16] = 0u;
@@ -895,15 +920,29 @@
     __shared__ int bstats[12];
     __shared__ uint32_t tmp[kNW];
     __shared__ uint32_t nhot_s;
+    __shared__ unsigned long long seen_s;
     int b, blk;
     if (!decode_window_block(B, nblk, b, blk)) return;
     const int64_t beg = off[b];
     const int64_t n = off[b + 1] - beg;
     const int64_t lo = (int64_t)blk * kChunk;
-    if (blk == 0 && threadIdx.x == 0) nwin[b] = n;
+    if (n <= 0) {
+        if (blk == 0 && threadIdx.x == 0) {
+            BlockStats none;
+            stats_identity(none);
+            meta[b] = window_meta_of(none, n);
+        }
+        return;
+    }
     if (lo >= n) return;
     const int nblock = (int)((lo + kChunk < n) ? kChunk : n - lo);
     const int lane = threadIdx.x & 63, wave = threadIdx.x >> 6;
+    constexpr int kChunkShift = TPB * PL == 4096 ? 12 : 13;
+    static_assert(TPB * PL == 1 << kChunkShift, "a block run is 4096 or 8192 events");
+    const uint32_t nb = (uint32_t)min((int)(((uint32_t)n + (1u << kChunkShift) - 1u) >> kChunkShift), nblk);
+    unsigned long long *tw = ticket + (size_t)b * (kTicketStride / sizeof(unsigned long long));
+    unsigned long long seen = 0ull;
+    if (threadIdx.x == 0 && !(KS_DEBUG & 16)) seen = __hip_atomic_load(tw, __ATOMIC_RELAXED, __HIP_MEMORY_SCOPE_AGENT);
     const int w0 = wave * kPerWave;
     const int lo32 = (int)lo;
     const int4 *evb = ev + beg + lo;
@@ -920,7 +959,7 @@
         }
     }
     for (int i = threadIdx.x; i <= NK; i += TPB) base[i] = 0;
-    if (threadIdx.x == 0) nhot_s = 0u;
+    if (threadIdx.x == 0) { nhot_s = 0u; seen_s = seen; }
     if (threadIdx.x < 12) {
         const int f = threadIdx.x;
         bstats[f] = (f == 0 || f == 2 || f == 4) ? INT32_MAX : ((f == 1 || f == 3 || f == 5) ? INT32_MIN : 0);
@@ -1013,7 +1052,8 @@
             run += c;
         }
     if (threadIdx.x == 0) base[NK] = total;
-    if (threadIdx.x < 12) reinterpret_cast<int *>(stats + (size_t)b * nblk + blk)[threadIdx.x] = bstats[threadIdx.x];
+    if (threadIdx.x < 12)
+        __hip_atomic_store(reinterpret_cast<int *>(stats + (size_t)b * nblk + blk) + threadIdx.x, bstats[threadIdx.x], __ATOMIC_RELAXED, __HIP_MEMORY_SCOPE_AGENT);
     __syncthreads();
     uint32_t *tb = table + ((size_t)b * nblk + blk) * ((size_t)NK + 1);
     if (!(KS_DEBUG & 8))
@@ -1092,6 +1132,33 @@
             if (ko[i] != 0xffffffffu) ko[i] = (ko[i] >> 31) ? (ko[i] & 0x7fffffffu) : gb[i] + sm[i];
     }
     if (nhot) __syncthreads();
+    const BlockStats *wrec = stats + (size_t)b * nblk;
+    uint32_t tk = 0u;
+    if (wave == 0 && !(KS_DEBUG & 16)) {
+        asm volatile("s_waitcnt vmcnt(0)" ::: "memory");
+        if (lane == 0) tk = ticket_arrive(tw, seen_s, nb);
+    }
+    bool asked = false, last = false;
+    int q[10] = {0, 0, 0, 0, 0, 0, 0, 0, 0, 0};
+    auto ask = [&]() {
+        asked = true;
+        last = (uint32_t)__builtin_amdgcn_readfirstlane((int)tk) == nb;
+        if (last && (uint32_t)lane < nb) stats_load_agent(wrec + lane, q);
+    };
+    auto publish = [&]() {
+        BlockStats st;
+        stats_identity(st);
+        if ((uint32_t)lane < nb) stats_merge_words(st, q);
+        for (uint32_t k = (uint32_t)(lane + kWave); k < nb; k += kWave) {
+            stats_load_agent(wrec + k, q);
+            stats_merge_words(st, q);
+        }
+        stats_wave_reduce(st);
+        if (lane == 0) {
+            meta[b] = window_meta_of(st, n);
+            __hip_atomic_store(tw, (unsigned long long)kTicketTag << 32, __ATOMIC_RELAXED, __HIP_MEMORY_SCOPE_AGENT);
+        }
+    };
     Rec8 *dst = reinterpret_cast<Rec8 *>(sorted1) + beg + lo;
 #if KS_DIRECT_WRITE
 #pragma unroll
@@ -1102,7 +1169,7 @@
             dst[ko[i]] = rec8_pack(col, lo32 + w0 + i * kWave + lane, e[i].z, e[i].w);
         }
     }
-    return;
+    total = 0u;
 #endif
     for (uint32_t pb = 0; pb < total && !(KS_DEBUG & 2); pb += (uint32_t)cap) {
         if (pb) __syncthreads();
@@ -1117,30 +1184,13 @@
         }
         __syncthreads();
         const uint32_t cnt = min((uint32_t)cap, total - pb);
+        if (PL == 4 && wave == 0 && cnt == total - pb) ask();
         for (uint32_t t = threadIdx.x; t < cnt; t += TPB) dst[pb + t] = stage[t];
     }
-}
-
-#ifdef EVREP_TU_CORE
-static __global__ __launch_bounds__(kWave) void k_window_meta(const int64_t *__restrict__ nwin, const BlockStats *__restrict__ stats,
-                                                      int nblk, int chunk_shift, WindowMeta *__restrict__ meta) {
-    const int b = blockIdx.x, lane = threadIdx.x;
-    const int64_t n_win = nwin[b];
-    const int nb = min((int)(((uint32_t)n_win + (1u << chunk_shift) - 1u) >> chunk_shift), nblk);
-    BlockStats st;
-    stats_identity(st);
-    for (int k = lane; k < nb; k += kWave) stats_merge(st, stats[(size_t)b * nblk + k]);
-    stats_wave_reduce(st);
-    if (lane == 0) {
-        WindowMeta m;
-        m.tmin = st.tmin; m.tmax = st.tmax; m.xmin = st.xmin; m.xmax = st.xmax; m.ymin = st.ymin; m.ymax = st.ymax;
-        m.neg_flags = st.neg_flags; m.oob_flags = st.oob_flags; m.status = st.status & 0xffffu; m.n_valid = st.n_valid;
-        if (n_win <= 0) m.status |= EVREP_ST_EMPTY;
-        else if (st.tmin == st.tmax) m.status |= EVREP_ST_FLAT_TIME;
-        for (int i = 0; i < 6; ++i) m.pad[i] = 0;
-        meta[b] = m;
-    }
-}
-#endif
-
-}
+    if (wave == 0) {
+        if (!asked) ask();
+        if (last) publish();
+    }
+}
+
+}
diff --git a/event_representation_study_amd/csrc/evrep_builders.hip b/event_representation_study_amd/csrc/evrep_builders.hip
--- a/event_representation_study_amd/csrc/evrep_builders.hip
+++ b/event_representation_study_amd/csrc/evrep_builders.hip
@@ -224,11 +224,17 @@
     uint32_t hot_cap;
     double *placed_pool;
     BlockStats *stats_rw;
+    WindowMeta *meta_rw;
 #ifdef EVREP_TIMING
     unsigned long long *dbg;
     unsigned long long *dbg_wave;
 #endif
 };
+
+__device__ inline void report_hot_overflow(const BinView &bv, int b) {
+    atomicOr(&bv.meta_rw[b].status, EVREP_ST_HOT_OVERFLOW);
+    atomicOr(&bv.stats_rw[(size_t)b * bv.nblk].status, EVREP_ST_HOT_OVERFLOW);
+}
 
 struct UnitRecs {
     const Rec *sorted;
@@ -606,7 +612,7 @@
             } else {
                 ok = defer_items(bv, uid, (uint32_t)kHotWhole, 1u);
             }
-            if (!ok && lane == 0) atomicOr(&bv.stats_rw[(size_t)b * bv.nblk].status, EVREP_ST_HOT_OVERFLOW);
+            if (!ok && lane == 0) report_hot_overflow(bv, b);
             u.deferred = true;
             u.ce = nrec;
             return u;
@@ -797,7 +803,7 @@
             wave_phase();
         }
         if constexpr (HOT) {
-            if (lane == 0) atomicOr(&bv.stats_rw[(size_t)b * bv.nblk].status, EVREP_ST_HOT_OVERFLOW);
+            if (lane == 0) report_hot_overflow(bv, b);
             u.deferred = true;
             return u;
         }
@@ -912,7 +918,7 @@
     wave_phase();
     if (defer) {
         if (!defer_unit(bv, uid, (npix_out + kWave - 1) / kWave, defer_mask) && lane == 0)
-            atomicOr(&bv.stats_rw[(size_t)b * bv.nblk].status, EVREP_ST_HOT_OVERFLOW);
+            report_hot_overflow(bv, b);
         u.deferred = true;
         u.ce = nrec;
         return u;
@@ -976,61 +982,21 @@
 __device__ inline MetaRaw meta_prefetch(const BinView &bv, int b) {
     MetaRaw r;
     r.q0 = make_int4(0, 0, 0, 0); r.q1 = r.q0; r.q2 = r.q0;
-    if (bv.fused) {
-        if ((int)threadIdx.x < bv.nblk) {
-            const int4 *sp = reinterpret_cast<const int4 *>(bv.stats + (size_t)b * bv.nblk + threadIdx.x);
-            r.q0 = sp[0]; r.q1 = sp[1]; r.q2 = sp[2];
-        }
-    } else if (threadIdx.x == 0) {
+    if (threadIdx.x == 0) {
         const int4 *mp = reinterpret_cast<const int4 *>(bv.meta + b);
         r.q0 = mp[0]; r.q1 = mp[1]; r.q2 = mp[2];
     }
     return r;
 }
-__device__ inline WindowMeta meta_finish(const BinView &bv, const int64_t *__restrict__ off, int b, const MetaRaw &r) {
+__device__ inline uint32_t meta_status(const BinView &bv, const MetaRaw &r) { return (uint32_t)r.q2.x | (bv.fused ? (uint32_t)r.q2.z : 0u); }
+__device__ inline WindowMeta meta_finish(const BinView &bv, const int64_t *__restrict__, int, const MetaRaw &r) {
     WindowMeta m;
-    if (!bv.fused) {
-        m.tmin = __builtin_amdgcn_readfirstlane(r.q0.x); m.tmax = __builtin_amdgcn_readfirstlane(r.q0.y);
-        m.xmin = __builtin_amdgcn_readfirstlane(r.q0.z); m.xmax = __builtin_amdgcn_readfirstlane(r.q0.w);
-        m.ymin = __builtin_amdgcn_readfirstlane(r.q1.x); m.ymax = __builtin_amdgcn_readfirstlane(r.q1.y);
-        m.neg_flags = (uint32_t)__builtin_amdgcn_readfirstlane(r.q1.z);
-        m.oob_flags = (uint32_t)__builtin_amdgcn_readfirstlane(r.q1.w);
-        m.status = (uint32_t)__builtin_amdgcn_readfirstlane(r.q2.x); m.n_valid = __builtin_amdgcn_readfirstlane(r.q2.y);
-        return m;
-    }
-    const int lane = threadIdx.x;
-    const int64_t n_win = off[b + 1] - off[b];
-    const int nb = min((int)(((uint32_t)n_win + (1u << bv.chunk_shift) - 1u) >> bv.chunk_shift), bv.nblk);
-    BlockStats st;
-    stats_identity(st);
-    if (lane < nb) {
-        st.tmin = r.q0.x; st.tmax = r.q0.y; st.xmin = r.q0.z; st.xmax = r.q0.w;
-        st.ymin = r.q1.x; st.ymax = r.q1.y; st.neg_flags = (uint32_t)r.q1.z; st.oob_flags = (uint32_t)r.q1.w;
-        st.status = (uint32_t)r.q2.x; st.n_valid = r.q2.y;
-    }
-    m.tmin = nb > 0 ? __builtin_amdgcn_readlane(st.tmin, 0) : INT32_MAX;
-    m.tmax = nb > 0 ? __builtin_amdgcn_readlane(st.tmax, min(nb, kWave) - 1) : INT32_MIN;
-    if (nb > kWave) {
-        BlockStats s2;
-        stats_identity(s2);
-        if (kWave + lane < nb) {
-            const int4 *sp = reinterpret_cast<const int4 *>(bv.stats + (size_t)b * bv.nblk + kWave + lane);
-            const int4 a0 = sp[0], a1 = sp[1], a2 = sp[2];
-            s2.tmin = a0.x; s2.tmax = a0.y; s2.xmin = a0.z; s2.xmax = a0.w;
-            s2.ymin = a1.x; s2.ymax = a1.y; s2.neg_flags = (uint32_t)a1.z; s2.oob_flags = (uint32_t)a1.w;
-            s2.status = (uint32_t)a2.x; s2.n_valid = a2.y;
-        }
-        m.tmax = __builtin_amdgcn_readlane(s2.tmax, nb - kWave - 1);
-        stats_merge(st, s2);
-    }
-    m.xmin = wave_min(st.xmin); m.xmax = wave_max(st.xmax);
-    m.ymin = wave_min(st.ymin); m.ymax = wave_max(st.ymax);
-    m.neg_flags = wave_or(st.neg_flags); m.oob_flags = wave_or(st.oob_flags);
-    m.status = wave_or(st.status); m.n_valid = wave_sum(st.n_valid);
-    if (m.status & EVREP_ST_UNSORTED) {
-        m.tmin = wave_min(st.tmin);
-        m.tmax = wave_max(st.tmax);
-    }
+    m.tmin = __builtin_amdgcn_readfirstlane(r.q0.x); m.tmax = __builtin_amdgcn_readfirstlane(r.q0.y);
+    m.xmin = __builtin_amdgcn_readfirstlane(r.q0.z); m.xmax = __builtin_amdgcn_readfirstlane(r.q0.w);
+    m.ymin = __builtin_amdgcn_readfirstlane(r.q1.x); m.ymax = __builtin_amdgcn_readfirstlane(r.q1.y);
+    m.neg_flags = (uint32_t)__builtin_amdgcn_readfirstlane(r.q1.z);
+    m.oob_flags = (uint32_t)__builtin_amdgcn_readfirstlane(r.q1.w);
+    m.status = (uint32_t)__builtin_amdgcn_readfirstlane((int)meta_status(bv, r)); m.n_valid = __builtin_amdgcn_readfirstlane(r.q2.y);
     return m;
 }
 __device__ inline WindowMeta window_meta(const BinView &bv, const int64_t *__restrict__ off, int b) {
@@ -1893,7 +1859,7 @@
         auto never = []() -> bool { return false; };
         auto nof = [](uint32_t, const Rec8 &, uint2 &, const uint2 &) -> bool { return false; };
         auto sp = unit_split<true>(never, nof, never, kErgoSplitWords,
-                                   (uint32_t)mraw.q2.x | ((uc.xflags & (kXfHandOverWhole | kXfHandOverMonsters | kXfCoopErgo12)) ? 0u : kStEscaped),
+                                   meta_status(bv, mraw) | ((uc.xflags & (kXfHandOverWhole | kXfHandOverMonsters | kXfCoopErgo12)) ? 0u : kStEscaped),
                                    (uc.xflags & kXfHandOverWhole) ? 0u : kHotSubMin);
         sp.coop_min = (uc.xflags & kXfCoopErgo12) ? kErgoCoopMin : 0u;
         u = unit_front<OutT, HOT, false, NoVisit>(bv, off, H, W, nchunk, uc, w, g, uid, part, NoVisit(), sp);
@@ -2748,16 +2714,7 @@
     const int64_t beg = off[b];
     const int64_t n = off[b + 1] - beg;
     int32_t wtmin = INT32_MAX, wtmax = INT32_MIN;
-    if (bv.fused) {
-        const int nb = min((int)(((uint32_t)n + (1u << bv.chunk_shift) - 1u) >> bv.chunk_shift), bv.nblk);
-        for (int k = s; k < nb; k += kWave) {
-            const int2 q = *reinterpret_cast<const int2 *>(bv.stats + (size_t)b * bv.nblk + k);
-            wtmin = min(wtmin, q.x);
-            wtmax = max(wtmax, q.y);
-        }
-        wtmin = wave_min(wtmin);
-        wtmax = wave_max(wtmax);
-    } else if (n > 0) {
+    if (n > 0) {
         wtmin = bv.meta[b].tmin;
         wtmax = bv.meta[b].tmax;
     }
@@ -3605,7 +3562,7 @@
         const uint32_t avg = (uint32_t)((uint64_t)n_win / (uint64_t)(H * nchunk));
         if (nrec > (uint32_t)uc.stage && nrec > 3u * avg) {
             if (!defer_items(bv, uid, (uint32_t)kHotWhole, 1u) && lane == 0)
-                atomicOr(&bv.stats_rw[(size_t)b * bv.nblk].status, EVREP_ST_HOT_OVERFLOW);
+                report_hot_overflow(bv, b);
             return;
         }
     }
diff --git a/event_representation_study_amd/csrc/evrep_capi.hip b/event_representation_study_amd/csrc/evrep_capi.hip
--- a/event_representation_study_amd/csrc/evrep_capi.hip
+++ b/event_representation_study_amd/csrc/evrep_capi.hip
@@ -100,7 +100,7 @@
         table_words = (size_t)B * nblk * ((size_t)NK + 1);
     }
     size_t o = 0;
-    plan->off_meta = o;    o += up256((size_t)B * sizeof(WindowMeta));
+    plan->off_meta = o;    o += meta_region_bytes(B);
     plan->off_table = o;   o += up256(table_words * sizeof(uint32_t));
     plan->off_stats = o;   o += up256((size_t)B * nblk * sizeof(BlockStats));
     plan->off_rowoff = o;  o += up256((size_t)B * (H + 1) * sizeof(uint32_t));
@@ -129,6 +129,7 @@
     Rec *s2 = WS(Rec, off_sorted2);
     BlockStats *stats = WS(BlockStats, off_stats);
     const unsigned xgrid = 8u * (unsigned)((B + 7) / 8) * (unsigned)nblk;
+    unsigned long long *tickets = reinterpret_cast<unsigned long long *>(static_cast<char *>(workspace) + ticket_offset(plan));
     uint32_t *hot = WS(uint32_t, off_scratch);
     if (plan->reserved != 2 && plan->reserved != 3) {
         int rc2 = hip_check(hipMemsetAsync(hot, 0, (size_t)kHotHdrWords * 4, stream), "hipMemsetAsync(hot list)");
@@ -147,13 +148,13 @@
                             : (block_keysort_lds_bytes(NK, 2048, 4096) <= 52 * 1024 ? 2048 : 4096);
             if (int rc2 = opt_in(reinterpret_cast<const void *>(&k_block_keysort<1024, 4>), block_keysort_lds_bytes(NK, cap, 4096))) return rc2;
             k_block_keysort<1024, 4><<<xgrid, 1024, block_keysort_lds_bytes(NK, cap, 4096), stream>>>(
-                ev, offsets, B, H, W, plan->nchunk, nblk, cap, table, stats, s1, reinterpret_cast<int64_t *>(row_off), hot);
+                ev, offsets, B, H, W, plan->nchunk, nblk, cap, table, stats, s1, meta, tickets, hot);
         } else {
             const int cap = block_keysort_lds_bytes(NK, 4096, kBsChunk) <= 79 * 1024 ? 4096
                             : (block_keysort_lds_bytes(NK, kBsChunk, kBsChunk) + 1024 <= 160 * 1024 ? kBsChunk : 4096);
             if (int rc2 = opt_in(reinterpret_cast<const void *>(&k_block_keysort<1024>), block_keysort_lds_bytes(NK, cap, kBsChunk))) return rc2;
             k_block_keysort<1024><<<xgrid, kBsThreads, block_keysort_lds_bytes(NK, cap, kBsChunk), stream>>>(
-                ev, offsets, B, H, W, plan->nchunk, nblk, cap, table, stats, s1, reinterpret_cast<int64_t *>(row_off), hot);
+                ev, offsets, B, H, W, plan->nchunk, nblk, cap, table, stats, s1, meta, tickets, hot);
         }
         LAUNCH_CHECK("k_block_keysort");
         if (plan->reserved == 3) return column_sort_keys(plan, events, offsets, workspace, stream);
@@ -197,14 +198,6 @@
 static int read_meta_field(const evrep_plan *plan, const void *workspace, size_t field_off, size_t field_bytes,
                            void *dst, hipStream_t stream) {
     const char *meta = static_cast<const char *>(workspace) + plan->off_meta;
-    if (plan->reserved == 2) {
-        char *ws = const_cast<char *>(static_cast<const char *>(workspace));
-        k_window_meta<<<plan->B, kWave, 0, stream>>>(reinterpret_cast<const int64_t *>(ws + plan->off_rowoff),
-                                                     reinterpret_cast<const BlockStats *>(ws + plan->off_stats), plan->nblk, plan->chunk == 4096 ? 12 : 13,
-                                                     reinterpret_cast<WindowMeta *>(ws + plan->off_meta));
-        int rc0 = hip_check(hipGetLastError(), "k_window_meta");
-        if (rc0) return rc0;
-    }
     int rc = hip_check(hipMemcpy2DAsync(dst, field_bytes, meta + field_off, sizeof(WindowMeta), field_bytes,
                                         (size_t)plan->B, hipMemcpyDeviceToHost, stream), "hipMemcpy2DAsync(meta)");
     if (rc) return rc;
@@ -215,13 +208,6 @@
     if (!plan || plan->abi_version != EVREP_ABI_VERSION || !workspace || !meta_out) return EVREP_EINVAL;
     hipStream_t stream = as_stream(stream_);
     const char *meta = static_cast<const char *>(workspace) + plan->off_meta;
-    if (plan->reserved == 2) {
-        char *ws = const_cast<char *>(static_cast<const char *>(workspace));
-        k_window_meta<<<plan->B, kWave, 0, stream>>>(reinterpret_cast<const int64_t *>(ws + plan->off_rowoff),
-                                                     reinterpret_cast<const BlockStats *>(ws + plan->off_stats), plan->nblk, plan->chunk == 4096 ? 12 : 13,
-                                                     reinterpret_cast<WindowMeta *>(ws + plan->off_meta));
-        LAUNCH_CHECK("k_window_meta");
-    }
     return hip_check(hipMemcpyAsync(meta_out, meta, (size_t)plan->B * sizeof(WindowMeta), hipMemcpyDeviceToHost, stream),
                      "hipMemcpyAsync(meta)");
 }
diff --git a/event_representation_study_amd/csrc/evrep_capi_builders.h b/event_representation_study_amd/csrc/evrep_capi_builders.h
--- a/event_representation_study_amd/csrc/evrep_capi_builders.h
+++ b/event_representation_study_amd/csrc/evrep_capi_builders.h
@@ -25,6 +25,7 @@
     bv.hot = WS(uint32_t, off_scratch);
     bv.hot_cap = hot_items_total(plan->total_events);
     bv.stats_rw = WS(BlockStats, off_stats);
+    bv.meta_rw = WS(WindowMeta, off_meta);
     bv.placed_pool = reinterpret_cast<double *>(static_cast<char *>(workspace) + plan->off_sorted1 + align16((size_t)plan->total_events * 8));
     bv.chunk_shift = plan->chunk == 4096 ? 12 : 13;
 #ifdef EVREP_TIMING
diff --git a/event_representation_study_amd/csrc/evrep_capi_builders.hip b/event_representation_study_amd/csrc/evrep_capi_builders.hip
--- a/event_representation_study_amd/csrc/evrep_capi_builders.hip
+++ b/event_representation_study_amd/csrc/evrep_capi_builders.hip
@@ -357,7 +357,7 @@
     const UnitCfg us = stream_cfg(plan, unit_cfg(plan, 4, 0, true, false));
     constexpr int kRB = 4;
     k_render_state<kRB><<<unit_grid(plan, us), kWave, render_state_lds_bytes(kChunkPx, kRB), stream>>>(
-        bin_view(plan, events, workspace, true), offsets, plan->H, plan->W, plan->nchunk, us, tau, WS(WindowMeta, off_meta), state, net, surface);
+        bin_view(plan, events, workspace, true), offsets, plan->H, plan->W, plan->nchunk, us, tau, state, net, surface);
     LAUNCH_CHECK("k_render_state");
     return EVREP_OK;
 }
diff --git a/event_representation_study_amd/csrc/evrep_capi_shared.h b/event_representation_study_amd/csrc/evrep_capi_shared.h
--- a/event_representation_study_amd/csrc/evrep_capi_shared.h
+++ b/event_representation_study_amd/csrc/evrep_capi_shared.h
@@ -46,6 +46,9 @@
     }
 };
 
+static inline size_t ticket_offset(const evrep_plan *plan) { return plan->off_meta + up256((size_t)plan->B * sizeof(evrep::WindowMeta)); }
+static inline size_t meta_region_bytes(int B) { return up256((size_t)B * sizeof(evrep::WindowMeta)) + up256((size_t)B * evrep::kTicketStride); }
+
 #define WS(type, field) reinterpret_cast<type *>(static_cast<char *>(workspace) + plan->field)
 #define CWS(type, field) reinterpret_cast<const type *>(static_cast<const char *>(workspace) + plan->field)
 
diff --git a/event_representation_study_amd/csrc/evrep_common.h b/event_representation_study_amd/csrc/evrep_common.h
--- a/event_representation_study_amd/csrc/evrep_common.h
+++ b/event_representation_study_amd/csrc/evrep_common.h
@@ -1,5 +1,6 @@
 #pragma once
 #include <hip/hip_runtime.h>
+#include <stddef.h>
 #include <stdint.h>
 
 #include "evrep.h"
@@ -48,9 +49,14 @@
     uint32_t oob_flags;
     uint32_t status;
     int32_t n_valid;
-    int32_t pad[6];
+    uint32_t lib_status;
+    int32_t pad[5];
 };
 static_assert(sizeof(WindowMeta) == 64, "WindowMeta is one 64-byte line");
+static_assert(offsetof(WindowMeta, lib_status) == 40, "the builders read status, n_valid and lib_status in one 16-byte load");
+
+constexpr uint32_t kTicketTag = 0x7e1c4e70u;
+constexpr size_t kTicketStride = 64;
 
 using Rec = int4;
 
diff --git a/event_representation_study_amd/csrc/evrep_render.hip b/event_representation_study_amd/csrc/evrep_render.hip
--- a/event_representation_study_amd/csrc/evrep_render.hip
+++ b/event_representation_study_amd/csrc/evrep_render.hip
@@ -7,7 +7,7 @@
 }
 template <int RB>
 __global__ __launch_bounds__(kWave, 6) void k_render_state(BinView bv, const int64_t *__restrict__ off, int H, int W, int nchunk, UnitCfg uc,
-                                                       double tau, WindowMeta *__restrict__ meta_out, unsigned char *__restrict__ state,
+                                                       double tau, unsigned char *__restrict__ state,
                                                        int32_t *__restrict__ net, float *__restrict__ surface) {
     extern __shared__ __align__(16) unsigned char smem[];
     const int lane = threadIdx.x;
@@ -102,16 +102,6 @@
     }
     if (net) for (int px = lane; px < g.npix; px += kWave) net[o + px] = netl[px];
     if (surface) for (int px = lane; px < g.npix; px += kWave) surface[o + px] = acc[px];
-    if (bv.fused && g.row == 0 && chunk == 0) {
-        WindowMeta m = window_meta(bv, off, b);
-        if (lane == 0) {
-            m.status &= 0xffffu;
-            if (n_win <= 0) m.status |= EVREP_ST_EMPTY;
-            else if (m.tmin == m.tmax) m.status |= EVREP_ST_FLAT_TIME;
-            for (int i = 0; i < 6; ++i) m.pad[i] = 0;
-            meta_out[b] = m;
-        }
-    }
 }
 
 constexpr int kRcThreads = 256;
```

Measured after the change: 9.211 billion (median of 6 runs). About the same (+0.4%).
